# ucl-exoplanets/wayne

Measured on AMD Instinct MI355X. Metric: simulated WFC3-IR exposures/sec (1014x1014, NSAMP=16, spatial scan), higher is better.
Workload: dtype k_ramp<float, true, 1, false, true>: exact integer sums (int64 accumulators + int32 sky counts) then an all-f32 per-read chain; f32 thrower (int32 LDS tiles -> int64 fixed-point accumulators, 2^-28 e-); f32 reads; 1 GPU; cfg4: G141 spatial scan 5 px/s, SUBARRAY=1024 (frame 1014x1014), SPARS10 NSAMP=16, K=128 sub-samples, W=4494 bins, 9.92e+08 electrons/exposure, all detector effects on (flat, sky, cosmic rays, gain, dark, non-linearity, clip, read noise), thrower=split (wide component per electron, narrow component multinomial), f32 reads (the default of ExposureGenerator, Observation, VisitRunner and the CLI), on; exposures_per_rank=2241

## Files before the change

include/wayne_hip.h:

```cpp
#ifndef WAYNE_HIP_H
#define WAYNE_HIP_H

#include <stddef.h>
#include <stdint.h>

#ifdef __cplusplus
extern "C" {
#endif

#define WAYNE_ABI_VERSION 7

#define WAYNE_OK 0
#define WAYNE_E_INVALID (-1)
#define WAYNE_E_NEGATIVE (-2)
#define WAYNE_E_OVERFLOW (-3)
#define WAYNE_E_NOMEM (-4)
#define WAYNE_E_HIP (-5)
#define WAYNE_E_NODEVICE (-6)
#define WAYNE_E_STATE (-7)

#define WAYNE_RNG_REPLAY 0
#define WAYNE_RNG_PHILOX 1
#define WAYNE_RNG_SPLIT 2

// ... 64 lines not shown
  const float *lin[4];
  const float *dark_sci;
  const float *dark_err;
  const double *zero_read;
} wayne_calibration;

int wayne_ctx_set_calibration(wayne_ctx *ctx, const wayne_calibration *c);


typedef struct wayne_exposure_desc {
  uint32_t seed;
  uint32_t exposure_index;
  int rng_mode;
  int threads_compat;
  uint32_t flags;
  int sub_scale;

  int n_wl;
  const double *wl_um;
  const double *flux;
  const double *depth;

  int n_samples;
  const double *x_ref;
  const double *y_ref;
  const double *dur_ms;
  const int32_t *replay_seed;
  const int32_t *sample_read;

  int n_reads;
  const double *read_dt_s;

  double sky_ct_s;
  double cosmic_rate;
  double scale_factor;
  double noise_mean;
  double noise_std;

  int thrower_margin;
  int thrower_splits;

  const double *lc_z;
  const double *lc_hidden;
  const double *lc_rp;
  double lc_ld[4];
} wayne_exposure_desc;

int wayne_ctx_slots(const wayne_ctx *ctx);
int wayne_exposure_upload(wayne_ctx *ctx, int slot, const wayne_exposure_desc *d);
int wayne_exposure_run(wayne_ctx *ctx, int slot);
int wayne_exposure_run_checked(wayne_ctx *ctx, int slot);
int wayne_exposure_status(wayne_ctx *ctx, int slot, int *status);
unsigned long long wayne_ctx_reruns(const wayne_ctx *ctx);
int wayne_exposure_download(wayne_ctx *ctx, int slot, void *out_reads);
int wayne_exposure_fetch_async(wayne_ctx *ctx, int slot);
int wayne_exposure_wait(wayne_ctx *ctx, int slot, void **host_reads);
void *wayne_exposure_device_reads(wayne_ctx *ctx, int slot);
int wayne_exposure_synthesize(wayne_ctx *ctx, const wayne_exposure_desc *d,
                              void *out_reads);

int wayne_exposure_debug_fetch(wayne_ctx *ctx, int slot, int32_t *counts,
                               double *x_pos, double *y_pos, double *acc_e);
int wayne_exposure_debug_depth(wayne_ctx *ctx, int slot, double *depth);
int wayne_exposure_debug_boxes(wayne_ctx *ctx, int slot, int32_t *boxes, int32_t *segments, int *use_box);
int wayne_exposure_run_front(wayne_ctx *ctx, int slot);
int wayne_exposure_run_back(wayne_ctx *ctx, int slot);
int wayne_exposure_ramp_variant(wayne_ctx *ctx, int slot, char *buf, int cap);


typedef struct wayne_source_desc {
  uint32_t tag;
  int n_wl;
  const double *wl_um;
  const double *flux;
  double dx, dy;
} wayne_source_desc;

#define WAYNE_MAX_SOURCES 8

int wayne_exposure_set_sources(wayne_ctx *ctx, int slot, const wayne_source_desc *src, int n);
uint32_t wayne_source_seed(uint32_t seed, uint32_t tag);
int wayne_exposure_debug_fetch_source(wayne_ctx *ctx, int slot, int source, int32_t *counts, double *x_pos,
                                      double *y_pos);


typedef struct wayne_trap_desc {
  double n_traps[2];
  double efficiency[2];
  double lifetime_s[2];
  int n_rate;
  double rate_lo, rate_hi;
  const double *start[2];
} wayne_trap_desc;

#define WAYNE_MAX_TRAP_RATES 4096

int wayne_exposure_set_traps(wayne_ctx *ctx, int slot, const wayne_trap_desc *t);

typedef struct wayne_trap_history_desc {
  double gap_s;
  int lit;
  double fill[2];
} wayne_trap_history_desc;

int wayne_ctx_trap_state_reset(wayne_ctx *ctx, const double initial[2]);
int wayne_ctx_trap_state_upload(wayne_ctx *ctx, const float *state);
int wayne_ctx_trap_state_download(wayne_ctx *ctx, float *state);

int wayne_exposure_set_trap_history(wayne_ctx *ctx, int slot, const wayne_trap_history_desc *h);


#define WAYNE_X_LINEARISE (1u << 0)
#define WAYNE_X_DARK (1u << 1)
#define WAYNE_X_GAIN (1u << 2)
#define WAYNE_X_SKY (1u << 3)
#define WAYNE_X_LAST_READ (1u << 4)
#define WAYNE_X_ALL 31u

typedef struct wayne_extract_desc {
  uint32_t steps;
  int row_lo[17];
  int row_hi[17];
  int bg_col_lo;
  int bg_col_hi;
} wayne_extract_desc;

int wayne_exposure_set_extraction(wayne_ctx *ctx, int slot, const wayne_extract_desc *x);
int wayne_exposure_fetch_spectra_async(wayne_ctx *ctx, int slot);
int wayne_exposure_wait_spectra(wayne_ctx *ctx, int slot, double **spectra, double **sky);
int wayne_exposure_download_spectra(wayne_ctx *ctx, int slot, double *spectra, double *sky);
typedef struct wayne_crrej_desc {
  double k;
  double read_noise_e;
} wayne_crrej_desc;

int wayne_exposure_set_crrej(wayne_ctx *ctx, int slot, const wayne_crrej_desc *r);
int wayne_exposure_rejected(wayne_ctx *ctx, int slot, const uint32_t **n_rejected);
int wayne_exposure_download_crmask(wayne_ctx *ctx, int slot, uint16_t *mask);
#define WAYNE_C_FLAT (1u << 0)
#define WAYNE_MAX_CHANNELS 256
#define WAYNE_MAX_CHANNEL_HULL 384

typedef struct wayne_channels_desc {
  int n_channels;
  const double *edges_um;
  const double *wl_a;
  const double *wl_b;
  uint32_t flags;
} wayne_channels_desc;

int wayne_exposure_set_channels(wayne_ctx *ctx, int slot, const wayne_channels_desc *d);
int wayne_exposure_channels(wayne_ctx *ctx, int slot, const double **channels);
typedef struct wayne_variance_desc {
  double read_noise;
} wayne_variance_desc;

int wayne_exposure_set_variance(wayne_ctx *ctx, int slot, const wayne_variance_desc *v);
int wayne_exposure_variances(wayne_ctx *ctx, int slot, const double **spectra_var, const double **sky_var,
                             const double **channels_var);
#define WAYNE_MAX_OPTIMAL_HALF_WIDTH 16
typedef struct wayne_optimal_desc {
  int half_width;
} wayne_optimal_desc;

int wayne_exposure_set_optimal(wayne_ctx *ctx, int slot, const wayne_optimal_desc *d);
int wayne_exposure_optimal(wayne_ctx *ctx, int slot, const double **optimal, const double **optimal_var);
// ... 104 lines not shown
```

wayne_amd/_lib.py:

```python
import ctypes as C
import os
import threading
import weakref

import numpy as np

from . import build as _build

OK, E_INVALID, E_NEGATIVE, E_OVERFLOW, E_NOMEM, E_HIP, E_NODEVICE, E_STATE = 0, -1, -2, -3, -4, -5, -6, -7
RNG_REPLAY, RNG_PHILOX, RNG_SPLIT = 0, 1, 2
F_ADD_FLAT = 1 << 0
F_ADD_GAIN_VARIATIONS = 1 << 1
F_ADD_NON_LINEAR = 1 << 2
F_CLIP_DET_LIMITS = 1 << 3
F_ADD_READ_NOISE = 1 << 4
F_ADD_STELLAR_NOISE = 1 << 5
F_ADD_DARK = 1 << 6
F_ADD_INITIAL_BIAS = 1 << 7
F_OUT_F64 = 1 << 16
F_OUT_U16 = 1 << 18
OUT_FLAGS = {np.dtype(np.float32): 0, np.dtype(np.float64): F_OUT_F64, np.dtype(np.uint16): F_OUT_U16}
F_EXACT_SAMPLERS = 1 << 17
PROF_KERNELS = 8
ABI_VERSION = 7
# ... 73 lines not shown

class CrrejDesc(C.Structure):
    _fields_ = [("k", C.c_double), ("read_noise_e", C.c_double)]


class ChannelsDesc(C.Structure):
    _fields_ = [("n_channels", C.c_int), ("edges_um", _dp), ("wl_a", _dp), ("wl_b", _dp), ("flags", C.c_uint32)]


class VarianceDesc(C.Structure):
    _fields_ = [("read_noise", C.c_double)]


class RampFitDesc(C.Structure):
    _fields_ = [("steps", C.c_uint32), ("read_noise_e", C.c_double), ("k_jump", C.c_double), ("saturation_dn", C.c_double)]


class ImaDesc(C.Structure):
    _fields_ = [("steps", C.c_uint32), ("units", C.c_int), ("read_noise_e", C.c_double), ("saturation_dn", C.c_double)]


class SpotsDesc(C.Structure):
    _fields_ = [("n", C.c_int32), ("cx", C.c_double * 8), ("cy", C.c_double * 8), ("radius", C.c_double * 8),
                ("contrast", C.POINTER(C.c_double)), ("px", C.POINTER(C.c_double)), ("py", C.POINTER(C.c_double))]


class IpcDesc(C.Structure):
    _fields_ = [("k", (C.c_double * 3) * 3)]


class OptimalDesc(C.Structure):
    _fields_ = [("half_width", C.c_int)]


class Profile(C.Structure):
    _fields_ = [("name", C.c_char_p * PROF_KERNELS), ("launches", C.c_uint64 * PROF_KERNELS),
                ("ms", C.c_double * PROF_KERNELS), ("electrons", C.c_uint64)]


_vp = C.c_void_p
SYMBOLS = {
    "wayne_abi_version": (C.c_int, []),
    "wayne_strerror": (C.c_char_p, [C.c_int]),
    "wayne_build_flags": (C.c_char_p, []),
    "wayne_device_count": (C.c_int, []),
    "wayne_ctx_create": (_vp, [C.c_int, C.POINTER(C.c_int)]),
    "wayne_ctx_destroy": (None, [_vp]),
    "wayne_last_error": (C.c_char_p, [_vp]),
    "wayne_ctx_synchronize": (C.c_int, [_vp]),
    "wayne_ctx_stream": (_vp, [_vp]),
    "wayne_ctx_set_knob": (C.c_int, [_vp, C.c_char_p, C.c_longlong]),
    "wayne_ctx_get_knob": (C.c_int, [_vp, C.c_char_p, C.POINTER(C.c_longlong)]),
    "wayne_psf_apply": (C.c_int, [_vp, _vp, C.c_int, _vp, _vp, _vp, _vp, _vp, C.c_int, C.c_int,
                                  C.c_uint32, C.c_int, C.c_int, C.c_uint32, C.c_uint32, _vp]),
    "wayne_psf_apply_ex": (C.c_int, [_vp, _vp, C.c_int, _vp, _vp, _vp, _vp, _vp, C.c_int, C.c_int,
                                     C.c_uint32, C.c_int, C.c_int, C.c_uint32, C.c_uint32, C.c_uint32, _vp]),
    "wayne_ctx_set_grism": (C.c_int, [_vp, C.POINTER(GrismDesc)]),
    "wayne_ctx_set_calibration": (C.c_int, [_vp, C.POINTER(Calibration)]),
    "wayne_ctx_slots": (C.c_int, [_vp]),
    "wayne_exposure_upload": (C.c_int, [_vp, C.c_int, C.POINTER(ExposureDesc)]),
    "wayne_exposure_run": (C.c_int, [_vp, C.c_int]),
    "wayne_exposure_run_checked": (C.c_int, [_vp, C.c_int]),
    "wayne_exposure_status": (C.c_int, [_vp, C.c_int, C.POINTER(C.c_int)]),
    "wayne_ctx_reruns": (C.c_ulonglong, [_vp]),
    "wayne_exposure_download": (C.c_int, [_vp, C.c_int, _vp]),
    "wayne_exposure_fetch_async": (C.c_int, [_vp, C.c_int]),
    "wayne_exposure_wait": (C.c_int, [_vp, C.c_int, C.POINTER(C.c_void_p)]),
    "wayne_exposure_device_reads": (_vp, [_vp, C.c_int]),
    "wayne_exposure_synthesize": (C.c_int, [_vp, C.POINTER(ExposureDesc), _vp]),
    "wayne_exposure_debug_fetch": (C.c_int, [_vp, C.c_int, _vp, _vp, _vp, _vp]),
    "wayne_exposure_debug_depth": (C.c_int, [_vp, C.c_int, _vp]),
    "wayne_exposure_debug_boxes": (C.c_int, [_vp, C.c_int, _vp, _vp, C.POINTER(C.c_int)]),
    "wayne_exposure_run_front": (C.c_int, [_vp, C.c_int]),
    "wayne_exposure_run_back": (C.c_int, [_vp, C.c_int]),
    "wayne_exposure_ramp_variant": (C.c_int, [_vp, C.c_int, C.c_char_p, C.c_int]),
    "wayne_exposure_set_sources": (C.c_int, [_vp, C.c_int, C.POINTER(SourceDesc), C.c_int]),
    "wayne_source_seed": (C.c_uint32, [C.c_uint32, C.c_uint32]),
    "wayne_exposure_set_traps": (C.c_int, [_vp, C.c_int, C.POINTER(TrapDesc)]),
    "wayne_ctx_trap_state_reset": (C.c_int, [_vp, _dp]),
    "wayne_ctx_trap_state_upload": (C.c_int, [_vp, _vp]),
    "wayne_ctx_trap_state_download": (C.c_int, [_vp, _vp]),
    "wayne_exposure_set_trap_history": (C.c_int, [_vp, C.c_int, C.POINTER(TrapHistoryDesc)]),
    "wayne_exposure_debug_fetch_source": (C.c_int, [_vp, C.c_int, C.c_int, _vp, _vp, _vp]),
    "wayne_exposure_set_extraction": (C.c_int, [_vp, C.c_int, C.POINTER(ExtractDesc)]),
    "wayne_exposure_fetch_spectra_async": (C.c_int, [_vp, C.c_int]),
    "wayne_exposure_wait_spectra": (C.c_int, [_vp, C.c_int, C.POINTER(_dp), C.POINTER(_dp)]),
    "wayne_exposure_download_spectra": (C.c_int, [_vp, C.c_int, _vp, _vp]),
    "wayne_exposure_set_crrej": (C.c_int, [_vp, C.c_int, C.POINTER(CrrejDesc)]),
    "wayne_exposure_rejected": (C.c_int, [_vp, C.c_int, C.POINTER(C.POINTER(C.c_uint32))]),
    "wayne_exposure_download_crmask": (C.c_int, [_vp, C.c_int, _vp]),
    "wayne_exposure_set_channels": (C.c_int, [_vp, C.c_int, C.POINTER(ChannelsDesc)]),
    "wayne_exposure_channels": (C.c_int, [_vp, C.c_int, C.POINTER(_dp)]),
    "wayne_exposure_set_variance": (C.c_int, [_vp, C.c_int, C.POINTER(VarianceDesc)]),
    "wayne_exposure_variances": (C.c_int, [_vp, C.c_int, C.POINTER(_dp), C.POINTER(_dp), C.POINTER(_dp)]),
    "wayne_exposure_set_optimal": (C.c_int, [_vp, C.c_int, C.POINTER(OptimalDesc)]),
    "wayne_exposure_optimal": (C.c_int, [_vp, C.c_int, C.POINTER(_dp), C.POINTER(_dp)]),
    "wayne_exposure_deliver_profile": (C.c_int, [_vp, C.c_int, C.c_int]),
    "wayne_exposure_set_optimal_profile": (C.c_int, [_vp, C.c_int, _dp, C.POINTER(C.c_int)]),
    "wayne_exposure_set_optimal_profile_tagged": (C.c_int, [_vp, C.c_int, _dp, C.POINTER(C.c_int), C.c_uint64]),
    "wayne_ctx_profile_uploads": (C.c_ulonglong, [_vp]),
    "wayne_exposure_set_optimal_channels": (C.c_int, [_vp, C.c_int, C.c_int]),
    "wayne_exposure_optimal_channels": (C.c_int, [_vp, C.c_int, C.POINTER(_dp), C.POINTER(_dp)]),
    "wayne_exposure_fetch_profile": (C.c_int, [_vp, C.c_int]),
    "wayne_exposure_profile": (C.c_int, [_vp, C.c_int, C.POINTER(_dp), C.POINTER(C.c_size_t)]),
    "wayne_extract_profile": (C.c_int, [_vp, C.POINTER(C.c_uint64), C.POINTER(C.c_double)]),
    "wayne_fits_layout": (C.c_int, [C.c_int, C.c_int, C.c_uint32, C.POINTER(C.c_size_t), C.POINTER(C.c_size_t),
                                    C.POINTER(C.c_int)]),
    "wayne_exposure_set_fits": (C.c_int, [_vp, C.c_int, C.c_int]),
    "wayne_exposure_fetch_fits_async": (C.c_int, [_vp, C.c_int]),
    "wayne_exposure_wait_fits": (C.c_int, [_vp, C.c_int, C.POINTER(C.c_void_p)]),
    "wayne_exposure_download_fits": (C.c_int, [_vp, C.c_int, _vp]),
    "wayne_fits_profile": (C.c_int, [_vp, C.POINTER(C.c_uint64), C.POINTER(C.c_double)]),
    "wayne_exposure_set_expected": (C.c_int, [_vp, C.c_int, C.c_int]),
    "wayne_exposure_download_expected": (C.c_int, [_vp, C.c_int, _dp]),
    "wayne_expected_profile": (C.c_int, [_vp, C.POINTER(C.c_uint64), C.POINTER(C.c_double)]),
    "wayne_exposure_set_rampfit": (C.c_int, [_vp, C.c_int, C.POINTER(RampFitDesc)]),
    "wayne_exposure_download_rampfit": (C.c_int, [_vp, C.c_int, _dp, _dp, C.POINTER(C.c_uint32)]),
    "wayne_rampfit_profile": (C.c_int, [_vp, C.POINTER(C.c_uint64), C.POINTER(C.c_double)]),
    "wayne_ima_layout": (C.c_int, [C.c_int, C.c_int, C.POINTER(C.c_size_t), C.POINTER(C.c_size_t), C.POINTER(C.c_size_t)]),
    "wayne_exposure_set_ima": (C.c_int, [_vp, C.c_int, C.POINTER(ImaDesc)]),
    "wayne_exposure_download_ima": (C.c_int, [_vp, C.c_int, _vp]),
    "wayne_ima_profile": (C.c_int, [_vp, C.POINTER(C.c_uint64), C.POINTER(C.c_double)]),
    "wayne_ipc_weights": (C.c_int, [C.POINTER(IpcDesc), C.POINTER(C.c_int32)]),
    "wayne_exposure_set_ipc": (C.c_int, [_vp, C.c_int, C.POINTER(IpcDesc)]),
    "wayne_ipc_profile": (C.c_int, [_vp, C.POINTER(C.c_uint64), C.POINTER(C.c_double)]),
    "wayne_exposure_set_limb_darkening": (C.c_int, [_vp, C.c_int, _dp, C.c_int]),
    "wayne_exposure_set_spots": (C.c_int, [_vp, C.c_int, C.POINTER(SpotsDesc), C.c_int, C.c_int]),
    "wayne_spot_lens_basis": (None, [C.c_double] * 6 + [_dp]),
    "wayne_spot_rule": (None, [_dp, _dp]),
    "wayne_spots_profile": (C.c_int, [_vp, C.POINTER(C.c_uint64), C.POINTER(C.c_double)]),
    "wayne_profile_enable": (C.c_int, [_vp, C.c_int]),
    "wayne_profile_select": (C.c_int, [_vp, C.c_uint]),
    "wayne_profile_reset": (C.c_int, [_vp]),
    "wayne_profile_get": (C.c_int, [_vp, C.POINTER(Profile)]),
    "wayne_philox4x32": (None, [_vp, _vp, _vp]),
    "wayne_host_sample_draws": (None, [C.c_uint32, C.c_uint32, C.c_int, _vp, _vp, _vp]),
}

_lib = None


def load():
    global _lib, _lib_path
    if _lib is None:
        path = _build.LIB
        override = os.environ.get("WAYNE_HIP_LIB")
        if override:
            path = override
        elif _build.stale():
            if os.path.exists(_build.HIPCC):
                _build.build(verbose=False)
            elif not os.path.exists(path):
                raise ImportError("libwayne_hip.so is not built and hipcc is unavailable (%s)" % _build.HIPCC)
        L = C.CDLL(path)
        for name, (res, args) in SYMBOLS.items():
            f = getattr(L, name)
            f.restype = res
            f.argtypes = args
        if L.wayne_abi_version() != ABI_VERSION:
            raise ImportError("libwayne_hip.so ABI version mismatch")
        flags = L.wayne_build_flags().decode().split()
        if flags and os.environ.get("WAYNE_ALLOW_FLAGGED_LIB", "") != "1":
            raise ImportError("%s was built with %s: not the product's library (tests and measurement scripts that mean "
                              "to load it set WAYNE_ALLOW_FLAGGED_LIB=1)" % (path, " ".join(flags)))
        _lib = L
        _lib_path = path
    return _lib


_lib_path = None


def library_info():
    L = load()
    return _lib_path or _build.LIB, L.wayne_build_flags().decode().strip()


def ptr(a, ctype=None):
    if a is None:
        return None
    assert a.flags["C_CONTIGUOUS"]
    if ctype is None:
        return a.ctypes.data_as(C.c_void_p)
    return a.ctypes.data_as(C.POINTER(ctype))


def out_dtype_of(flags):
    return np.dtype(np.float64 if flags & F_OUT_F64 else np.uint16 if flags & F_OUT_U16 else np.float32)


def f64(a):
    return np.ascontiguousarray(a, dtype=np.float64)


def f32(a):
    return np.ascontiguousarray(a, dtype=np.float32)


def i32(a):
    return np.ascontiguousarray(a, dtype=np.int32)


KNOBS = ("tile_ints", "batch", "thin", "no_acc_box", "lane_reach", "throw_wgs", "keep_narrow", "no_fuse", "fork_narrow",
         "streams", "upload_timing", "ramp_reads", "narrow_compact", "lane_tight_tile",
         "fuse_thrower", "prep_wl_per_run")
_live_contexts = weakref.WeakSet()
_knob_defaults = {}


def set_knob_all(name, value):
    if name not in KNOBS:
        raise KeyError("no knob named %r" % (name,))
    if value is None:
        _knob_defaults.pop(name, None)
    else:
        _knob_defaults[name] = int(value)
    for c in list(_live_contexts):
        if getattr(c, "_h", None):
            c.set_knob(name, value)


def reset_knobs_all():
    for name in list(_knob_defaults):
        set_knob_all(name, None)


class Context(object):

    def __init__(self, device=0):
        self._L = load()
        st = C.c_int(0)
        self._h = self._L.wayne_ctx_create(int(device), C.byref(st))
        if not self._h:
            msg = self._L.wayne_strerror(st.value).decode()
            cls = WayneNoDeviceError if st.value == E_NODEVICE else WayneError
            raise cls(st.value, "wayne_ctx_create(device=%d): %s -- the HIP path is the only path, "
                                "there is no CPU fallback" % (device, msg))
        self.device = device
        self._slot_meta = {}
        self._slot_src = {}
        self._slot_crrej = set()
        self._slot_chan = {}
        self._slot_var = set()
        self._slot_opt = set()
        self._slot_optch = set()
        self._slot_prof = set()
        self._slot_fits = {}
        self._slot_expected = {}
        self._slot_rampfit = {}
        self._slot_ima = {}
        _live_contexts.add(self)
        for name, value in _knob_defaults.items():
            self.set_knob(name, value)

    def close(self):
        if getattr(self, "_h", None):
            self._L.wayne_ctx_destroy(self._h)
            self._h = None

    def __del__(self):
        try:
            self.close()
        except Exception:
            pass

    def __enter__(self):
        return self

    def __exit__(self, *a):
        self.close()

    def check(self, status):
        if status != OK:
            raise WayneError(status, self._L.wayne_last_error(self._h).decode())

    def synchronize(self):
        self.check(self._L.wayne_ctx_synchronize(self._h))

    def set_knob(self, name, value):
        self.check(self._L.wayne_ctx_set_knob(self._h, name.encode(), -1 if value is None else int(value)))

    def get_knob(self, name):
        v = C.c_longlong(0)
        self.check(self._L.wayne_ctx_get_knob(self._h, name.encode(), C.byref(v)))
        return None if v.value < 0 else int(v.value)

    @property
    def stream(self):
# ... 472 lines not shown
        self.check(self._L.wayne_extract_profile(self._h, C.byref(n), C.byref(ms)))
        return {"launches": int(n.value), "ms": float(ms.value)}

    def set_ipc(self, slot, ipc):
        if ipc is None:
            self.check(self._L.wayne_exposure_set_ipc(self._h, int(slot), None))
            return
        self.check(self._L.wayne_exposure_set_ipc(self._h, int(slot), C.byref(ipc_desc(ipc))))

    def ipc_profile(self):
        n, ms = C.c_uint64(0), C.c_double(0.0)
        self.check(self._L.wayne_ipc_profile(self._h, C.byref(n), C.byref(ms)))
        return int(n.value), float(ms.value)

    def set_traps(self, slot, traps):
        if traps is None:
            self.check(self._L.wayne_exposure_set_traps(self._h, int(slot), None))
            return
        m, table = traps.traps, np.ascontiguousarray(traps.table, dtype=np.float64)
        if table.ndim != 2 or table.shape[0] != 2:
            raise ValueError("charge traps: the start tables have shape (2, G)")
        t = TrapDesc()
        t.n_traps[:] = [float(v) for v in m.array("n_traps")]
        t.efficiency[:] = [float(v) for v in m.array("efficiency")]
        t.lifetime_s[:] = [float(v) for v in m.array("lifetime_s")]
        t.n_rate, t.rate_lo, t.rate_hi = int(table.shape[1]), float(m.rate_lo), float(m.rate_hi)
        rows = [np.ascontiguousarray(table[0]), np.ascontiguousarray(table[1])]
        t.start[0], t.start[1] = ptr(rows[0], C.c_double), ptr(rows[1], C.c_double)
        self.check(self._L.wayne_exposure_set_traps(self._h, int(slot), C.byref(t)))

    def set_trap_history(self, slot, history):
        if history is None:
            self.check(self._L.wayne_exposure_set_trap_history(self._h, int(slot), None))
            return
        h = TrapHistoryDesc()
        h.gap_s, h.lit = float(history.gap_s), int(bool(history.lit))
        h.fill[:] = [float(v) for v in history.fill]
        self.check(self._L.wayne_exposure_set_trap_history(self._h, int(slot), C.byref(h)))

    def trap_state_reset(self, initial):
        v = (C.c_double * 2)(float(initial[0]), float(initial[1]))
        self.check(self._L.wayne_ctx_trap_state_reset(self._h, v))

    def trap_state_upload(self, state):
        if not getattr(self, "S", 0):
            raise WayneError(E_STATE, "trap_state_upload: set the calibration first")
        state = np.ascontiguousarray(state, dtype=np.float32)
        if state.shape != (self.S, self.S, 2):
            raise ValueError("trap state: expected shape (%d, %d, 2), got %s" % (self.S, self.S, state.shape))
        self.check(self._L.wayne_ctx_trap_state_upload(self._h, state.ctypes.data_as(C.c_void_p)))

    def trap_state_download(self):
        if not getattr(self, "S", 0):
            raise WayneError(E_STATE, "trap_state_download: set the calibration first")
        out = np.empty((self.S, self.S, 2), dtype=np.float32)
        self.check(self._L.wayne_ctx_trap_state_download(self._h, out.ctypes.data_as(C.c_void_p)))
        return out

    def set_sources(self, slot, sources):
        sources = list(sources)
        arr = (SourceDesc * max(len(sources), 1))()
        keep = []
        for i, s in enumerate(sources):
            wl, fl = f64(s.wl), f64(s.flux)
            if wl.size != fl.size:
                raise ValueError("contaminant %d: wl and flux differ in length" % i)
            keep += [wl, fl]
            arr[i].tag, arr[i].n_wl = int(s.tag), wl.size
            arr[i].wl_um, arr[i].flux = ptr(wl, C.c_double), ptr(fl, C.c_double)
            arr[i].dx, arr[i].dy = float(s.dx), float(s.dy)
        self._slot_src[slot] = ()
        self.check(self._L.wayne_exposure_set_sources(self._h, int(slot), arr, len(sources)))
        self._slot_src[slot] = tuple(int(k.size) for k in keep[0::2])

    def debug_fetch_source(self, slot, source):
        K, W, R, _ = self._slot_meta[slot]
        if source > 0:
            W = self._slot_src[slot][source - 1]
        counts = np.empty((K, W), dtype=np.int32)
        x = np.empty((K, W), dtype=np.float64)
        y = np.empty((K, W), dtype=np.float64)
        self.check(self._L.wayne_exposure_debug_fetch_source(self._h, int(slot), int(source), ptr(counts), ptr(x), ptr(y)))
        return counts, x, y

    def run(self, slot):
        self.check(self._L.wayne_exposure_run(self._h, int(slot)))

    def run_checked(self, slot):
        self.check(self._L.wayne_exposure_run_checked(self._h, int(slot)))

    def run_front(self, slot):
        self.check(self._L.wayne_exposure_run_front(self._h, int(slot)))

    def run_back(self, slot):
        self.check(self._L.wayne_exposure_run_back(self._h, int(slot)))

    def ramp_variant(self, slot):
        buf = C.create_string_buffer(128)
        self.check(self._L.wayne_exposure_ramp_variant(self._h, int(slot), buf, len(buf)))
        return buf.value.decode()

    def status(self, slot):
        st = C.c_int(0)
        self.check(self._L.wayne_exposure_status(self._h, int(slot), C.byref(st)))
        return st.value

    @property
    def reruns(self):
        return int(self._L.wayne_ctx_reruns(self._h))

    def download(self, slot):
        K, W, R, dtype = self._slot_meta[slot]
        out = np.empty((R + 1, self.S, self.S), dtype=dtype)
        self.check(self._L.wayne_exposure_download(self._h, int(slot), ptr(out)))
        return out

    def fetch_async(self, slot):
        self.check(self._L.wayne_exposure_fetch_async(self._h, int(slot)))

    def wait(self, slot):
        K, W, R, dtype = self._slot_meta[slot]
        p = C.c_void_p()
        self.check(self._L.wayne_exposure_wait(self._h, int(slot), C.byref(p)))
        n = (R + 1) * self.S * self.S
        buf = (C.c_ubyte * (n * dtype.itemsize)).from_address(p.value)
        return np.frombuffer(buf, dtype=dtype).reshape(R + 1, self.S, self.S)

    def synthesize(self, desc):
        self.upload(0, desc)
        self.run(0)
        return self.download(0)

    def debug_depth(self, slot):
        K, W, R, _ = self._slot_meta[slot]
        out = np.empty((K, W), dtype=np.float64)
        self.check(self._L.wayne_exposure_debug_depth(self._h, int(slot), ptr(out)))
        return out

    def debug_boxes(self, slot):
        boxes = np.zeros((16, 4), dtype=np.int32)
        seg = np.zeros(16, dtype=np.int32)
        use = C.c_int(0)
        self.check(self._L.wayne_exposure_debug_boxes(self._h, int(slot), ptr(boxes), ptr(seg), C.byref(use)))
        return bool(use.value), boxes, seg

    def debug_fetch(self, slot, acc=False):
        K, W, R, _ = self._slot_meta[slot]
        counts = np.empty((K, W), dtype=np.int32)
        x = np.empty((K, W), dtype=np.float64)
        y = np.empty((K, W), dtype=np.float64)
        a = np.empty((R, self.S, self.S), dtype=np.float64) if acc else None
        self.check(self._L.wayne_exposure_debug_fetch(self._h, int(slot), ptr(counts), ptr(x), ptr(y), ptr(a)))
        return counts, x, y, a

    def profile_enable(self, on=True):
        self.check(self._L.wayne_profile_enable(self._h, 1 if on else 0))

    def profile_select(self, names=None):
        if names is None:
            mask = 0xFFFFFFFF
        else:
            order = list(self.profile_get().keys())[:PROF_KERNELS] + ["k_extract", "k_fits_words", "k_expect", "k_ramp_fit", "k_ima", "k_ipc",
                                                                     "k_lightcurve_spots"]
            mask = 0
            for n in names:
                mask |= 1 << order.index(n)
# ... 184 lines not shown
```

wayne_amd/csrc/common.h:

```cpp
#pragma once
#include <hip/hip_runtime.h>
#include <stdint.h>
#include <type_traits>
#include "philox.h"
#include "plan_consts.h"
#include "samplers.h"

namespace wayne {

constexpr int kQBits = 28;
constexpr double kQ = 268435456.0;
constexpr double kInvQ = 1.0 / 268435456.0;
constexpr double kGain = 2.35;
constexpr double kReadNoise = 14.1 / 2.35;
constexpr double kMinCounts = -20.0;
constexpr double kMaxCounts = 78000.0;
constexpr double kPi = 3.14159265358979323846;



struct SubInfo {
  uint32_t electrons;
  int tx0, ty0, tw, th;
  int read;
  int replay_seed;
  int pad_;
  double x_ref, y_ref;
  double a_t_i, a_w, b_w;
  double inv_norm;
};

struct WlArrays {
  double* ratio;
  double* sigl;
  double* sigh;
  double* sens;
  double* dlam;
};

__device__ __forceinline__ double poly3(const double* c, double x) {
  return ((c[0] * x + c[1]) * x + c[2]) * x + c[3];
}

#if defined(__HIPCC__)
struct BinLocal { float fx, fy; int ox, oy; bool sane; };
__device__ __forceinline__ BinLocal bin_local(double xd, double yd) {
  BinLocal b;
  const bool sane = fabs(xd) < 1e6 && fabs(yd) < 1e6;
  b.sane = sane;
  const double flx = sane ? floor(xd) : 0., fly = sane ? floor(yd) : 0.;
  b.fx = (float)(xd - flx); b.fy = (float)(yd - fly);
  b.ox = (int)flx; b.oy = (int)fly;
#ifdef WAYNE_NEGCTL_DROP_FRACTION
  b.fx = 0.f; b.fy = 0.f;
#endif
  return b;
}
__device__ __forceinline__ int floor_to_int(float v) {
  int r;
  asm("v_cvt_flr_i32_f32 %0, %1" : "=v"(r) : "v"(v));
  return r;
}


template <int CTRL> __device__ __forceinline__ int dpp_row(int v) { return __builtin_amdgcn_update_dpp(v, v, CTRL, 0xF, 0xF, false); }
#define WAYNE_ROW16(name, T, cast_in, cast_out, op)                                   \
  __device__ __forceinline__ T name(T v) {                                            \
    v = op(v, cast_out(dpp_row<0x128>(cast_in(v))));                   \
    v = op(v, cast_out(dpp_row<0x124>(cast_in(v))));                   \
    v = op(v, cast_out(dpp_row<0x122>(cast_in(v))));                   \
    v = op(v, cast_out(dpp_row<0x121>(cast_in(v))));                   \
    return v;                                                                         \
  }
__device__ __forceinline__ int wayne_addi(int a, int b) { return a + b; }
WAYNE_ROW16(row16_min, float, __float_as_int, __int_as_float, fminf)
WAYNE_ROW16(row16_max, float, __float_as_int, __int_as_float, fmaxf)
WAYNE_ROW16(row16_mini, int, , , min)
WAYNE_ROW16(row16_maxi, int, , , max)
WAYNE_ROW16(row16_sum, int, , , wayne_addi)
#undef WAYNE_ROW16
__device__ __forceinline__ int wave_mini(int v) {
  v = row16_mini(v);
  return min(min(__builtin_amdgcn_readlane(v, 0), __builtin_amdgcn_readlane(v, 16)),
             min(__builtin_amdgcn_readlane(v, 32), __builtin_amdgcn_readlane(v, 48)));
}
__device__ __forceinline__ int wave_maxi(int v) {
  v = row16_maxi(v);
  return max(max(__builtin_amdgcn_readlane(v, 0), __builtin_amdgcn_readlane(v, 16)),
             max(__builtin_amdgcn_readlane(v, 32), __builtin_amdgcn_readlane(v, 48)));
}
__device__ __forceinline__ unsigned long long wave_sum_u32(uint32_t n) {
  const int lo = row16_sum((int)(n & 0xFFFFFFu)), hi = row16_sum((int)(n >> 24));
  const unsigned long long L = (unsigned long long)(uint32_t)(__builtin_amdgcn_readlane(lo, 0) + __builtin_amdgcn_readlane(lo, 16) +
                                                              __builtin_amdgcn_readlane(lo, 32) + __builtin_amdgcn_readlane(lo, 48));
  const unsigned long long H = (unsigned long long)(uint32_t)(__builtin_amdgcn_readlane(hi, 0) + __builtin_amdgcn_readlane(hi, 16) +
                                                              __builtin_amdgcn_readlane(hi, 32) + __builtin_amdgcn_readlane(hi, 48));
  return L + (H << 24);
}
#endif

}
```

wayne_amd/csrc/k_narrow.h:

```cpp
#pragma once
#include "common.h"
#include "k_throw.h"

namespace wayne {

constexpr int kNarrowCells = 2 * kNarrowR + 1;
constexpr int kPoolRows = 2 * kNarrowR + 2;
constexpr int kNarrowTile = 1536;

constexpr float kTailCut = 6.5f;
template <class M>
__device__ __forceinline__ float upper_tail(float t) {
  if (__all(t > kTailCut)) return 0.f;
  const float z = t * 0.70710678118654752f;
  const float u = M::div_(1.f, 1.f + 0.5f * z);
  float p = 0.17087277f;
  p = fmaf(p, u, -0.82215223f);
  p = fmaf(p, u, 1.48851587f);
  p = fmaf(p, u, -1.13520398f);
  p = fmaf(p, u, 0.27886807f);
  p = fmaf(p, u, -0.18628806f);
  p = fmaf(p, u, 0.09678418f);
  p = fmaf(p, u, 0.37409196f);
  p = fmaf(p, u, 1.00002368f);
  p = fmaf(p, u, -1.26551223f);
  p = fmaf(-z, z, p);
  return (t > kTailCut) ? 0.f : (0.5f * u) * M::exp_(p);
}

constexpr int kLaneTile = 9216;
constexpr int kNarrowLds = kNarrowTile + kPoolRows * kNarrowThreads + 2 * kNarrowThreads;
constexpr int kThrowerLds = kNarrowLds > kLaneTile ? kNarrowLds : kLaneTile;

template <int FLUSH, bool FAST, bool COMPACT>
__device__ __forceinline__ void narrow_body(const ThrowArgs& a, int* const lds, const unsigned by) {
  typedef typename std::conditional<FAST, FastMath, ExactMath<float> >::type M;
  int* const tile = lds;
  float (*const s_q)[kNarrowThreads] = reinterpret_cast<float (*)[kNarrowThreads]>(lds + kNarrowTile);
  int* const s_pool = lds + kNarrowTile + kPoolRows * kNarrowThreads;
  float* const s_cond = reinterpret_cast<float*>(s_pool + kNarrowThreads);
  __shared__ int s_box[4];
  __shared__ float s_fc[10];
  __shared__ int s_gx[COMPACT ? kNarrowThreads / 16 : 1], s_gj[COMPACT ? kNarrowThreads / 16 : 1], s_hist[COMPACT ? 32 : 1];
  if (threadIdx.x < 10) s_fc[threadIdx.x] = (float)kStirlingSmall[threadIdx.x];
  if (COMPACT && threadIdx.x < 32) s_hist[threadIdx.x] = 0;
  const int k = blockIdx.x;
  const int tid = threadIdx.x;
  const uint32_t order_word = reinterpret_cast<const uint32_t*>(a.chunk_order)[by >> 2];
  const int w = (int)((order_word >> (8 * (by & 3))) & 0xFFu) * kNarrowThreads + tid;
  const SubInfo si = a.sub[k];
  int n0 = 0;
  double xd = 0., yd = 0., sgd = 1.;
  if (w < a.W) {
    const size_t kw = (size_t)k * a.W + w;
    n0 = a.nsplit[kw];
    xd = a.xpos[kw];
    yd = a.ypos[kw];
    sgd = a.sigl[w];
  }
  if (!__syncthreads_or(n0 > 0)) return;
  const bool split = n0 > 0;
  BinLocal bl{};
  if (split) bl = bin_local(xd, yd);
  const bool act = split && bl.sane;
  const float sg = split ? (float)sgd : 1.f;
  const int ic0 = bl.ox, jc0 = bl.oy;
  s_pool[tid] = 0;
  if (tid == 0) { s_box[0] = 0x7FFFFFFF; s_box[1] = -0x7FFFFFFF; s_box[2] = 0x7FFFFFFF; s_box[3] = -0x7FFFFFFF; }
  __syncthreads();
  {
    const int x_lo = wave_mini(act ? ic0 - kNarrowR : 0x7FFFFFFF), x_hi = wave_maxi(act ? ic0 + kNarrowR + 1 : -0x7FFFFFFF);
    const int y_lo = wave_mini(act ? jc0 - kNarrowR : 0x7FFFFFFF), y_hi = wave_maxi(act ? jc0 + kNarrowR + 1 : -0x7FFFFFFF);
    if ((tid & 63) == 0) {
      atomicMin(&s_box[0], x_lo); atomicMax(&s_box[1], x_hi);
      atomicMin(&s_box[2], y_lo); atomicMax(&s_box[3], y_hi);
    }
  }
  __syncthreads();
  int tx0 = max(s_box[0], 1), tx1 = min(s_box[1], a.N), ty0 = max(s_box[2], 1), ty1 = min(s_box[3], a.N);
  int tw = max(tx1 - tx0, 0), th = max(ty1 - ty0, 0);
  if ((long long)tw * th > kNarrowTile) { th = min(th, kNarrowTile / max(tw, 1)); if (th < 1) { th = 0; tw = 0; } }
  const int tarea = tw * th;
  for (int i = tid; i < tarea; i += kNarrowThreads) tile[i] = 0;

  auto deposit = [&](int ci, int rj, int m) {
    const int lx = ci - tx0, ly = rj - ty0;
    if ((unsigned)lx < (unsigned)tw && (unsigned)ly < (unsigned)th)
      atomicAdd(&tile[ly * tw + lx], m);
    else if (ci > 0 && ci < a.N && rj > 0 && rj < a.N)
      deposit_global<FLUSH>(a, si, ci, rj, m);
  };

  const bool any_multi = __any(act);
  const float inv_s = 1.f / sg;
  const int grp = tid & ~15, gl = tid & 15;
  bool pool = false;
  int X0 = 0, J0 = 0, res = 0;
  float Z = 1.f, Rb = 0.f, yl = 0.f;
  if (any_multi) {
    const int cnt = row16_sum(split ? 1 : 0), cnt_sane = row16_sum(act ? 1 : 0), tot = row16_sum(split ? n0 : 0);
    const int icmin = row16_mini(act ? ic0 : 0x7FFFFFFF), icmax = row16_maxi(act ? ic0 : -0x7FFFFFFF);
    const int jcmin = row16_mini(act ? jc0 : 0x7FFFFFFF);
    X0 = icmin - kNarrowR;
    J0 = jcmin - kNarrowR;
    yl = act ? (float)(yd - (double)J0) : 0.f;
    const float ymin = row16_min(act ? yl : 3e38f), ymax = row16_max(act ? yl : -3e38f);
    const float smin = row16_min(split ? sg : 3e38f), smax = row16_max(split ? sg : 0.f);
    pool = cnt >= 2 && cnt_sane == cnt && icmax - icmin <= 2 && (ymax - ymin) <= 0.25f * smin && smax <= 1.1f * smin &&
           tot <= 16777216;

    float qh[kPoolRows];
#pragma unroll
    for (int t = 0; t < kPoolRows; ++t) qh[t] = 3e38f;
    if (act && pool) {
      float Ep = -yl, Ap = upper_tail<M>(fabsf(Ep) * inv_s), S = 0.f;
#pragma unroll
      for (int t = 0; t < kPoolRows; ++t) {
        const float E = (float)(t + 1) - yl, A = upper_tail<M>(fabsf(E) * inv_s);
        const float m = (Ep >= 0.f) ? Ap - A : ((E <= 0.f) ? A - Ap : 1.f - Ap - A);
        qh[t] = fmaxf(m, 0.f);
        S += qh[t];
        Ep = E; Ap = A;
      }
#pragma unroll
      for (int t = 0; t < kPoolRows; ++t) qh[t] = M::div_(qh[t], S);
    } else if (act) {
      const float f = bl.fy;
      float up = upper_tail<M>((1.f - f) * inv_s), lo = upper_tail<M>(f * inv_s);
      s_q[0][tid] = 1.f - up - lo;
      for (int c = 1; c < kNarrowCells; ++c) {
        const int d = (c + 1) >> 1;
        const float rem = up + lo;
        float Q;
        if (c & 1) { const float nx = upper_tail<M>(((float)(d + 1) - f) * inv_s); Q = up - nx; up = nx; }
        else       { const float nx = upper_tail<M>(((float)d + f) * inv_s);       Q = lo - nx; lo = nx; }
        s_q[c][tid] = fminf(fmaxf(M::div_(Q, rem), 0.f), 1.f);
      }
    }
    if (__any(pool)) {
      float qb[kPoolRows];
#pragma unroll
      for (int t = 0; t < kPoolRows; ++t) qb[t] = row16_min(qh[t]);
      float PL[kNarrowR + 1], SU[kPoolRows + 1];
      PL[0] = qb[0];
#pragma unroll
      for (int t = 1; t <= kNarrowR; ++t) PL[t] = PL[t - 1] + qb[t];
      SU[kPoolRows] = 0.f;
#pragma unroll
      for (int t = kPoolRows - 1; t > kNarrowR; --t) SU[t] = SU[t + 1] + qb[t];
      Z = fminf(PL[kNarrowR] + SU[kNarrowR + 1], 1.f);
      if (act && pool) {
#pragma unroll
        for (int t = 0; t < kPoolRows; ++t) {
          Rb += qh[t] - qb[t];
          s_q[t][tid] = Rb;
        }
      }
      if (pool && gl == 0) {
        s_cond[grp] = fminf(fmaxf(M::div_(qb[kNarrowR], PL[kNarrowR] + SU[kNarrowR + 1]), 0.f), 1.f);
#pragma unroll
        for (int i = 1; i < kPoolRows; ++i) {
          const int u = (i + 1) >> 1;
// ... 83 lines not shown
          if (left > 0.f) {
            m = binomial<M>(left, s_cond[grp + i], rp, s_fc);
            left -= m;
          }
          if (m > 0.f) {
            const int u = (i + 1) >> 1;
            deposit(X0 + gl, J0 + ((i & 1) ? kNarrowR + u : kNarrowR - u), (int)m);
          }
        }
      }
    }
  }
  if (COMPACT) {
    __builtin_amdgcn_fence(__ATOMIC_RELEASE, "wavefront");
    __builtin_amdgcn_wave_barrier();
    __builtin_amdgcn_fence(__ATOMIC_ACQUIRE, "wavefront");
    const int mine = pool ? s_pool[tid] : 0;
    if (gl == 0) { s_gx[tid >> 4] = X0; s_gj[tid >> 4] = J0; }
    if (__syncthreads_or(mine > 0)) {
      int* const list = reinterpret_cast<int*>(&s_q[0][0]);
      const int cls = (mine > 0) ? 31 - __clz(mine) : 0;
      int rank = 0;
      if (mine > 0) rank = atomicAdd(&s_hist[cls], 1);
      __syncthreads();
      const int lane = tid & 63;
      const int h = (lane < 32) ? s_hist[31 - lane] : 0;
      int incl = h;
#pragma unroll
      for (int off = 1; off < 32; off <<= 1) {
        const int v = __shfl_up(incl, off);
        if (lane >= off) incl += v;
      }
      const int first = __shfl(incl - h, 31 - cls), n_live = __shfl(incl, 31);
      if (mine > 0) list[first + rank] = tid;
      __syncthreads();
      if ((tid & ~63) < n_live) {
        const int slot = (tid < n_live) ? list[tid] : 0;
        float left = (tid < n_live) ? (float)s_pool[slot] : 0.f;
        const int cgrp = slot & ~15, cl = slot & 15;
        const int cX = s_gx[slot >> 4] + cl, cJ0 = s_gj[slot >> 4];
        SeededStream rp(a.seed, STAGE_POOL, (uint32_t)(w - tid + slot) >> 4, (uint32_t)k + a.subsample0, a.exposure, (uint32_t)cl);
        for (int i = 0; i < kPoolRows; ++i) {
          if (!__any(left > 0.f)) break;
          float m = 0.f;
          if (left > 0.f) {
            m = binomial<M>(left, s_cond[cgrp + i], rp, s_fc);
            left -= m;
          }
          if (m > 0.f) {
            const int u = (i + 1) >> 1;
            deposit(cX, cJ0 + ((i & 1) ? kNarrowR + u : kNarrowR - u), (int)m);
          }
        }
      }
    }
  }
  __syncthreads();
  flush_tile<FLUSH, false, kNarrowThreads>(a, si, tile, tx0, ty0, tw, tarea);
}

template <int FLUSH, bool FAST, bool COMPACT>
__global__ __launch_bounds__(kNarrowThreads) void k_narrow(ThrowArgs a) {
  __shared__ int lds[kNarrowLds];
  narrow_body<FLUSH, FAST, COMPACT>(a, lds, blockIdx.y);
}

constexpr float kLaneR16 = 4.63f;
constexpr float kLaneR34 = 6.9f;
constexpr int kLaneMargin = 30;
constexpr int kLaneReachMax = 48;


template <int FLUSH, bool THIN, bool BATCH, bool FUSED>
__device__ __forceinline__ void lane_body(const ThrowArgs& a, const PrepArgs& p, const CosmicArgs& ca, int* const tile, const unsigned by) {
  __shared__ SubInfo s_sub[FUSED ? kLaneBatchMax : 1];
  __shared__ uint32_t s_hits;
  __shared__ unsigned short s_list[THIN ? kLaneListCap : 1];
  __shared__ int s_cnt[2];
  __shared__ int s_box[4];
  __shared__ int s_reach;
  const int k0 = BATCH ? (int)blockIdx.x * a.kb : (int)blockIdx.x, k1 = BATCH ? min(k0 + a.kb, a.K) : k0 + 1;
  const int tid = threadIdx.x;
  const uint32_t order_word = reinterpret_cast<const uint32_t*>(a.lane_order)[by >> 2];
  const int w = (int)((order_word >> (8 * (by & 3))) & 0xFFu) * kLaneThreads + tid;
  const bool inw = w < a.W;
  int n_one = 0, nw_one = 0;
  BinLocal bl_one{};
  float ch = 0.f, cl = 0.f, sh = 0.f, sl = 0.f;
  if (inw) {
    double sh_d = a.sigh[w], sl_d = a.sigl[w];
    if (!FUSED && !BATCH) {
      const size_t kw0 = (size_t)k0 * a.W + w;
      n_one = a.nlane[kw0];
      const double xd = a.xpos[kw0], yd = a.ypos[kw0];
      nw_one = a.nwide[kw0];
      bl_one = bin_local(xd, yd);
      nw_one = min(max(nw_one, 0), n_one);
    }
    sh = (float)sh_d; sl = (float)sl_d;
    ch = (-1.3862943611198906f * sh) * sh;
    cl = (-1.3862943611198906f * sl) * sl;
  }
  const bool bad_h = !(ch > -3e38f), bad_l = !(cl > -3e38f);
  if (bad_h) ch = 0.f;
  if (bad_l) cl = 0.f;
  double f_wl = 0., f_flux = 0., f_sens = 0., f_dlam = 0., f_ratio = 0., f_sigl = 0.;
  unsigned long long f_electrons = 0ull;
  if (FUSED) {
    if (ca.rate >= 0.) {
      const int n_wg = gridDim.x * gridDim.y;
      for (int r = blockIdx.y * gridDim.x + blockIdx.x; r < ca.R; r += n_wg) { cosmic_hits(ca, r, &s_hits); __syncthreads(); }
    }
    if (inw) { f_wl = p.wl[w]; f_flux = p.flux[w]; f_sens = p.wa.sens[w]; f_dlam = p.wa.dlam[w]; f_ratio = p.wa.ratio[w]; f_sigl = p.wa.sigl[w]; }
    if (tid < k1 - k0) {
      const int k = k0 + tid;
      s_sub[tid] = make_sub_info(p, k, p.x_ref[k], p.y_ref[k], p.tr + kTrStride * (size_t)k, 0u, 1e300, -1e300, 1e300, -1e300);
    }
  }
  int x_lo = 0x7FFFFFFF, x_hi = -0x7FFFFFFF, y_lo = 0x7FFFFFFF, y_hi = -0x7FFFFFFF;
  float reach = 0.f;
  bool any = false;
  for (int k = k0; k < k1; ++k) {
    const size_t kw = (size_t)k * a.W + (inw ? w : 0);
    int n = 0, nw = 0;
    int ic = 0, jc = 0;
    bool sane = false;
    if (FUSED) {
      if (inw) {
        float x = 0.f, y = 0.f;
        bin_position_bound(p, f_wl, p.tr + kTrStride * (size_t)k, p.x_ref[k], p.y_ref[k], &x, &y);
        sane = fabsf(x) < 1e6f && fabsf(y) < 1e6f;
        ic = (int)floorf(x); jc = (int)floorf(y);
        n = 2; nw = 1;
      }
    } else if (!BATCH) {
      n = n_one;
      if (n > 0) { sane = bl_one.sane; ic = bl_one.ox; jc = bl_one.oy; nw = nw_one; }
    } else if (inw) {
      n = a.nlane[kw];
      if (n > 0) {
        const BinLocal b = bin_local(a.xpos[kw], a.ypos[kw]);
        sane = b.sane; ic = b.ox; jc = b.oy;
        nw = min(max(a.nwide[kw], 0), n);
      }
    }
    if (n > 0) {
      any = true;
      const bool sig_ok = (nw > 0 ? (sh >= 0.f && sh < 1e6f) : true) && (n > nw ? (sl >= 0.f && sl < 1e6f) : true);
      const float smax = fmaxf(nw > 0 ? sh : 0.f, n > nw ? sl : 0.f);
      float r = sig_ok ? a.lane_reach_sigmas * smax + 1.f : __int_as_float(0x7F800000);
      if (sane) {
        constexpr int spare = FUSED ? 1 : 0;
        x_lo = min(x_lo, ic - spare); x_hi = max(x_hi, ic + spare); y_lo = min(y_lo, jc - spare); y_hi = max(y_hi, jc + spare);
      } else {
        r = __int_as_float(0x7F800000);
      }
      reach = fmaxf(reach, r);
    }
  }
  if (!__syncthreads_or(any)) return;
  if (tid == 0) { s_box[0] = 0x7FFFFFFF; s_box[1] = -0x7FFFFFFF; s_box[2] = 0x7FFFFFFF; s_box[3] = -0x7FFFFFFF; s_reach = 0; s_cnt[0] = 0; s_cnt[1] = 0; }
  __syncthreads();
  {
    x_lo = wave_mini(x_lo); x_hi = wave_maxi(x_hi); y_lo = wave_mini(y_lo); y_hi = wave_maxi(y_hi);
    const int r_hi = wave_maxi(__float_as_int(reach));
    if ((tid & 63) == 0) {
      atomicMin(&s_box[0], x_lo); atomicMax(&s_box[1], x_hi);
      atomicMin(&s_box[2], y_lo); atomicMax(&s_box[3], y_hi);
      atomicMax(&s_reach, r_hi);
    }
  }
  __syncthreads();
  const float reach_wg = __int_as_float(s_reach);
  bool sure = reach_wg <= (float)kLaneReachMax;
  const int margin = sure ? (int)ceilf(reach_wg) : kLaneMargin;
  const int bx0 = s_box[0] - margin, bx1 = s_box[1] + margin + 1, by0 = s_box[2] - margin, by1 = s_box[3] + margin + 1;
  int tx0 = max(bx0, 1), tx1 = min(bx1, a.N), ty0 = max(by0, 1), ty1 = min(by1, a.N);
  int tw = max(tx1 - tx0, 0), th = max(ty1 - ty0, 0);
  sure = sure && s_box[0] <= s_box[1] && tx0 == bx0 && tx1 == bx1 && ty0 == by0 && ty1 == by1 && (long long)tw * th <= kLaneTile;
  while ((long long)tw * th > kLaneTile && th > 1) { ty0 += 1; th = max(th - 2, 1); }
  while ((long long)tw * th > kLaneTile && tw > 1) { tx0 += 1; tw = max(tw - 2, 1); }
  if ((long long)tw * th > kLaneTile) { tw = 0; th = 0; }
  const int tarea = tw * th;
  for (int i = tid; i < tarea; i += kLaneThreads) tile[i] = 0;

  int par = 0;
  auto tile_add = [&](int addr) {
    if (THIN) {
      if (atomicAdd((int*)((char*)tile + addr), 1) == 0) {
        const unsigned long long m = __ballot(1);
        const int before = __builtin_amdgcn_mbcnt_hi((unsigned)(m >> 32), __builtin_amdgcn_mbcnt_lo((unsigned)m, 0u));
        int base = 0;
        if (before == 0) base = atomicAdd(&s_cnt[par], __popcll(m));
        base = __builtin_amdgcn_readfirstlane(base);
        if (base + before < kLaneListCap) s_list[base + before] = (unsigned short)(addr >> 2);
      }
    } else {
      atomicAdd((int*)((char*)tile + addr), 1);
    }
  };

  for (int k = k0; k < k1; ++k) {
  const size_t kw = (size_t)k * a.W + (inw ? w : 0);
  int n = 0, nw = 0;
  BinLocal bl{};
  if (FUSED) {
    if (inw) {
      const BinPlan b = plan_bin(p, k, w, f_wl, f_flux, f_sens, f_dlam, f_ratio, f_sigl, p.tr + kTrStride * (size_t)k, p.x_ref[k],
                                 p.y_ref[k], p.dur_ms[k], p.depth ? p.depth[kw] : 0.);
      p.counts[kw] = (int32_t)b.count;
      if (b.overflow) raise_status(p, 1);
      if (b.narrow > 0u || b.rest > 0u) raise_status(p, 2);
      n = (int)b.lane;
      f_electrons += b.lane;
      if (n > 0) { bl = bin_local(b.xs, b.ys); nw = min(max(b.nwide, 0), n); }
    }
  } else if (!BATCH) {
    n = n_one;
  } else if (inw) {
    n = a.nlane[kw];
  }
  if (!__syncthreads_or(n > 0)) continue;
  const SubInfo si = FUSED ? s_sub[k - k0] : a.sub[__builtin_amdgcn_readfirstlane(k)];
  if (!FUSED && !BATCH) {
    if (n > 0) { bl = bl_one; nw = nw_one; }
  } else if (!FUSED && n > 0) {
    bl = bin_local(a.xpos[kw], a.ypos[kw]);
    nw = min(max(a.nwide[kw], 0), n);
  }
  const float x = n > 0 ? bl.fx : -1e30f, y = n > 0 ? bl.fy : -1e30f;
  const int ox = bl.ox, oy = bl.oy;

  const int tw4 = tw * 4;
  const int origin = (oy - ty0) * tw4 + (ox - tx0) * 4;
  uint32_t refine = 0u;
  auto draw = [&](SeededStream& rng, uint32_t wd, float c, float c16, float px, float py, float& vx, float& vy) {
    const float rev = __uint_as_float(__builtin_amdgcn_alignbit(0x7Fu, wd, 9));
    const uint32_t h = wd & 0xFFFFu;
    float r2 = fmaf(c, __builtin_amdgcn_logf((float)h + 0.5f), c16);
    if (__builtin_expect(h == 0u, 0)) {
      refine = refine * 1664525u + 1013904223u;
      r2 = fmaf(c, __builtin_amdgcn_logf((float)(refine >> 15) + 0.5f), -33.f * c);
    }
    const float Rs = __builtin_amdgcn_sqrtf(r2);
    vx = fmaf(__builtin_amdgcn_cosf(rev), Rs, px);
    vy = fmaf(__builtin_amdgcn_sinf(rev), Rs, py);
  };
  const uint32_t oxl = (uint32_t)ox - (uint32_t)tx0, oyl = (uint32_t)oy - (uint32_t)ty0;
  auto deposit_checked = [&](float vx, float vy) {
    uint32_t lx, ly;
    asm("v_cvt_flr_i32_f32 %0, %2\n\tv_cvt_flr_i32_f32 %1, %3\n\tv_add_u32 %0, %0, %4\n\tv_add_u32 %1, %1, %5"
        : "=&v"(lx), "=&v"(ly) : "v"(vx), "v"(vy), "v"(oxl), "v"(oyl));
    if (lx < (uint32_t)tw && ly < (uint32_t)th) {
      tile_add(__umul24(ly, tw4) + (lx << 2));
    } else {
      const int xi = (int)(lx + (uint32_t)tx0), yi = (int)(ly + (uint32_t)ty0);
      if (xi > 0 && xi < a.N && yi > 0 && yi < a.N) deposit_global<FLUSH>(a, si, xi, yi, 1);
    }
  };
  auto throw_sure = [&](uint32_t wd, float c, float c16, bool live) {
    const float rev = __uint_as_float(__builtin_amdgcn_alignbit(0x7Fu, wd, 9));
    const float Rs = __builtin_amdgcn_sqrtf(fmaf(c, __builtin_amdgcn_logf((float)(wd & 0xFFFFu) + 0.5f), c16));
// ... 124 lines not shown
```

wayne_amd/csrc/k_prep.h:

```cpp
#pragma once
#include "common.h"

namespace wayne {


__device__ __forceinline__ void prep_wl_bin(const GrismDev& g, int W, const double* __restrict__ wl, const WlArrays& o, int i) {
  const double x = wl[i];
  o.ratio[i] = poly3(g.p_ratio, x);
  o.sigl[i] = poly3(g.p_sigl, x);
  o.sigh[i] = poly3(g.p_sigh, x);

  double s;
  const int n = g.n_sens;
  if (n <= 0) {
    s = 1.0;
  } else if (n < 2 || x <= g.sens_wl[0]) {
    s = (x != x) ? x : g.sens_val[0];
  } else if (x >= g.sens_wl[n - 1]) {
    s = g.sens_val[n - 1];
  } else {
    const double w0 = g.sens_wl[0], w1 = g.sens_wl[n - 1];
    int lo = (int)((x - w0) / (w1 - w0) * (double)(n - 1));
    lo = min(max(lo, 0), n - 2);
    if (g.sens_wl[lo] > x) {
// ... 1 lines not shown
        lo -= 1;
      } else {
        int hi = lo;
        lo = 0;
        while (hi - lo > 1) { const int mid = (lo + hi) >> 1; if (g.sens_wl[mid] <= x) lo = mid; else hi = mid; }
      }
    } else if (!(x < g.sens_wl[lo + 1])) {
      if (lo + 2 <= n - 1 && x < g.sens_wl[lo + 2]) {
        lo += 1;
      } else {
        int hi = n - 1;
        lo += 1;
        while (hi - lo > 1) { const int mid = (lo + hi) >> 1; if (g.sens_wl[mid] <= x) lo = mid; else hi = mid; }
      }
    }
    lo = min(lo, n - 2);
    const double slope = (g.sens_val[lo + 1] - g.sens_val[lo]) / (g.sens_wl[lo + 1] - g.sens_wl[lo]);
    s = slope * (x - g.sens_wl[lo]) + g.sens_val[lo];
  }
  o.sens[i] = s;

  double left, right;
  if (W < 2) {
    left = right = 0.0;
  } else {
    left = (i == 0) ? (wl[1] - wl[0]) / 2. : (wl[i] - wl[i - 1]) / 2.;
    right = (i == W - 1) ? (wl[W - 1] - wl[W - 2]) / 2. : (wl[i + 1] - wl[i]) / 2.;
  }
  o.dlam[i] = left + right;
}
__global__ void k_prep_wl(GrismDev g, int W, const double* __restrict__ wl, WlArrays o) {
  const int i = blockIdx.x * blockDim.x + threadIdx.x;
  if (i < W) prep_wl_bin(g, W, wl, o, i);
}
__global__ void k_prep_wl_run(GrismDev g, int W, const double* __restrict__ wl, WlArrays o, uint32_t* misc, int K,
                              const double* __restrict__ x_ref, const double* __restrict__ y_ref, double* __restrict__ tr) {
  const int i = blockIdx.x * blockDim.x + threadIdx.x;
  if (misc && i < 16) misc[i] = 0u;
  if (i < K) {
    double* t = tr + kTrStride * (size_t)i;
    trace_coeffs(g, x_ref[i], y_ref[i], t);
    t[6] = 1. / t[4];
    t[7] = 0.;
  }
  if (i < W) prep_wl_bin(g, W, wl, o, i);
}

struct PrepArgs {
  GrismDev g;
  int W, K, N;
  int sub_scale;
  int margin;
  int max_tile;
  uint32_t seed, exposure;
  uint32_t flags;
  int split_min;
  int lane_max;
  double scale_factor;
  const double* wl;
  const double* flux;
  const double* depth;
  const double* x_ref;
  const double* y_ref;
  const double* dur_ms;
  const int32_t* replay_seed;
  const int32_t* sample_read;
  const double* tr;
  WlArrays wa;
  int32_t* counts;
  int32_t* nwide;
  int32_t* nsplit;
  int32_t* nlane;
  uint32_t* prefix;
  double* xpos;
  double* ypos;
  SubInfo* sub;
  unsigned long long* total_electrons;
  uint32_t* status;
  uint32_t run;
  uint32_t* chunk_total;
  double* chunk_box;
  int fix_inline;
  int no_narrow;
};

__device__ __forceinline__ void raise_status(const PrepArgs& a, int bit) { atomicMax(a.status + (bit >> 1), a.run); }

constexpr int kCounterStripes = 64;
constexpr int kCounterStride = 16;
__device__ __forceinline__ void count_electrons(unsigned long long* counter, unsigned wg, unsigned long long n) {
  atomicAdd(counter + (size_t)kCounterStride * (wg & (kCounterStripes - 1)), n);
}

#ifndef WAYNE_PREP_THREADS
#define WAYNE_PREP_THREADS 512
#endif
constexpr int kPrepThreads = WAYNE_PREP_THREADS;
constexpr int kMaxPrepChunks = 128;

struct CosmicArgs {
  int R, N, S;
  uint32_t seed, exposure;
  double rate;
  const double* read_dt;
  long long* acc;
  uint32_t* seg;
};

__device__ __forceinline__ void cosmic_hits(const CosmicArgs& a, int r, uint32_t* s_n) {
  if (threadIdx.x == 0) {
    const double rate_size = a.rate / (1024. * 1024.) * (double)((long long)a.N * a.N);
    PhiloxStream rng(a.seed, STAGE_CR_COUNT, 0u, (uint32_t)r, a.exposure);
    double n = poisson<ExactMath<double> >(rate_size * a.read_dt[r], rng);
    if (!(n >= 0.)) n = 0.;
    if (n > 1e7) n = 1e7;
    *s_n = (uint32_t)n;
  }
  __syncthreads();
  const uint32_t n = *s_n;
  for (uint32_t i = threadIdx.x; i < n; i += blockDim.x) {
    const u32x4 w = philox4x32_10(i, 0u, (uint32_t)r, a.exposure, a.seed, STAGE_CR_HIT);
    const uint32_t energy = 10000u + uint_below(w.v[0], 25000u);
    const uint32_t y = uint_below(w.v[1], (uint32_t)a.N);
    const uint32_t x = uint_below(w.v[2], (uint32_t)a.N);
    const long long q = (long long)energy << kQBits;
    const size_t pix = (size_t)(y + kBorder) * a.S + (x + kBorder);
    atomicAdd((unsigned long long*)&a.acc[(size_t)r * a.S * a.S + pix], (unsigned long long)q);
    atomicOr(&a.seg[pix >> 6], 1u << r);
  }
}

#if defined(__HIP_DEVICE_COMPILE__)
__device__ __forceinline__ int ptrs_squeeze(double lam, double k, double lhs_arg) {
  const double d = k - lam;
  if (!(k >= 10. && lam <= 4194304. && fabs(d) <= 0.25 * lam)) return 0;
  const float df = (float)d, kf = (float)k;
  const float rl = __builtin_amdgcn_rcpf((float)lam), rk = __builtin_amdgcn_rcpf(kf);
  const float x = df * rl;
  float p = 1.f / 15.f;
  p = fmaf(p, x, -1.f / 14.f); p = fmaf(p, x, 1.f / 13.f); p = fmaf(p, x, -1.f / 12.f);
  p = fmaf(p, x, 1.f / 11.f);  p = fmaf(p, x, -1.f / 10.f); p = fmaf(p, x, 1.f / 9.f);
  p = fmaf(p, x, -1.f / 8.f);  p = fmaf(p, x, 1.f / 7.f);   p = fmaf(p, x, -1.f / 6.f);
  p = fmaf(p, x, 1.f / 5.f);   p = fmaf(p, x, -1.f / 4.f);  p = fmaf(p, x, 1.f / 3.f);
  p = fmaf(p, x, -0.5f);
  const float scale = fmaf(df * df, rl, 1.f);
  const float ln2 = 0.6931471805599453f;
  const float rhs = -(df * df) * rl - kf * (p * x * x) - 0.5f * ln2 * __builtin_amdgcn_logf(6.283185307179586f * kf) -
                    rk * (1.f / 12.f - rk * rk * (1.f / 360.f));
  const float D = ln2 * __builtin_amdgcn_logf((float)lhs_arg) - rhs;
  const float eps = 2e-4f * scale;
  return (D <= -eps) ? 1 : ((D >= eps) ? -1 : 0);
}

template <class RNG>
__device__ __forceinline__ double poisson_small(double lam, RNG& rng) {
  const double u = u01d(rng.next());
  const float lf = (float)lam, uf = (float)u;
  float p = FastMath::exp_(-lf), c = p;
  int k = 0;
  bool unsure = true;
  for (int it = 1; it < 64; ++it) {
    const float tol = fmaf(c, 2e-5f, 2e-7f);
    if (uf <= c - tol) { unsure = false; break; }
    if (!(uf > c + tol)) break;
    p = p * (lf * (1.0f / (float)it));
    c = c + p;
// ... 85 lines not shown
  const double y = __dadd_rn(__dmul_rn(m_t, x - x_ref), c_t) + y_ref;
  *xs = x - (double)a.sub_scale;
  *ys = y - (double)a.sub_scale;
}
__device__ __forceinline__ void bin_position_bound(const PrepArgs& a, double wl, const double* tr, double x_ref, double y_ref,
                                                   float* xs, float* ys) {
  const double x = (wl - tr[5]) * tr[6];
  const double y = fma(tr[0], x - x_ref, tr[1]) + y_ref;
  *xs = (float)(x - (double)a.sub_scale);
  *ys = (float)(y - (double)a.sub_scale);
}
__device__ __forceinline__ double bin_mean_counts(const PrepArgs& a, double flux_w, double sens_w, double dlam_w, double dur,
                                                  double depth) {
  double f = flux_w;
  if (a.depth) f = f * (1. - depth);
  double lam = f * sens_w;
  lam = lam * dlam_w;
  lam = lam * 1e4;
  lam = lam * dur;
  lam = lam * 1e-3;
  lam = lam * a.scale_factor;
  return lam;
}
__device__ __forceinline__ BinPlan plan_bin(const PrepArgs& a, int k, int w, double wl, double flux_w, double sens_w,
                                            double dlam_w, double ratio_w, double sigl_w, const double* tr,
                                            double x_ref, double y_ref, double dur, double depth) {
  BinPlan o;
  bin_position(a, wl, tr, x_ref, y_ref, &o.xs, &o.ys);
  const double lam = bin_mean_counts(a, flux_w, sens_w, dlam_w, dur, depth);
  double cnt;
  if ((a.flags & (1u << 5)) != 0) {
    PhiloxStream rng(a.seed, STAGE_COUNTS, (uint32_t)w, (uint32_t)k, a.exposure);
    cnt = poisson_counts(lam, rng);
  } else {
    cnt = rint(lam);
  }
  o.overflow = false;
  if (!(cnt >= 0.)) cnt = 0.;
  if (cnt > 2147483647.) { cnt = 2147483647.; o.overflow = true; }
  const uint32_t c = (uint32_t)cnt;
  o.count = c;
  const double nw = (double)(int32_t)c * ratio_w;
  o.nwide = (nw >= 2147483647.) ? 2147483647 : (nw <= -2147483648.) ? (int32_t)(-2147483647 - 1) : (int32_t)nw;
  o.narrow = 0u; o.lane = 0u; o.rest = c;
  if (a.nsplit) {
    const uint32_t wide = (uint32_t)min(max(o.nwide, 0), (int32_t)min(c, 0x7FFFFFFFu));
    const uint32_t narrow = c - wide;
    const bool split = a.split_min > 0 && narrow >= (uint32_t)a.split_min && narrow <= kSplitMaxNarrow && sigl_w > 0.05 &&
                       sigl_w * 6.5 <= (double)kNarrowR;
    const uint32_t ind = split ? wide : c;
    const bool lane = a.split_min > 0 && ind <= (uint32_t)a.lane_max;
    o.narrow = split ? narrow : 0u;
    o.lane = lane ? ind : 0u;
    o.rest = lane ? 0u : ind;
  }
  return o;
}

__global__ __launch_bounds__(kPrepThreads) void k_prep_sub(PrepArgs a, CosmicArgs ca) {
  const int k = blockIdx.x;
  const int ch = blockIdx.y;
  const int tid = threadIdx.x;
  const int lane = tid & 63, wave = tid >> 6;
  const int W = a.W;
  constexpr int NW = kPrepThreads / 64;
  __shared__ uint32_t s_wsum[NW];
  __shared__ double s_red[4][NW];
  __shared__ uint32_t s_hits;

  if (ca.rate >= 0.) {
    const int n_wg = gridDim.x * gridDim.y;
    for (int r = blockIdx.y * gridDim.x + blockIdx.x; r < ca.R; r += n_wg) { cosmic_hits(ca, r, &s_hits); __syncthreads(); }
  }
  const double x_ref = a.x_ref[k], y_ref = a.y_ref[k];
  const double* s_tr = a.tr + kTrStride * (size_t)k;
  const double dur = a.dur_ms[k];

  double xmin = 1e300, xmax = -1e300, ymin = 1e300, ymax = -1e300;
  bool overflow = false;
  uint32_t n_split = 0;

  const int w = ch * kPrepThreads + tid;
  uint32_t c = 0;
  if (w < W) {
    const size_t kw = (size_t)k * W + w;
    const BinPlan b = plan_bin(a, k, w, a.wl[w], a.flux[w], a.wa.sens[w], a.wa.dlam[w], a.wa.ratio[w], a.wa.sigl[w], s_tr,
                               x_ref, y_ref, dur, a.depth ? a.depth[kw] : 0.);
    a.xpos[kw] = b.xs;
    a.ypos[kw] = b.ys;
    a.counts[kw] = (int32_t)b.count;
    a.nwide[kw] = b.nwide;
    overflow = b.overflow;
    c = b.count;
    if (c > 0) {
      xmin = fmin(xmin, b.xs); xmax = fmax(xmax, b.xs);
      ymin = fmin(ymin, b.ys); ymax = fmax(ymax, b.ys);
    }
    if (a.nsplit) {
      a.nsplit[kw] = (int32_t)b.narrow;
      a.nlane[kw] = (int32_t)b.lane;
      n_split = b.narrow + b.lane;
      c = b.rest;
      if (a.fix_inline && c > 0u) raise_status(a, 2);
      if (a.no_narrow && b.narrow > 0u) raise_status(a, 2);
    }
  }
  if (overflow) raise_status(a, 1);
  const unsigned long long n_split_total = wave_sum_u32(n_split);
  __shared__ unsigned long long s_split[NW];
  if (lane == 0) s_split[wave] = n_split_total;

  if (!a.fix_inline) {
    uint32_t incl = c;
#pragma unroll
    for (int off = 1; off < 64; off <<= 1) {
      const uint32_t v = __shfl_up(incl, off);
      if (lane >= off) incl += v;
    }
    if (lane == 63) s_wsum[wave] = incl;
    for (int off = 32; off > 0; off >>= 1) {
      xmin = fmin(xmin, __shfl_down(xmin, off));
      xmax = fmax(xmax, __shfl_down(xmax, off));
      ymin = fmin(ymin, __shfl_down(ymin, off));
      ymax = fmax(ymax, __shfl_down(ymax, off));
    }
    if (lane == 0) {
      s_red[0][wave] = xmin; s_red[1][wave] = xmax;
      s_red[2][wave] = ymin; s_red[3][wave] = ymax;
    }
    __syncthreads();
    uint64_t wave_off = 0, chunk_total = 0;
#pragma unroll
    for (int i = 0; i < NW; ++i) {
      const uint32_t t = s_wsum[i];
      if (i < wave) wave_off += t;
      chunk_total += t;
    }
    if (chunk_total > 0xFFFFFFFFull) raise_status(a, 1);
    if (w < W) a.prefix[(size_t)k * (W + 1) + w] = (uint32_t)(wave_off + incl - c);
    if (tid == 0) {
      for (int i = 1; i < NW; ++i) {
        xmin = fmin(xmin, s_red[0][i]); xmax = fmax(xmax, s_red[1][i]);
        ymin = fmin(ymin, s_red[2][i]); ymax = fmax(ymax, s_red[3][i]);
      }
      const size_t ci = (size_t)k * gridDim.y + ch;
      a.chunk_total[ci] = (uint32_t)chunk_total;
      a.chunk_box[4 * ci + 0] = xmin; a.chunk_box[4 * ci + 1] = xmax;
      a.chunk_box[4 * ci + 2] = ymin; a.chunk_box[4 * ci + 3] = ymax;
    }
  }
  __syncthreads();
  if (tid == 0) {
    unsigned long long tot = 0;
    for (int i = 0; i < NW; ++i) tot += s_split[i];
    if (tot) count_electrons(a.total_electrons, blockIdx.y * gridDim.x + blockIdx.x, tot);
  }

  if (a.fix_inline && ch == 0 && tid == 0) a.sub[k] = make_sub_info(a, k, x_ref, y_ref, s_tr, 0u, 1e300, -1e300, 1e300, -1e300);
}

__global__ __launch_bounds__(kPrepThreads) void k_prep_fix(PrepArgs a, int n_chunks) {
  const int k = blockIdx.x;
  const int tid = threadIdx.x;
  const int W = a.W;
  __shared__ uint32_t s_off[kMaxPrepChunks];
  __shared__ uint32_t s_E;
  __shared__ int s_over;
  if (tid == 0) {
    uint64_t run = 0;
    int over = 0;
    for (int i = 0; i < n_chunks; ++i) {
      s_off[i] = (uint32_t)run;
      run += a.chunk_total[(size_t)k * n_chunks + i];
      if (run > 0xFFFFFFFFull) over = 1;
    }
    s_E = (uint32_t)run;
    s_over = over;
  }
  __syncthreads();
  for (int w = tid; w < W; w += kPrepThreads) a.prefix[(size_t)k * (W + 1) + w] += s_off[w / kPrepThreads];
  if (tid == 0) {
    if (s_over) raise_status(a, 1);
    double xmin = 1e300, xmax = -1e300, ymin = 1e300, ymax = -1e300;
    for (int i = 0; i < n_chunks; ++i) {
      const size_t ci = (size_t)k * n_chunks + i;
      xmin = fmin(xmin, a.chunk_box[4 * ci + 0]); xmax = fmax(xmax, a.chunk_box[4 * ci + 1]);
      ymin = fmin(ymin, a.chunk_box[4 * ci + 2]); ymax = fmax(ymax, a.chunk_box[4 * ci + 3]);
    }
    const double x_ref = a.x_ref[k], y_ref = a.y_ref[k];
    double tr[6];
    trace_coeffs(a.g, x_ref, y_ref, tr);
    const uint32_t E = s_E;
    a.prefix[(size_t)k * (W + 1) + W] = E;
    a.sub[k] = make_sub_info(a, k, x_ref, y_ref, tr, E, xmin, xmax, ymin, ymax);
    count_electrons(a.total_electrons, k, (unsigned long long)E);
  }
}

}
```

wayne_amd/csrc/k_ramp.h:

```cpp
#pragma once
#include "common.h"

namespace wayne {

struct RampArgs {
  int R, N, S;
  uint32_t seed, exposure, flags;
  double sky_ct_s;
  double noise_mean, noise_std;
  const double* read_dt;
  long long* acc;
  const float* pfl;
  const float* sky;
  const float* lin[4];
  const float* dark_sci;
  const float* dark_err;
  const double* zero_read;
  void* out;
  const uint32_t* sky_alias;
  uint32_t alias_mask;
  int sky_levels;
  float sky_level[16];
  unsigned char sky_tab0[16];
  float bg[16];
  int tab0[16];
  int use_box;
  int box[16][4];
  uint32_t* seg;
};

struct TrapArgs {
  const double* start_d;
  const float* start_f;
  int G;
  double rate_lo, ln_lo, u_scale;
  double eta[2], eta_n[2], inv_tau[2];
  double sum_dt;
  double sum_bg;
  float eta_f[2], eta_n_f[2], inv_tau_f[2], inv_sum_dt_f, sum_bg_f;
  float dt[16], inv_dt[16];
};

struct TrapHistArgs {
  float2* state;
  double gap_s;
  float gap_f;
  int lit;
  double fill[2];
  float fill_f[2];
  double n[2];
  float n_f[2];
};

__device__ __forceinline__ float one_minus_exp_neg(float x) {
  const float p = x * fmaf(x, fmaf(x, fmaf(x, fmaf(x, 1.f / 120.f, -1.f / 24.f), 1.f / 6.f), -0.5f), 1.f);
  return x < 0.125f ? p : 1.0f - __builtin_amdgcn_exp2f(-1.4426950408889634f * x);
}
__device__ __forceinline__ double one_minus_exp_neg(double x) { return -expm1(-x); }

template <class T>
__device__ __forceinline__ T trap_step(T E, T f, T dt, T eta, T eta_n, T inv_tau) {
  const T c = eta_n * f + inv_tau;
  T einf;
  if constexpr (std::is_same<T, float>::value) einf = (eta * f) * __builtin_amdgcn_rcpf(c);
  else einf = (eta * f) / c;
  return E + (einf - E) * one_minus_exp_neg(c * dt);
}

template <class T>
__device__ __forceinline__ T trap_start(const T* tab, const TrapArgs& t, int pop, T f) {
  const T* e = tab + pop * t.G;
  const T lo = (T)t.rate_lo;
  if (!(f > (T)0)) return e[0];
  if (f < lo) return e[0] + (e[1] - e[0]) * (f / lo);
  T ln_f;
  if constexpr (std::is_same<T, float>::value) ln_f = __logf(f);
  else ln_f = log(f);
  const T u = (ln_f - (T)t.ln_lo) * (T)t.u_scale;
  if (!(u < (T)(t.G - 2))) return e[t.G - 1];
  const int i = (int)u;
  const T w = u - (T)i;
  return e[1 + i] + (e[2 + i] - e[1 + i]) * w;
}


#ifndef WAYNE_RAMP_THREADS
#define WAYNE_RAMP_THREADS 1024
#endif
constexpr int kRampThreads = WAYNE_RAMP_THREADS;

template <bool FAST>
__device__ __forceinline__ void bm_pair(uint32_t w0, uint32_t w1, float& z0, float& z1) {
  const float rev = rev12(w0), ub = u01f(w1);
  if (FAST) {
    const float Rr = __builtin_amdgcn_sqrtf(-1.3862943611198906f * __builtin_amdgcn_logf(ub));
// ... 126 lines not shown
  k += (wr > sr.t2) ? 1 : 0;
  if (wr > sr.t3) {
    k += 1;
    const float u = u01f(wr);
    float t = sr.term3, cdf = sr.c3;
#pragma nounroll
    for (int it = 4; it < 512; ++it) {
      t = t * FastMath::div_(sr.m, (float)it);
      const float cn = cdf + t;
#ifndef WAYNE_NEGCTL_SKY_RUNAWAY
      if (cn == cdf) break;
#endif
      cdf = cn;
      if (!(u > cdf)) break;
      k = k + 1;
    }
  }
  return k;
}

template <bool FAST>
__device__ __forceinline__ void sky_counts(const RampArgs& a, uint32_t p, int tid, bool active, float skyv,
                                           const float* s_c, uint32_t (*s_sky)[kRampThreads]) {
  typedef typename std::conditional<FAST, FastMath, ExactMath<float> >::type M;
  SeededStream rng(a.seed, STAGE_SKY, p, 0u, a.exposure);
  int r = 0, mode = 0, guard = 0;
  PtrsSetup<M> ps;
  ps.lam = ps.b = ps.a = ps.vr = ps.loglam = ps.invalpha = 0.f;
  float prod = 1.f, enlam = 0.f, kk = 0.f, lam = 0.f;
  const int R = a.R;
  while (__any(active)) {
    if (active) {
      float done = -1.f;
      if (mode == 0) {
        lam = skyv * s_c[r];
        if (!(lam > 0.f)) {
          done = 0.f;
        } else if (lam < 10.f) {
          enlam = M::exp_(-lam); prod = 1.f; kk = 0.f; mode = 1;
        } else if (lam < 256.f) {
          if (lam != ps.lam) ps.init(lam);
          mode = 2;
        } else {
          done = (float)poisson<ExactMath<double> >((double)lam, rng);
        }
      }
      if (mode == 1) {
        prod = prod * M::u01(rng.next());
        if (prod > enlam) kk = kk + 1.f; else done = kk;
      } else if (mode == 2) {
        uint32_t w1, w2;
        rng.next2(w1, w2);
        float k;
        if (ps.trial(w1, w2, k)) done = k;
      }
      if (++guard > 64 + 600 * kMaxReads && done < 0.f) done = floorf(lam + 0.5f);
      if (done >= 0.f) {
        s_sky[r][tid] = (uint32_t)done;
        mode = 0;
        if (++r >= R) active = false;
      }
    }
  }
}

template <class OutT, bool FAST, int SKY, bool NOISE, bool ALLON, bool TRAP = false, bool HIST = false>
__device__ __forceinline__ void ramp_body(const RampArgs& a, const TrapArgs& tr = TrapArgs{},
                                          const TrapHistArgs& th = TrapHistArgs{}) {
  static_assert(TRAP || !HIST, "a carried history needs the traps");
  constexpr bool ALIAS = SKY != 0;
  constexpr bool U16 = std::is_same<OutT, uint16_t>::value;
  typedef typename std::conditional<U16, float, OutT>::type ArithT;
  constexpr bool PROD = std::is_same<ArithT, float>::value && FAST && SKY == 1 && !NOISE;
  typedef typename std::conditional<FAST, FastMath, ExactMath<float> >::type M;
  static_assert(kSkyAlias <= kRampThreads, "the sky tables and the per-thread sky counts share one LDS array");
  __shared__ uint32_t s_tab[kMaxReads][ALIAS ? kSkyAlias : kRampThreads];
  __shared__ float s_c[kMaxReads + 1];
  __shared__ int s_tab0[kMaxReads + 1];
  const int S = a.S;
  const int tid = threadIdx.x;
  const int p_raw = blockIdx.x * blockDim.x + tid;
  const bool valid = p_raw < S * S;
  const int p = valid ? p_raw : 0;
  const int Y = p / S, X = p - Y * S;
  const bool interior = valid && (X >= kBorder && X < S - kBorder && Y >= kBorder && Y < S - kBorder);
  const size_t SS = (size_t)S * S;
  OutT* out = (OutT*)a.out;
  const bool clip = (a.flags & (1u << 3)) != 0;
  const bool rdn = (a.flags & (1u << 4)) != 0;
  const bool do_dark = (a.flags & (1u << 6)) != 0 && a.dark_sci && a.dark_err;
  const bool do_lin = (a.flags & (1u << 2)) != 0 && a.lin[0];
  const bool gainvar = (a.flags & (1u << 1)) != 0 && a.pfl;
  const bool do_noise = NOISE && (a.noise_mean != 0.) && (a.noise_std != 0.);
  const bool do_sky = a.sky_ct_s > 0. && a.sky;

  typedef unsigned v2u __attribute__((ext_vector_type(2)));
  const int n_acc = (int)((size_t)a.R * SS * sizeof(long long)), n_f32 = (int)((size_t)a.R * SS * sizeof(float));
  const int n_out = (int)((size_t)(a.R + 1) * SS * sizeof(OutT));
  const __amdgpu_buffer_rsrc_t rs_acc = __builtin_amdgcn_make_buffer_rsrc((void*)a.acc, 0, n_acc, 0x00020000);
  const __amdgpu_buffer_rsrc_t rs_ds = __builtin_amdgcn_make_buffer_rsrc((void*)a.dark_sci, 0, a.dark_sci ? n_f32 : 0, 0x00020000);
  const __amdgpu_buffer_rsrc_t rs_de = __builtin_amdgcn_make_buffer_rsrc((void*)a.dark_err, 0, a.dark_err ? n_f32 : 0, 0x00020000);
  const __amdgpu_buffer_rsrc_t rs_out = __builtin_amdgcn_make_buffer_rsrc((void*)out, 0, n_out, 0x00020000);
  const uint32_t off8 = (uint32_t)p * 8u, off4 = (uint32_t)p * 4u, offo = (uint32_t)p * (uint32_t)sizeof(OutT);
  const uint32_t acc_plane = (uint32_t)(SS * sizeof(long long)), f32_plane = (uint32_t)(SS * sizeof(float));
  const uint32_t out_plane = (uint32_t)(SS * sizeof(OutT));
  constexpr int kNT = 2;
  auto ld_acc = [&](int r) -> long long {
    const v2u w = __builtin_amdgcn_raw_buffer_load_b64(rs_acc, off8, (uint32_t)r * acc_plane, 0);
    return (long long)(((unsigned long long)w.y << 32) | w.x);
  };
  auto ld_f32 = [&](const __amdgpu_buffer_rsrc_t& rs, int r) -> float {
#ifdef WAYNE_TIMING_RAMP_NO_DARK
    return 0.02f + 1e-9f * (float)(r + (int)off4);
#endif
    return __uint_as_float(__builtin_amdgcn_raw_buffer_load_b32(rs, off4, (uint32_t)r * f32_plane, kNT));
  };
  auto st_out = [&](int plane, ArithT v) {
    if constexpr (U16) {
      const float q = __builtin_amdgcn_fmed3f(__builtin_rintf(v), 0.f, 65535.f);
      const unsigned short w = (v != v) ? (unsigned short)0 : (unsigned short)(int)q;
      __builtin_amdgcn_raw_buffer_store_b16(w, rs_out, offo, (uint32_t)plane * out_plane, kNT);
    } else if constexpr (sizeof(OutT) == 4) {
      __builtin_amdgcn_raw_buffer_store_b32(__float_as_uint((float)v), rs_out, offo, (uint32_t)plane * out_plane, kNT);
    } else {
      const unsigned long long b = (unsigned long long)__double_as_longlong((double)v);
      const v2u w = {(unsigned)b, (unsigned)(b >> 32)};
      __builtin_amdgcn_raw_buffer_store_b64(w, rs_out, offo, (uint32_t)plane * out_plane, kNT);
    }
  };

  const int lane_r = min(tid & 63, kMaxReads);
  const int p0 = __builtin_amdgcn_readfirstlane(p_raw) & ~63;
#ifdef WAYNE_TIMING_RAMP_NO_ONCE
  const float t_sky = (interior && do_sky) ? 1.0f + 1e-4f * (float)(p & 255) : 0.f;
  const float t_pfl = 1.0f + 1e-5f * (float)(p & 127);
  float c1 = 0, c2 = 7e-7f + 1e-12f * (float)(p & 63), c3 = 0, c4 = 0;
#else
  const float t_sky = (interior && do_sky) ? a.sky[p] : 0.f;
  const float t_pfl = (interior && gainvar) ? a.pfl[p] : 1.0f;
  float c1 = 0, c2 = 0, c3 = 0, c4 = 0;
  if (do_lin && valid) { c1 = a.lin[0][p]; c2 = a.lin[1][p]; c3 = a.lin[2][p]; c4 = a.lin[3][p]; }
#endif
  const double t_zero = (valid && a.zero_read && (a.flags & (1u << 7))) ? a.zero_read[p] : 0.;
  const int v_bg = __float_as_int(a.bg[lane_r]), v_tab0 = a.tab0[lane_r];
  const int v_lvl = __float_as_int(a.sky_level[lane_r]);
  int bx0 = 0, bx1 = 0, by0 = 0, by1 = 0;
  uint32_t t_seg = 0u;
  if (a.use_box) {
    bx0 = a.box[lane_r][0]; bx1 = a.box[lane_r][1]; by0 = a.box[lane_r][2]; by1 = a.box[lane_r][3];
    if (p0 < S * S) t_seg = a.seg[p0 >> 6];
  }
  constexpr int kTabWords = kMaxReads * kSkyAlias, kTabPer = (kTabWords + kRampThreads - 1) / kRampThreads;
  uint32_t t_tab[ALIAS ? kTabPer : 1];
  if (ALIAS && do_sky) {
#pragma unroll
    for (int i = 0; i < kTabPer; ++i) {
      const int j = tid + i * kRampThreads;
      t_tab[i] = j < kTabWords ? a.sky_alias[j] : 0u;
    }
  }

  const bool ld_dark = do_dark && valid;
  float ds_next = ld_dark ? ld_f32(rs_ds, 0) : 0.f, de_next = ld_dark ? ld_f32(rs_de, 0) : 0.f;

  SeededStream rn, rg;
  if (rdn || do_dark || (ALIAS && do_sky)) rn = SeededStream(a.seed, STAGE_READ, (uint32_t)p, 0u, a.exposure);
  SeededStream& rs = rn;
  if (do_noise) rg = SeededStream(a.seed, STAGE_NOISE, (uint32_t)p, 0u, a.exposure);
  asm volatile("" : "+v"(c1), "+v"(c2), "+v"(c3), "+v"(c4));
  asm volatile("" : "+v"(ds_next), "+v"(de_next));

  if (tid < a.R) {
    s_c[tid] = __int_as_float(v_bg);
    s_tab0[tid] = v_tab0;
  }
  if (ALIAS && do_sky) {
#pragma unroll
    for (int i = 0; i < kTabPer; ++i) {
      const int j = tid + i * kRampThreads;
      if (j < kTabWords) (&s_tab[0][0])[j] = t_tab[i];
    }
  }
  const float skyv = t_sky;
  __syncthreads();
  if (!ALIAS) {
    if (do_sky) sky_counts<FAST>(a, (uint32_t)p, tid, interior && skyv > 0.f, skyv, s_c,
                                 (uint32_t (*)[kRampThreads])&s_tab[0][0]);
    __syncthreads();
  }
  if (!valid) return;
  int sky_lvl = 0;
  float sky_base = __int_as_float(__builtin_amdgcn_readlane(v_lvl, 0));
  if (ALIAS && skyv > 0.f) {
    for (int l = 1; l < a.sky_levels; ++l) {
      const float lv = __int_as_float(__builtin_amdgcn_readlane(v_lvl, l));
      if (lv <= skyv) { sky_lvl += 1; sky_base = lv; }
    }
  }

  const int wy0 = p0 / S, wy1 = min(p0 + 63, S * S - 1) / S, wx0 = p0 - wy0 * S;
  unsigned long long live_bits = ~0ull;
  if (a.use_box) {
    uint32_t cbits = 0u;
    if (p0 < S * S) {
      cbits = __builtin_amdgcn_readfirstlane(t_seg);
      if (cbits != 0u && (tid & 63) == 0) a.seg[p0 >> 6] = 0u;
    }
    const bool rows = wy0 < by1 && wy1 >= by0;
    const bool cols = (wy0 != wy1) || (wx0 < bx1 && wx0 + 64 > bx0);
    live_bits = __ballot((rows && cols) || ((cbits >> lane_r) & 1u) != 0u);
  }
  auto acc_live = [&](int r) -> bool { return ((live_bits >> r) & 1ull) != 0ull; };

  double z = t_zero;
  if (clip) z = fmin(fmax(z, kMinCounts), kMaxCounts);
  if (!interior) z = 0.;
  {
    float zd, zr;
    uint32_t w0, w1;
    rn.next2(w0, w1);
    double v = z;
    if (rdn) { bm_pair<FAST>(w0, w1, zd, zr); v = v + kReadNoise * (double)zr; }
    st_out(0, (ArithT)v);
  }

  const float g32 = 2.35f / t_pfl;
  double inv_g = 1.0 / kGain;
  if (interior && gainvar && !PROD) inv_g = 1.0 / (double)g32;

  float te_s = 0.f, te_f = 0.f, te_0 = 0.f;
  double td_s = 0., td_f = 0.;
  const __amdgpu_buffer_rsrc_t rs_state =
      __builtin_amdgcn_make_buffer_rsrc((void*)th.state, 0, HIST ? (int)(SS * sizeof(float2)) : 0, 0x00020000);
  if constexpr (TRAP) {
    if (interior) {
      v2u st_bits = {0u, 0u};
      if constexpr (HIST) st_bits = __builtin_amdgcn_raw_buffer_load_b64(rs_state, off8, 0, 0);
      long long qs = 0;
      for (int r = 0; r < a.R; ++r)
        if (acc_live(r)) qs += ld_acc(r);
      const float sky_px = skyv > 0.f ? skyv : 0.f;
      if constexpr (PROD) {
        const float e_acc = fmaf((float)(int)(qs >> 32), 16.0f, (float)(uint32_t)qs * 3.725290298461914e-09f);
        const float fbar = fmaf(sky_px, tr.sum_bg_f, e_acc) * tr.inv_sum_dt_f;
        if constexpr (HIST) {
          const float f_gap = th.lit ? fbar : 0.f;
          te_s = trap_step<float>(__uint_as_float(st_bits.x), f_gap, th.gap_f, tr.eta_f[0], tr.eta_n_f[0], tr.inv_tau_f[0]);
          te_f = trap_step<float>(__uint_as_float(st_bits.y), f_gap, th.gap_f, tr.eta_f[1], tr.eta_n_f[1], tr.inv_tau_f[1]);
          te_s = fminf(te_s + th.fill_f[0], th.n_f[0]);
          te_f = fminf(te_f + th.fill_f[1], th.n_f[1]);
        } else {
          te_s = trap_start<float>(tr.start_f, tr, 0, fbar);
          te_f = trap_start<float>(tr.start_f, tr, 1, fbar);
        }
        te_0 = te_s + te_f;
      } else {
        const double fbar = ((double)qs * kInvQ + (double)sky_px * tr.sum_bg) / tr.sum_dt;
        if constexpr (HIST) {
          const double f_gap = th.lit ? fbar : 0.;
          td_s = trap_step<double>((double)__uint_as_float(st_bits.x), f_gap, th.gap_s, tr.eta[0], tr.eta_n[0], tr.inv_tau[0]);
          td_f = trap_step<double>((double)__uint_as_float(st_bits.y), f_gap, th.gap_s, tr.eta[1], tr.eta_n[1], tr.inv_tau[1]);
          td_s = fmin(td_s + th.fill[0], th.n[0]);
          td_f = fmin(td_f + th.fill[1], th.n[1]);
        } else {
          td_s = trap_start<double>(tr.start_d, tr, 0, fbar);
          td_f = trap_start<double>(tr.start_d, tr, 1, fbar);
        }
      }
    }
  }
  auto st_state = [&](float es, float ef) {
    if (interior)
      __builtin_amdgcn_raw_buffer_store_b64(v2u{__float_as_uint(es), __float_as_uint(ef)}, rs_state, off8, 0, 0);
  };

  long long q_next = (interior && acc_live(0)) ? ld_acc(0) : 0;
  double cum = 0.;
  NlState nl = {0.f, 0.f, 0.f};
  float sky_c = -1.f;
  SkyRem srem;
  srem.m = 0.f; srem.t0 = srem.t1 = srem.t2 = srem.t3 = 0xFFFFFFFFu; srem.c3 = 1.f; srem.term3 = 0.f;
  if (PROD) {
    {
      const bool f_dark = ALLON || do_dark, f_lin = ALLON || do_lin, f_clip = ALLON || clip, f_rdn = ALLON || rdn;
      const float inv_gf = !interior ? 0.f : (gainvar ? 1.0f / g32 : (float)(1.0 / kGain));
      const float c1p = (1.0f + c1) - 1.0f;
      const float zf = (float)z;
      const bool has_sky_px = skyv > 0.f;
      uint32_t bg_prev = 0xFFFFFFFFu;
      unsigned long long Q = 0ull;
      int ksum = 0;
      bool q_any = false;
      SkyRem sr;
      sr.m = 0.f; sr.t0 = sr.t1 = sr.t2 = sr.t3 = 0xFFFFFFFFu; sr.c3 = 1.f; sr.term3 = 0.f;
#ifndef WAYNE_RAMP_PF
#define WAYNE_RAMP_PF 2
#endif
      constexpr int PF = WAYNE_RAMP_PF;
      long long qA = q_next, qB = 0, qC = 0;
      float dsA = ds_next, deA = de_next, dsB = 0.f, deB = 0.f, dsC = 0.f, deC = 0.f;
      if (PF == 2 && a.R > 1) {
        if (acc_live(1)) qB = ld_acc(1);
        if (f_dark) { dsB = ld_f32(rs_ds, 1); deB = ld_f32(rs_de, 1); }
      }
      auto step = [&](const int r, const long long q, const float ds, const float de, long long& q_nx, float& ds_nx,
                      float& de_nx) {
        const bool live = acc_live(r);
        if (r + PF < a.R) {
          if (acc_live(r + PF)) q_nx = ld_acc(r + PF);
          if (f_dark) { ds_nx = ld_f32(rs_ds, r + PF); de_nx = ld_f32(rs_de, r + PF); }
        }
        const float bg = __int_as_float(__builtin_amdgcn_readlane(v_bg, r));
        const int tab = __builtin_amdgcn_readlane(v_tab0, r);
        const uint32_t bg_bits = __builtin_amdgcn_readfirstlane(__float_as_uint(bg));
        if (bg_bits != bg_prev) {
          bg_prev = bg_bits;
          sr.set(fmaxf(skyv * bg - sky_base * bg, 0.f));
        }
        float dn = 0.f;
        if (live) {
          if (q != 0) __builtin_amdgcn_raw_buffer_store_b64(v2u{0u, 0u}, rs_acc, off8, (uint32_t)r * acc_plane, 0);
          Q += (unsigned long long)q;
          q_any = true;
          if constexpr (TRAP) dn = fmaf((float)(int)(q >> 32), 16.0f, (float)(uint32_t)q * 3.725290298461914e-09f);
        }
        if constexpr (TRAP) {
          if (has_sky_px && bg > 0.f) {
            const int k_sky = sky_draw_count_int(s_tab[tab + sky_lvl], sr, rn);
            ksum += k_sky;
            dn += (float)k_sky;
          }
        } else {
          if (has_sky_px && bg > 0.f) ksum += sky_draw_count_int(s_tab[tab + sky_lvl], sr, rn);
        }
        float zd = 0.f, zr = 0.f;
        uint32_t w0, w1;
        rn.next2(w0, w1);
        if (f_rdn || f_dark) bm_pair<true>(w0, w1, zd, zr);
        float e = (float)ksum;
        if (q_any) {
          asm volatile("" ::: "memory");
          e = fmaf((float)(int)(Q >> 32), 16.0f, fmaf((float)(uint32_t)Q, 3.725290298461914e-09f, e));
        }
        if constexpr (TRAP) {
          const float f = dn * tr.inv_dt[r], dt = tr.dt[r];
          te_s = trap_step<float>(te_s, f, dt, tr.eta_f[0], tr.eta_n_f[0], tr.inv_tau_f[0]);
          te_f = trap_step<float>(te_f, f, dt, tr.eta_f[1], tr.eta_n_f[1], tr.inv_tau_f[1]);
          e = e - ((te_s + te_f) - te_0);
        }
        float v = e * inv_gf;
        if (f_dark) v = v + fmaf(de, zd, ds);
        if (f_lin) v = nonlinear_gap_f32(v, c1p, c2, c3, c4, nl);
        if (f_clip) v = __builtin_amdgcn_fmed3f(v, (float)kMinCounts, (float)kMaxCounts);
        if (!interior) v = 0.f;
        const float tail = f_rdn ? fmaf((float)kReadNoise, zr, zf) : zf;
        st_out(r + 1, (ArithT)(v + tail));
      };
      int r = 0;
      if (PF == 1) {
        for (; r + 1 < a.R; r += 2) {
          step(r, qA, dsA, deA, qB, dsB, deB);
          step(r + 1, qB, dsB, deB, qA, dsA, deA);
        }
        if (r < a.R) step(r, qA, dsA, deA, qB, dsB, deB);
      } else {
        for (; r + 2 < a.R; r += 3) {
          step(r, qA, dsA, deA, qC, dsC, deC);
          step(r + 1, qB, dsB, deB, qA, dsA, deA);
// ... 25 lines not shown
        const double dt = a.read_dt[r];
        float z0, z1;
        bm_pair<FAST>(g0, g1, z0, z1);
        px = px + (a.noise_mean * dt + (a.noise_std * dt) * (double)z0);
      }
      if (skyv > 0.f) {
        const float lam = skyv * s_c[r];
        if (ALIAS && FAST && SKY == 1) {
          if (s_c[r] != sky_c) {
            sky_c = s_c[r];
            srem.set(fmaxf(lam - sky_base * sky_c, 0.f));
          }
          if constexpr (TRAP) {
            if (lam > 0.f) {
              const double k = (double)sky_draw_count_int(s_tab[s_tab0[r] + sky_lvl], srem, rs);
              px = px + k;
              chg = chg + k;
            }
          } else {
            if (lam > 0.f) px = px + (double)sky_draw_count_int(s_tab[s_tab0[r] + sky_lvl], srem, rs);
          }
        } else if (ALIAS) {
          if (lam > 0.f) {
            const double k = (double)sky_draw<M, SKY == 2>(s_tab[s_tab0[r] + sky_lvl], sky_base * s_c[r], lam, rs);
            px = px + k;
            if constexpr (TRAP) chg = chg + k;
          }
        } else {
          const double k = (double)s_tab[r][tid];
          px = px + k;
          if constexpr (TRAP) chg = chg + k;
        }
      }
      if constexpr (TRAP) {
        const double dt = a.read_dt[r];
        const double es = trap_step<double>(td_s, chg / dt, dt, tr.eta[0], tr.eta_n[0], tr.inv_tau[0]);
        const double ef = trap_step<double>(td_f, chg / dt, dt, tr.eta[1], tr.eta_n[1], tr.inv_tau[1]);
        px = px - ((es + ef) - (td_s + td_f));
        td_s = es;
        td_f = ef;
      }
      px = px * inv_g;
    }
    cum = cum + px;
    double v = cum;
    float zd = 0.f, zr = 0.f;
    uint32_t w0, w1;
    rn.next2(w0, w1);
    if (rdn || ld_dark) bm_pair<FAST>(w0, w1, zd, zr);
    if (interior) {
      if (do_dark) {
        const double err = (de > 0.f) ? (double)de : (double)0.00001f;
        v = v + ((double)ds + err * (double)zd);
      }
      if (do_lin) v = nonlinear_response(v, c1, c2, c3, c4, nl);
      if (clip) v = fmin(fmax(v, kMinCounts), kMaxCounts);
    } else {
      v = 0.;
    }
    v = v + z;
    if (rdn) v = v + kReadNoise * (double)zr;
    st_out(r + 1, (ArithT)v);
  }
  if constexpr (HIST) st_state((float)td_s, (float)td_f);
}

template <class OutT, bool FAST, int SKY, bool NOISE, bool ALLON = false>
__global__ __launch_bounds__(kRampThreads) __attribute__((amdgpu_waves_per_eu(8, 8))) void k_ramp(RampArgs a) {
  ramp_body<OutT, FAST, SKY, NOISE, ALLON>(a);
}
template <class OutT, bool FAST, int SKY, bool NOISE>
__global__ __launch_bounds__(kRampThreads) void k_ramp_wide(RampArgs a) {
  ramp_body<OutT, FAST, SKY, NOISE, false>(a);
}
template <class OutT, bool FAST, int SKY, bool NOISE, bool ALLON>
__global__ __launch_bounds__(kRampThreads) void k_ramp_trap(RampArgs a, TrapArgs t) {
  ramp_body<OutT, FAST, SKY, NOISE, ALLON, true>(a, t);
}
template <class OutT, bool FAST, int SKY, bool NOISE, bool ALLON>
__global__ __launch_bounds__(kRampThreads) void k_ramp_hist(RampArgs a, TrapArgs t, TrapHistArgs h) {
  ramp_body<OutT, FAST, SKY, NOISE, ALLON, true, true>(a, t, h);
}

__global__ __launch_bounds__(256) void k_trap_state_fill(float2* state, int n, float initial_s, float initial_f) {
  const int i = blockIdx.x * blockDim.x + threadIdx.x;
  if (i < n) state[i] = make_float2(initial_s, initial_f);
}

}
```

wayne_amd/csrc/k_throw.h:

```cpp
#pragma once
#include "common.h"
#include "flush_math.h"
#include "k_prep.h"

namespace wayne {

constexpr int kThrowThreads = 512;
constexpr int kThrowPCache = 256;

struct ThrowArgs {
  int W, K, N, S;
  int kb;
  int splits;
  int min_wgs;
  int threads_compat;
  uint32_t seed, exposure, subsample0;
  uint32_t flags;
  int margin, lds_ints;
  int flat_off;
  int off32;
  float lane_reach_sigmas;
  double flat_wmin, flat_wmax, flat_inv_range;
  const SubInfo* sub;
  const uint32_t* prefix;
  const int32_t* nwide;
  const int32_t* nsplit;
  const int32_t* nlane;
  unsigned char chunk_order[kMaxChunks];
  unsigned char lane_order[kMaxChunks];
  const double* xpos;
  const double* ypos;
  const double* sigl;
  const double* sigh;
  const float* flat[4];
  long long* acc;
  int32_t* frame;
};

struct Affine { uint32_t a, c; };
__device__ __forceinline__ uint32_t lcg_jump(uint32_t state, uint64_t n) {
  uint32_t a = 1103515245u, c = 12345u;
  uint32_t ra = 1u, rc = 0u;
  while (n) {
    if (n & 1ull) { ra = ra * a; rc = rc * a + c; }
    c = c * a + c;
    a = a * a;
    n >>= 1;
  }
  return ra * state + rc;
}
__device__ __forceinline__ int rand_r_step(uint32_t& s) {
  uint32_t r;
  s = s * 1103515245u + 12345u; r = (s >> 16) & 2047u;
  s = s * 1103515245u + 12345u; r = (r << 10) ^ ((s >> 16) & 1023u);
  s = s * 1103515245u + 12345u; r = (r << 10) ^ ((s >> 16) & 1023u);
  return (int)r;
}

__device__ __forceinline__ double flat_poly(const ThrowArgs& a, const SubInfo& si, int x, int y, float f0, float f1, float f2, float f3) {
  const int xf = x + a.flat_off, yf = y + a.flat_off;
  const double arr = si.y_ref - (double)yf + si.a_t_i * si.x_ref - si.a_t_i * (double)xf;
  const double d = fabs(arr) * si.inv_norm;
  const double wl = si.a_w * d + si.b_w;
  const double t = (wl - a.flat_wmin) * a.flat_inv_range;
  const double t2 = t * t, t3 = t2 * t;
  const double f = (double)f0 + ((double)f1 * t) + ((double)f2 * t2) +
                   ((double)f3 * t3);
  return (double)(float)f;
}
__device__ __forceinline__ double flat_value(const ThrowArgs& a, const SubInfo& si, int x, int y) {
  const size_t i = (size_t)y * a.N + x;
  return flat_poly(a, si, x, y, a.flat[0][i], a.flat[1][i], a.flat[2][i], a.flat[3][i]);
}

struct ThrowBin {
  float x, y;
  float ch, cl;
  uint32_t bin_end;
  uint32_t wide_end;
  int ox, oy;
};

__device__ __forceinline__ ThrowBin load_throw_bin(const uint32_t* P, const int32_t* NW, const double* XP, const double* YP,
                                                   const double* sigl, const double* sigh, int b) {
  ThrowBin r;
  const BinLocal bl = bin_local(XP[b], YP[b]);
  r.x = bl.fx; r.y = bl.fy; r.ox = bl.ox; r.oy = bl.oy;
  const float sh = (float)sigh[b], sl = (float)sigl[b];
  r.ch = (-1.3862943611198906f * sh) * sh;
  r.cl = (-1.3862943611198906f * sl) * sl;
  const uint32_t start = P[b];
  r.bin_end = P[b + 1];
  r.wide_end = start + min((uint32_t)max(NW[b], 0), r.bin_end - start);
  return r;
}

template <int FLUSH>
__device__ __forceinline__ void deposit_global(const ThrowArgs& a, const SubInfo& si, int x, int y, int n) {
  if (FLUSH == 0) {
    atomicAdd(&a.frame[(size_t)y * a.N + x], n);
  } else {
    double v = (double)n;
    if ((a.flags & 1u) && a.flat[0]) v = v * flat_value(a, si, x, y);
    const long long q = __double2ll_rn(v * kQ);
    atomicAdd((unsigned long long*)&a.acc[((size_t)si.read * a.S + (y + kBorder)) * a.S + (x + kBorder)],
              (unsigned long long)q);
  }
}

template <int FLUSH, bool CLEAR, int T>
__device__ __forceinline__ void flush_tile(const ThrowArgs& a, const SubInfo& si, int* const tile, int tx0, int ty0, int tw, int tarea) {
  const int tid = threadIdx.x;
  if (tarea <= 0) return;
  const FlushWalk w = flush_walk(T, tw, tx0, a.N, a.S);
  FlushCell c = flush_first(tid, tw, tx0, ty0, a.N, a.S, kBorder, kBorder);
  if (!a.off32) {
    for (int i = tid; i < tarea; i += T, flush_next(c, w)) {
      const int m = tile[i];
      if (m > 0) {
// ... 278 lines not shown
```

wayne_amd/csrc/plan_consts.h:

```cpp
#pragma once
#include <math.h>
#include <stdint.h>
#include "philox.h"

namespace wayne {

constexpr int kBorder = 5;

struct GrismDev {
  double trace[9], wlsol[9];
  double p_ratio[4], p_sigl[4], p_sigh[4];
  double flat_wmin, flat_wmax;
  int n_sens;
  const double* sens_wl;
  const double* sens_val;
};

constexpr int kSplitMin = 32;
constexpr int kNarrowR = 6;
constexpr int kLaneMax = 4096;
constexpr int kLaneReach = 64 * kLaneMax;
constexpr uint32_t kSplitMaxNarrow = 1u << 24;

constexpr int kNarrowThreads = 512;
constexpr int kLaneThreads = 512;
constexpr int kMaxChunks = 128;
constexpr int kLaneListCap = 4096;
constexpr int kLaneBatchMax = 32;

constexpr int kSkyAlias = 256;
constexpr float kSkyPiece = 16.f;
constexpr int kMaxReads = 15;

constexpr int kExtractRows = 32;
constexpr int kExtractProducts = kMaxReads + 2;
constexpr int kExtractMaxS = 1024;
constexpr unsigned X_LINEARISE = 1u << 0, X_DARK = 1u << 1, X_GAIN = 1u << 2, X_SKY = 1u << 3, X_LAST_READ = 1u << 4;
constexpr unsigned X_ALL = X_LINEARISE | X_DARK | X_GAIN | X_SKY | X_LAST_READ;
constexpr int kCrMargin = 7;
constexpr int kCrHalo = 2;
constexpr int kCrTileCols = 64, kCrTileRows = kExtractRows;
constexpr int kChanMaxChannels = 256;
constexpr int kChanMaxHull = 384;
constexpr unsigned C_FLAT = 1u << 0, C_ALL = C_FLAT;
constexpr int kOptMaxH = 16;

constexpr int kTrStride = 8;

WAYNE_HD void trace_coeffs(const GrismDev& g, double x_ref, double y_ref, double* o) {
    const double* t = g.trace;
    const double* b = g.wlsol;
    const double m_t = t[3] + t[4] * x_ref + t[5] * y_ref + t[6] * (x_ref * x_ref) +
                       t[7] * x_ref * y_ref + t[8] * (y_ref * y_ref);
    const double c_t = t[0] + t[1] * x_ref + t[2] * y_ref;
    const double m_w = b[3] + b[4] * x_ref + b[5] * y_ref + b[6] * (x_ref * x_ref) +
                       b[7] * x_ref * y_ref + b[8] * (y_ref * y_ref);
    const double c_w = (b[0] + b[1] * x_ref) + b[2] * y_ref;
    const double xa = x_ref + 10, xb = x_ref + 20;
    const double ya = m_t * (xa - x_ref) + c_t + y_ref;
    const double yb = m_t * (xb - x_ref) + c_t + y_ref;
    const double da = sqrt((ya - y_ref) * (ya - y_ref) + (xa - x_ref) * (xa - x_ref));
    const double db = sqrt((yb - y_ref) * (yb - y_ref) + (xb - x_ref) * (xb - x_ref));
    const double wa_ = (m_w * da + c_w) * 1e-4;
    const double wb_ = (m_w * db + c_w) * 1e-4;
    const double m_wl = (wb_ - wa_) / (xb - xa);
    const double c_wl = wa_ - m_wl * xa;
    o[0] = m_t; o[1] = c_t; o[2] = m_w; o[3] = c_w; o[4] = m_wl; o[5] = c_wl;
}

}
```

wayne_amd/csrc/wayne_hip.hip:

```cpp
#include "../../include/wayne_hip.h"

#include <hip/hip_runtime.h>
#include <hip/hip_ext.h>

#include <algorithm>
#include <chrono>
#include <cmath>
#include <cstdio>
#include <cstdlib>
#include <cstring>
#include <limits>
#include <map>
#include <new>
#include <string>
#include <type_traits>
#include <vector>

#include "kernels.h"
#include "host_plan.h"

using namespace wayne;

struct wayne_ctx;

// ... 27 lines not shown
  hipError_t reserve(size_t bytes) {
    if (!owns) { p = nullptr; cap = 0; owns = true; }
    if (bytes <= cap) return hipSuccess;
    if (p) (void)hipFree(p);
    p = nullptr;
    cap = 0;
    if (bytes == 0) return hipSuccess;
    hipError_t e = hipMalloc(&p, bytes);
    if (e == hipSuccess) cap = bytes;
    return e;
  }
  void view(void* at) {
    if (owns && p) (void)hipFree(p);
    p = at;
    cap = 0;
    owns = false;
  }
  template <class T> T* as() const { return (T*)p; }
};

struct PinnedBuf {
  char* p = nullptr;
  size_t cap = 0;
  PinnedBuf() = default;
  PinnedBuf(const PinnedBuf&) = delete;
  PinnedBuf& operator=(const PinnedBuf&) = delete;
  ~PinnedBuf() { if (p) (void)hipHostFree(p); }
  bool reserve(size_t bytes) {
    if (bytes <= cap) return true;
    if (p) (void)hipHostFree(p);
    p = nullptr;
    cap = 0;
    if (hipHostMalloc((void**)&p, bytes, hipHostMallocDefault) != hipSuccess) { p = nullptr; return false; }
    cap = bytes;
    return true;
  }
};

struct StageArena {
  PinnedBuf host;
  DevBuf dev;
  hipEvent_t ev = nullptr;
  bool pending = false;
  size_t used = 0;
  ~StageArena() { if (ev) (void)hipEventDestroy(ev); }
  int begin(wayne_ctx* c, size_t bytes, const char* nomem_msg, bool with_event = true) {
    if (pending) { HIP_TRY(c, hipEventSynchronize(ev)); pending = false; }
    if (!host.reserve(align64(bytes))) return fail(c, WAYNE_E_NOMEM, nomem_msg);
    if (with_event && !ev) HIP_TRY(c, hipEventCreateWithFlags(&ev, hipEventDisableTiming));
    HIP_TRY(c, dev.reserve(host.cap));
    used = 0;
    return WAYNE_OK;
  }
  char* place(DevBuf& view, size_t bytes) {
    bytes = std::max<size_t>(bytes, 1);
    if (used + bytes > host.cap) return nullptr;
    char* h = host.p + used;
    view.view((char*)dev.p + used);
    used += align64(bytes);
    return h;
  }
  bool put(DevBuf& view, const void* src, size_t bytes) {
    char* h = place(view, bytes);
    if (h && bytes) std::memcpy(h, src, bytes);
    return h != nullptr;
  }
  int commit(wayne_ctx* c, hipStream_t stream) {
    HIP_TRY(c, hipMemcpyAsync(dev.p, host.p, used, hipMemcpyHostToDevice, stream));
    if (ev) { HIP_TRY(c, hipEventRecord(ev, stream)); pending = true; }
    return WAYNE_OK;
  }
  template <class T> const T* host_of(const DevBuf& view) const { return (const T*)(host.p + ((const char*)view.p - (const char*)dev.p)); }
};

struct SourceState {
  bool fused_last = false;
  PrepArgs last_prep{};
  int last_chunks = 0;
  int W = 0;
  uint32_t seed = 0;
  DevBuf wl, flux, xref, yref;
  DevBuf ratio, sigl, sigh, sens, dlam;
  DevBuf counts, nwide, nsplit, nlane, prefix, xpos, ypos, sub, chunk_total, chunk_box;
  DevBuf tr;
  int kb = 1;
  bool thin = false;
  double max_narrow = 0.;
  double max_chunk_electrons = 0.;
  double est_thrown = 0.;
  unsigned char chunk_order[kMaxChunks] = {0};
  unsigned char lane_order[kMaxChunks] = {0};
  StageArena src_stage;
  plan::WlCache wl_cache;
};

constexpr int kMaxSources = WAYNE_MAX_SOURCES;

struct Slot : SourceState {
  bool uploaded = false;
  bool front_done = false;
  bool acc_dirty = false;
  bool acc_init = false;
  bool force_throw = false;
  bool ran = false;
  uint32_t run_no = 0, pinned_run = 0, ex_pinned_run = 0;
  wayne_exposure_desc d{};
  int K = 0, R = 0;
  bool has_depth = false, has_replay_seed = false, has_lc = false, has_lc_hidden = false;
  DevBuf depth, dur, rseed, sread, read_dt, lc_z, lc_hidden, lc_rp;
  int n_extra = 0;
  SourceState extra[kMaxSources];
  uint32_t extra_tag[kMaxSources] = {0};
  SourceState& source(int i) { return i == 0 ? *this : extra[i - 1]; }
  DevBuf acc, out, misc;
  DevBuf seg;
  bool use_box = false;
  int acc_box[16][4] = {{0}};
  PinnedBuf pinned;
  struct Misc {
    unsigned long long spare;
    uint32_t over_run, beyond_run;
    int bits(uint32_t run) const { return (run && over_run == run ? 1 : 0) | (run && beyond_run == run ? 2 : 0); }
  };
  Misc* pinned_misc = nullptr;
  StageArena sky_stage;
  DevBuf sky_tab;
  std::vector<uint32_t> sky_tab_keys;
  bool sky_alias_on = false, sky_pieces = false;
  uint32_t sky_mask = 0;
  int sky_L = 1;
  float sky_level[16] = {0};
  unsigned char sky_tab0[16] = {0};
  std::vector<double> read_dt_host;
  double lc_p_lo = 0., lc_p_hi = 0.;
  bool ld_on = false;
  StageArena ld_stage;
  DevBuf ld_tab;
  bool spots_on = false;
  StageArena spot_stage;
  DevBuf spot_contrast, spot_px, spot_py, spot_ld;
  SpotArgs spot_args{};
  bool traps_on = false;
  double trap_n[2] = {1., 1.}, trap_eta[2] = {0., 0.}, trap_tau[2] = {1., 1.}, trap_lo = 0., trap_hi = 0.;
  int trap_G = 0;
  StageArena trap_stage;
  DevBuf trap_d, trap_f;
  bool hist_on = false;
  double hist_gap = 0., hist_fill[2] = {0., 0.};
  int hist_lit = 0;
  bool extract_on = false;
  wayne_extract_desc ex{};
  int ex_chunks = 0;
  DevBuf ex_part, ex_out;
  plan::SpectraLayout lay;
  PinnedBuf ex_pinned;
  Misc* ex_pinned_misc = nullptr;
  const char* ex_base = nullptr;
  std::vector<double> ex_host;
  bool crrej_on = false;
  double cr_k = 0., cr_rn = 0.;
  int cr_lo = 0, cr_hi = 0;
  DevBuf cr_mask, ex_part_n;
  bool chan_on = false;
  int ch_C = 0, ch_lo = 0, ch_hi = 0;
  uint32_t ch_flags = 0;
  StageArena ch_stage;
  DevBuf ch_edges, ch_wa, ch_wb, ch_part;
  bool var_on = false;
  double var_rn = 0.;
  DevBuf ex_part_v, ch_part_v;
  bool opt_on = false;
  int opt_H = 0;
  DevBuf opt_part;
  bool prof_deliver = false, prof_valid = false, prof_fetched = false;
  DevBuf prof_planes;
  PinnedBuf prof_pinned;
  bool prof_fixed = false;
  int prof_rows[kExtractProducts] = {0};
  DevBuf prof_fix;
  bool optch_on = false;
  DevBuf optch_part;
  bool prof_fix_valid = false;
  size_t prof_fix_n = 0;
  uint64_t prof_fix_hash = 0;
  int prof_fix_R = 0;
  bool fits_on = false;
  size_t fits_plane_bytes = 0, fits_stride = 0;
  DevBuf fits_dev;
  PinnedBuf fits_pinned;
  Misc* fits_pinned_misc = nullptr;
  uint32_t fits_pinned_run = 0;
  int expect_mode = 0;
  DevBuf expect_plane;
  bool rampfit_on = false, rampfit_ran = false;
  wayne_rampfit_desc rampfit{};
  DevBuf rampfit_planes;
  bool ima_on = false, ima_ran = false;
  wayne_ima_desc ima{};
  size_t ima_sci_stride = 0, ima_dq_stride = 0, ima_imset_stride = 0;
  DevBuf ima_dev;
  bool ipc_on = false, ipc_front = false, b_dirty = false;
  int ipc_w[9] = {0};
  DevBuf acc_b, seg_b;
  StageArena stage;
};

struct ProfRec {
  int kernel;
  hipEvent_t a, b;
};

constexpr int kSlots = 256;

}

constexpr int kStreams = 2;

struct Knobs {
  long long tile_ints = -1;
  long long batch = -1;
  long long thin = -1;
  long long no_acc_box = -1;
  long long lane_reach = -1;
  long long throw_wgs = -1;
  long long keep_narrow = -1;
  long long no_fuse = -1;
  long long fork_narrow = -1;
  long long streams = -1;
  long long upload_timing = -1;
  long long narrow_compact = -1;
  long long prep_wl_per_run = -1;
  long long fuse_thrower = -1;
  long long lane_tight_tile = -1;
  long long ramp_reads = -1;
};
struct KnobName { const char* name; const char* env; long long Knobs::*field; };
const KnobName kKnobNames[] = {
    {"tile_ints", "WAYNE_TILE_INTS", &Knobs::tile_ints},       {"batch", "WAYNE_BATCH", &Knobs::batch},
    {"thin", "WAYNE_THIN", &Knobs::thin},                      {"no_acc_box", "WAYNE_NO_ACC_BOX", &Knobs::no_acc_box},
    {"lane_reach", "WAYNE_LANE_REACH", &Knobs::lane_reach},    {"throw_wgs", "WAYNE_THROW_WGS", &Knobs::throw_wgs},
    {"keep_narrow", "WAYNE_KEEP_NARROW", &Knobs::keep_narrow}, {"no_fuse", "WAYNE_NO_FUSE", &Knobs::no_fuse},
    {"fork_narrow", "WAYNE_FORK_NARROW", &Knobs::fork_narrow}, {"streams", "WAYNE_STREAMS", &Knobs::streams},
    {"upload_timing", "WAYNE_UPLOAD_TIMING", &Knobs::upload_timing}, {"ramp_reads", "WAYNE_RAMP_READS", &Knobs::ramp_reads},
    {"narrow_compact", "WAYNE_NARROW_COMPACT", &Knobs::narrow_compact},
    {"lane_tight_tile", "WAYNE_LANE_TIGHT_TILE", &Knobs::lane_tight_tile},
    {"fuse_thrower", "WAYNE_FUSE_THROWER", &Knobs::fuse_thrower},
    {"prep_wl_per_run", "WAYNE_PREP_WL_PER_RUN", &Knobs::prep_wl_per_run},
};
constexpr size_t kMiscBytes = 64;

constexpr size_t kCounterBytes = (size_t)kCounterStripes * kCounterStride * sizeof(unsigned long long);

struct CtxStreams {
  hipStream_t stream = nullptr;
  hipStream_t streams[kStreams] = {nullptr, nullptr};
  hipStream_t side[kStreams] = {nullptr, nullptr};
  hipEvent_t ev_fork[kStreams] = {nullptr, nullptr}, ev_join[kStreams] = {nullptr, nullptr};
  bool fork_narrow = true;
  hipEvent_t ev_kdone[kStreams] = {nullptr, nullptr};
  bool kdone_valid[kStreams] = {false, false};
  hipEvent_t ev_trap_chain = nullptr;
  bool trap_chain_valid = false;
  ~CtxStreams() {
    if (ev_trap_chain) (void)hipEventDestroy(ev_trap_chain);
    for (int i = 0; i < kStreams; ++i) {
      if (streams[i]) (void)hipStreamDestroy(streams[i]);
      if (side[i]) (void)hipStreamDestroy(side[i]);
      if (ev_fork[i]) (void)hipEventDestroy(ev_fork[i]);
      if (ev_join[i]) (void)hipEventDestroy(ev_join[i]);
      if (ev_kdone[i]) (void)hipEventDestroy(ev_kdone[i]);
    }
  }
};

struct wayne_ctx : CtxStreams {
  int device = 0;
  int n_streams = kStreams;
  Knobs knobs;
  DevBuf status_all;
  PinnedBuf status_host;
  std::string err;
  bool have_grism = false;
  unsigned long long grism_gen = 1;
  GrismDev g{};
  DevBuf sens_wl, sens_val;
  plan::SpectrumEstimate est;
  plan::SpectrumEstimate src_est[kMaxSources];
  bool have_cal = false;
  int subarray = 0, N = 0, S = 0, cal_R = 0;
  DevBuf flat[4], pfl, sky, lin[4], dark_sci, dark_err, zero_read;
  bool has_flat = false, has_pfl = false, has_sky = false, has_lin = false, has_dark = false,
       has_zero = false;
  float sky_max = 0.f, sky_min = 0.f;
  std::vector<float> sky_sorted;
  double up_us[6] = {0, 0, 0, 0, 0, 0};
  long up_calls = 0;
  Slot slots[kSlots];
  DevBuf pa_prefix, pa_nwide, pa_nsplit, pa_nlane, pa_x, pa_y, pa_sl, pa_sh, pa_sub, pa_frame;
  StageArena pa_stage;
  bool prof_on = false;
  unsigned prof_mask = ~0u;
  std::vector<ProfRec> prof;
  std::vector<hipEvent_t> ev_pool;
  uint64_t prof_launches[kProfKernels] = {0};
  double prof_ms[kProfKernels] = {0};
  uint64_t electrons = 0;
  uint64_t profile_uploads = 0;
  DevBuf trap_state;
  bool trap_state_valid = false;
  uint64_t reruns = 0;
  DevBuf counters;
};

namespace {

void plan_lanes(const wayne_ctx* c, SourceState& ss, int K, int W) {
  int kb = 1;
  plan::lane_batches(K, W, ss.max_chunk_electrons, &kb, &ss.thin);
  {
    if (c->knobs.batch >= 0) kb = (int)std::min<long long>(std::max<long long>(c->knobs.batch, 1), kLaneBatchMax);
    if (c->knobs.thin >= 0) ss.thin = c->knobs.thin != 0;
  }
  ss.kb = kb;
}

int reserve_source(wayne_ctx* c, SourceState& ss, int K, int W) {
  const size_t KW = (size_t)K * W, n_chunks = (size_t)(W + kPrepThreads - 1) / kPrepThreads;
  for (DevBuf* b : {&ss.ratio, &ss.sigl, &ss.sigh, &ss.sens, &ss.dlam}) HIP_TRY(c, b->reserve((size_t)W * sizeof(double)));
  for (DevBuf* b : {&ss.counts, &ss.nwide, &ss.nsplit, &ss.nlane}) HIP_TRY(c, b->reserve(KW * sizeof(int32_t)));
  HIP_TRY(c, ss.prefix.reserve((size_t)K * (W + 1) * sizeof(uint32_t)));
  HIP_TRY(c, ss.xpos.reserve(KW * sizeof(double)));
  HIP_TRY(c, ss.ypos.reserve(KW * sizeof(double)));
  HIP_TRY(c, ss.sub.reserve((size_t)K * sizeof(SubInfo)));
  HIP_TRY(c, ss.chunk_total.reserve(K * n_chunks * sizeof(uint32_t)));
  HIP_TRY(c, ss.chunk_box.reserve(K * n_chunks * 4 * sizeof(double)));
  return WAYNE_OK;
}

void adopt_plan(const wayne_ctx* c, SourceState& ss, int K, int W, const plan::ThrowPlan& tp) {
  ss.est_thrown = tp.est_thrown; ss.max_chunk_electrons = tp.max_chunk_electrons; ss.max_narrow = tp.max_narrow;
  std::memcpy(ss.chunk_order, tp.chunk_order, sizeof ss.chunk_order);
  std::memcpy(ss.lane_order, tp.lane_order, sizeof ss.lane_order);
  plan_lanes(c, ss, K, W);
}

int fail(wayne_ctx* c, int code, const std::string& msg) {
  if (c) c->err = msg;
  return code;
}

hipEvent_t get_event(wayne_ctx* c) {
  if (!c->ev_pool.empty()) {
    hipEvent_t e = c->ev_pool.back();
    c->ev_pool.pop_back();
    return e;
  }
  hipEvent_t e = nullptr;
  if (hipEventCreate(&e) != hipSuccess) return nullptr;
  return e;
}

struct ProfScope {
  wayne_ctx* c;
  ProfRec rec{};
  bool on;
  bool ext = false;
  ProfScope(wayne_ctx* c_, int kernel, bool ext_launch = false) : c(c_), on(c_->prof_on && ((c_->prof_mask >> kernel) & 1u)) {
    if (!on) return;
    rec.kernel = kernel;
    rec.a = get_event(c);
    rec.b = get_event(c);
    if (!rec.a || !rec.b) { on = false; return; }
    ext = ext_launch;
    if (!ext) (void)hipEventRecord(rec.a, c->stream);
  }
  ~ProfScope() {
    if (!on) return;
    if (!ext) (void)hipEventRecord(rec.b, c->stream);
    c->prof.push_back(rec);
  }
};

int sync_all(wayne_ctx* c) {
  for (int i = 0; i < kStreams; ++i) {
    HIP_TRY(c, hipStreamSynchronize(c->streams[i]));
    if (c->side[i]) HIP_TRY(c, hipStreamSynchronize(c->side[i]));
  }
  return WAYNE_OK;
}

void use_slot_stream(wayne_ctx* c, int slot) { c->stream = c->streams[slot % c->n_streams]; }

int collect_profile(wayne_ctx* c) {
  int rc = sync_all(c);
  if (rc) return rc;
  for (ProfRec& r : c->prof) {
    float ms = 0.f;
    if (hipEventElapsedTime(&ms, r.a, r.b) == hipSuccess) {
      c->prof_ms[r.kernel] += ms;
      c->prof_launches[r.kernel] += 1;
    }
    c->ev_pool.push_back(r.a);
    c->ev_pool.push_back(r.b);
  }
  c->prof.clear();
  return WAYNE_OK;
}

template <class T>
int upload(wayne_ctx* c, DevBuf& b, const T* src, size_t n) {
  HIP_TRY(c, b.reserve(std::max<size_t>(n, 1) * sizeof(T)));
  if (n) HIP_TRY(c, hipMemcpyAsync(b.p, src, n * sizeof(T), hipMemcpyHostToDevice, c->stream));
  return WAYNE_OK;
}

using plan::build_sky_alias;

template <class T>
// ... 812 lines not shown
    a.frame = c->pa_frame.as<int32_t>();
    if ((size + kNarrowThreads - 1) / kNarrowThreads > kMaxChunks && (any_lane || any_split))
      return fail(c, WAYNE_E_INVALID, "psf_apply: more than 65536 bins in split mode");
    for (int i = 0; i < kMaxChunks; ++i) a.chunk_order[i] = a.lane_order[i] = (unsigned char)i;
    if (run > 0) {
      ProfScope ps(c, PK_THROW);
      rc = (rng_mode == WAYNE_RNG_REPLAY) ? launch_throw<0, 0>(c, a, lds_ints) : launch_throw<1, 0>(c, a, lds_ints);
      if (rc) return rc;
    }
    const bool exact = (flags & WAYNE_F_EXACT_SAMPLERS) != 0;
    if (any_lane && any_split && fuse_thrower(c, a, false, exact)) {
      ProfScope ps_throw(c, PK_THROW);
      ProfScope ps(c, PK_LANE);
      if ((rc = launch_thrower<0>(c, a))) return rc;
    } else {
      if (any_lane) {
        ProfScope ps(c, PK_LANE);
        if ((rc = launch_lane<0>(c, a, false))) return rc;
      }
      if (any_split) {
        ProfScope ps(c, PK_NARROW);
        if ((rc = launch_narrow<0>(c, a, exact))) return rc;
      }
    }
    c->electrons += (uint64_t)total;
  }
  HIP_TRY(c, hipMemcpyAsync(out, c->pa_frame.p, (size_t)N * N * sizeof(int32_t), hipMemcpyDeviceToHost,
                            c->stream));
  HIP_TRY(c, hipStreamSynchronize(c->stream));
  return WAYNE_OK;
}

int wayne_ctx_set_grism(wayne_ctx* c, const wayne_grism_desc* g) {
  if (!c || !g) return WAYNE_E_INVALID;
  if (g->n_sens < 0 || (g->n_sens > 0 && (!g->sens_wl_um || !g->sens_val)))
    return fail(c, WAYNE_E_INVALID, "set_grism: sensitivity table");
  if (!plan::sens_table_ok(g->sens_wl_um, g->sens_val, g->n_sens))
    return fail(c, WAYNE_E_INVALID, "set_grism: sensitivity table must have finite values at finite, non-decreasing wavelengths");
  (void)hipSetDevice(c->device);
  c->stream = c->streams[0];
  int rc;
  if ((rc = upload(c, c->sens_wl, g->sens_wl_um, (size_t)g->n_sens))) return rc;
  if ((rc = upload(c, c->sens_val, g->sens_val, (size_t)g->n_sens))) return rc;
  HIP_TRY(c, hipStreamSynchronize(c->stream));
  GrismDev& d = c->g;
  std::memcpy(d.trace, g->trace_coeff, sizeof d.trace);
  std::memcpy(d.wlsol, g->wl_solution, sizeof d.wlsol);
  std::memcpy(d.p_ratio, g->psf_ratio_poly, sizeof d.p_ratio);
  std::memcpy(d.p_sigl, g->psf_sigmal_poly, sizeof d.p_sigl);
  std::memcpy(d.p_sigh, g->psf_sigmah_poly, sizeof d.p_sigh);
  d.flat_wmin = g->flat_wmin;
  d.flat_wmax = g->flat_wmax;
  d.n_sens = g->n_sens;
  d.sens_wl = c->sens_wl.as<double>();
  d.sens_val = c->sens_val.as<double>();
  c->have_grism = true;
  c->grism_gen += 1;
  c->est.set_grism(d, g->sens_wl_um, g->sens_val, g->n_sens);
  for (plan::SpectrumEstimate& e : c->src_est) e.set_grism(d, g->sens_wl_um, g->sens_val, g->n_sens);
  return WAYNE_OK;
}

int wayne_ctx_set_calibration(wayne_ctx* c, const wayne_calibration* k) {
  if (!c || !k) return WAYNE_E_INVALID;
  const int sub = k->subarray;
  if (sub != 64 && sub != 128 && sub != 256 && sub != 512 && sub != 1024)
    return fail(c, WAYNE_E_INVALID, "set_calibration: SUBARRAY must be 64,128,256,512 or 1024");
  if (k->n_reads < 1 || k->n_reads > kMaxReads) return fail(c, WAYNE_E_INVALID, "set_calibration: n_reads must be 1..15");
  (void)hipSetDevice(c->device);
  { int rc0 = sync_all(c); if (rc0) return rc0; }
  c->stream = c->streams[0];
  const int N = side_of(sub), S = N + 2 * kBorder;
  const size_t NN = (size_t)N * N, SS = (size_t)S * S;
  int rc;
  if (c->have_cal && S != c->S) c->trap_state_valid = false;
  c->has_flat = k->flat[0] && k->flat[1] && k->flat[2] && k->flat[3];
  if (c->has_flat)
    for (int i = 0; i < 4; ++i)
      if ((rc = upload(c, c->flat[i], k->flat[i], NN))) return rc;
  c->has_pfl = k->pfl != nullptr;
  if (c->has_pfl) {
    std::vector<float> v = embed(k->pfl, N, S, 1.0f);
    if ((rc = upload(c, c->pfl, v.data(), SS))) return rc;
    HIP_TRY(c, hipStreamSynchronize(c->stream));
  }
  c->has_sky = k->sky != nullptr;
  c->sky_max = 0.f;
  c->sky_min = 0.f;
  if (c->has_sky) {
    c->sky_sorted.clear();
    for (size_t i = 0; i < NN; ++i)
      if (k->sky[i] > 0.f) c->sky_sorted.push_back(k->sky[i]);
    std::sort(c->sky_sorted.begin(), c->sky_sorted.end());
    if (!c->sky_sorted.empty()) { c->sky_min = c->sky_sorted.front(); c->sky_max = c->sky_sorted.back(); }
    std::vector<float> v = embed(k->sky, N, S, 0.0f);
    if ((rc = upload(c, c->sky, v.data(), SS))) return rc;
    HIP_TRY(c, hipStreamSynchronize(c->stream));
  }
  c->has_lin = k->lin[0] && k->lin[1] && k->lin[2] && k->lin[3];
  if (c->has_lin)
    for (int i = 0; i < 4; ++i)
      if ((rc = upload(c, c->lin[i], k->lin[i], SS))) return rc;
  c->has_dark = k->dark_sci && k->dark_err;
  if (c->has_dark) {
    if ((rc = upload(c, c->dark_sci, k->dark_sci, SS * k->n_reads))) return rc;
    {
      std::vector<float> e(k->dark_err, k->dark_err + SS * k->n_reads);
      for (float& x : e) if (!(x > 0.f)) x = 0.00001f;
      if ((rc = upload(c, c->dark_err, e.data(), e.size()))) return rc;
      HIP_TRY(c, hipStreamSynchronize(c->stream));
    }
  }
  c->has_zero = k->zero_read != nullptr;
  if (c->has_zero)
    if ((rc = upload(c, c->zero_read, k->zero_read, SS))) return rc;
  HIP_TRY(c, hipStreamSynchronize(c->stream));
  c->subarray = sub; c->N = N; c->S = S; c->cal_R = k->n_reads;
  c->have_cal = true;
  c->grism_gen += 1;
  for (Slot& s : c->slots) { s.uploaded = false; s.acc_init = false; }
  return WAYNE_OK;
}

int wayne_exposure_upload(wayne_ctx* c, int slot, const wayne_exposure_desc* d) {
  if (!c || !d) return WAYNE_E_INVALID;
  if (slot < 0 || slot >= kSlots) return fail(c, WAYNE_E_INVALID, "upload: slot");
  if (!c->have_grism || !c->have_cal) return fail(c, WAYNE_E_STATE, "upload: set grism and calibration first");
  const int W = d->n_wl, K = d->n_samples, R = d->n_reads;
  if (W < 2 || K < 1 || R < 1) return fail(c, WAYNE_E_INVALID, "upload: need n_wl >= 2, n_samples >= 1, n_reads >= 1");
  if (R != c->cal_R) return fail(c, WAYNE_E_INVALID, "upload: n_reads differs from the calibration's");
  if (!d->wl_um || !d->flux || !d->x_ref || !d->y_ref || !d->dur_ms || !d->sample_read || !d->read_dt_s)
    return fail(c, WAYNE_E_INVALID, "upload: null array");
  if (d->rng_mode != WAYNE_RNG_REPLAY && d->rng_mode != WAYNE_RNG_PHILOX && d->rng_mode != WAYNE_RNG_SPLIT)
    return fail(c, WAYNE_E_INVALID, "upload: rng_mode");
  if ((d->flags & WAYNE_F_OUT_F64) && (d->flags & WAYNE_F_OUT_U16))
    return fail(c, WAYNE_E_INVALID, "upload: WAYNE_F_OUT_F64 and WAYNE_F_OUT_U16 are mutually exclusive");
  if (d->rng_mode == WAYNE_RNG_REPLAY && (d->threads_compat <= 0 || !d->replay_seed))
    return fail(c, WAYNE_E_INVALID, "upload: replay mode needs threads_compat >= 1 and replay_seed");
  for (int k = 0; k < K; ++k)
    if (d->sample_read[k] < 0 || d->sample_read[k] >= R) return fail(c, WAYNE_E_INVALID, "upload: sample_read out of range");
  if ((long long)K * W > 0x7FFFFFFFLL) return fail(c, WAYNE_E_INVALID, "upload: K*W too large");
  (void)hipSetDevice(c->device);
  use_slot_stream(c, slot);
  Slot& s = c->slots[slot];
  const auto t_up0 = std::chrono::steady_clock::now();
  auto lap = [&](int part, std::chrono::steady_clock::time_point& t_) {
    const auto now = std::chrono::steady_clock::now();
    c->up_us[part] += std::chrono::duration<double, std::micro>(now - t_).count();
    t_ = now;
  };
  auto t_lap = t_up0;
  s.uploaded = false;
  s.front_done = false;
  s.fused_last = false;
  s.n_extra = 0;
  s.traps_on = false;
  s.hist_on = false;
  ex_clear(s);
  s.fits_on = false;
  s.fits_pinned_misc = nullptr;
  s.expect_mode = 0;
  s.rampfit_on = s.rampfit_ran = false;
  s.ima_on = s.ima_ran = false;
  s.ld_on = false;
  s.ipc_on = false;
  s.spots_on = false;
// ... 66 lines not shown
  s.read_dt_host.assign(d->read_dt_s, d->read_dt_s + R);
  lap(0, t_lap);
  {
    plan::ThrowPlan tp;
    plan::estimate_thrown(c->est, W, d->wl_um, d->flux, K, d->dur_ms, d->scale_factor, d->rng_mode, &tp);
    adopt_plan(c, s, K, W, tp);
  }
  lap(1, t_lap);
  s.use_box = plan::accumulator_boxes(c->est, W, d->wl_um, d->flux, K, R, c->S, d->sub_scale, d->x_ref, d->y_ref,
                                      d->sample_read, s.acc_box) && !(c->knobs.no_acc_box > 0);
  lap(2, t_lap);
  {
    const size_t seg_bytes = ((SS + 63) / 64) * sizeof(uint32_t);
    if (s.seg.cap < seg_bytes) {
      HIP_TRY(c, s.seg.reserve(seg_bytes));
      HIP_TRY(c, hipMemsetAsync(s.seg.p, 0, s.seg.cap, c->stream));
    }
  }
  if ((rc = prepare_sky_tables(c, s))) return rc;
  lap(3, t_lap);
  c->up_calls += 1;
  s.force_throw = false;
  s.uploaded = true;
  s.front_done = false;
  return WAYNE_OK;
}

static int front_source(wayne_ctx* c, int slot, Slot& s, SourceState& ss, int src) {
  const wayne_exposure_desc& d = s.d;
  const int W = ss.W, K = s.K, R = s.R, N = c->N, S = c->S;
  WlArrays wa{ss.ratio.as<double>(), ss.sigl.as<double>(), ss.sigh.as<double>(), ss.sens.as<double>(),
              ss.dlam.as<double>()};
  if (c->knobs.prep_wl_per_run > 0 || ss.wl_cache.gen != c->grism_gen) {
    ProfScope ps(c, PK_PREP_WL);
    hipLaunchKernelGGL(k_prep_wl_run, dim3((std::max(W, K) + 255) / 256), dim3(256), 0, c->stream, c->g, W,
                       ss.wl.as<double>(), wa, src == 0 ? s.misc.as<uint32_t>() : nullptr, K, ss.xref.as<double>(), ss.yref.as<double>(),
                       ss.tr.as<double>());
    HIP_TRY(c, hipGetLastError());
    if (ss.wl_cache.valid) ss.wl_cache.gen = c->grism_gen;
  }
  bool skip_narrow = false;
  bool lane_unlimited = false;
  bool fused = false;
  const bool force_throw = s.force_throw || (s.traps_on && s.hist_on);
  const int margin = d.thrower_margin > 0 ? d.thrower_margin : 30;
  PrepArgs prep_args{};
  CosmicArgs cosmic_args{};
  {
    PrepArgs& a = prep_args;
    a.g = c->g;
    a.W = W; a.K = K; a.N = N;
    a.sub_scale = d.sub_scale;
    a.margin = margin;
    a.max_tile = 0x7FFFFFFF;
    a.seed = ss.seed; a.exposure = d.exposure_index; a.flags = d.flags;
    a.scale_factor = d.scale_factor;
    a.wl = ss.wl.as<double>(); a.flux = ss.flux.as<double>();
    a.depth = (src == 0 && s.has_depth) ? s.depth.as<double>() : nullptr;
    a.x_ref = ss.xref.as<double>(); a.y_ref = ss.yref.as<double>(); a.dur_ms = s.dur.as<double>();
    a.replay_seed = s.has_replay_seed ? s.rseed.as<int32_t>() : nullptr;
    a.sample_read = s.sread.as<int32_t>();
    a.tr = ss.tr.as<double>();
    a.wa = wa;
    a.counts = ss.counts.as<int32_t>(); a.nwide = ss.nwide.as<int32_t>();
    a.nsplit = ss.nsplit.as<int32_t>();
    a.nlane = ss.nlane.as<int32_t>();
    a.split_min = (d.rng_mode == WAYNE_RNG_SPLIT) ? kSplitMin : 0;
    int reach = kLaneReach;
    if (c->knobs.lane_reach >= 0) reach = (int)std::min<long long>(std::max<long long>(c->knobs.lane_reach, 1), kLaneReach);
    lane_unlimited = d.rng_mode == WAYNE_RNG_SPLIT && ss.est_thrown <= 0. && d.thrower_splits <= 0 && !force_throw &&
                     c->knobs.throw_wgs < 0;
    a.lane_max = lane_unlimited ? reach : kLaneMax;
    a.prefix = ss.prefix.as<uint32_t>(); a.xpos = ss.xpos.as<double>(); a.ypos = ss.ypos.as<double>();
    a.sub = ss.sub.as<SubInfo>();
    a.total_electrons = c->counters.as<unsigned long long>();
    a.status = (uint32_t*)(s.misc.as<char>() + 8);
    a.run = s.run_no;
    const int n_chunks = (W + kPrepThreads - 1) / kPrepThreads;
    a.chunk_total = ss.chunk_total.as<uint32_t>();
    a.chunk_box = ss.chunk_box.as<double>();
    a.fix_inline = lane_unlimited ? 1 : 0;
    skip_narrow = lane_unlimited && ss.max_narrow <= 6. && !(c->knobs.keep_narrow > 0);
    a.no_narrow = skip_narrow ? 1 : 0;
    CosmicArgs& ca = cosmic_args;
    ca.R = R; ca.N = N; ca.S = S; ca.seed = ss.seed; ca.exposure = d.exposure_index;
    ca.rate = (src == 0 && d.cosmic_rate >= 0.) ? d.cosmic_rate : -1.;
    ca.read_dt = s.read_dt.as<double>(); ca.acc = s.acc.as<long long>();
    ca.seg = s.seg.as<uint32_t>();
    fused = lane_unlimited && skip_narrow && ss.thin && !(c->knobs.no_fuse > 0);
    ss.fused_last = fused;
    ss.last_prep = a;
    ss.last_chunks = n_chunks;
    if (!fused) {
      ProfScope ps(c, PK_PREP_SUB);
      hipLaunchKernelGGL(k_prep_sub, dim3(K, n_chunks), dim3(kPrepThreads), 0, c->stream, a, ca);
      HIP_TRY(c, hipGetLastError());
      if (!a.fix_inline) {
        hipLaunchKernelGGL(k_prep_fix, dim3(K), dim3(kPrepThreads), 0, c->stream, a, n_chunks);
        HIP_TRY(c, hipGetLastError());
      }
    }
  }
  {
    ThrowArgs a{};
    a.W = W; a.K = K; a.N = N; a.S = S;
    a.off32 = offsets_fit_32(N, S) ? 1 : 0;
    a.kb = ss.kb;
    a.lane_reach_sigmas = lane_reach_sigmas(c);
    const int min_wgs = 1024;
    int splits = d.thrower_splits;
    if (splits <= 0) {
      if (c->knobs.throw_wgs >= 0) {
        splits = (int)std::max<long long>(1, (std::max<long long>(c->knobs.throw_wgs, 1) + K - 1) / K);
      } else {
        const double unit = (d.rng_mode == WAYNE_RNG_REPLAY) ? 1. : (double)kThrowBlock;
        const double lanes = 1.08 * ss.est_thrown / unit;
        splits = (int)std::min(4096., std::ceil(lanes / kThrowThreads));
        if (d.rng_mode == WAYNE_RNG_SPLIT && ss.est_thrown <= 0. && !force_throw) splits = -1;
        const int cap = std::max(1, (3072 + K - 1) / K);
        if (splits > 2 * cap) splits = cap;
        splits = splits < 0 ? 1 : std::max(splits, (min_wgs + K - 1) / K);
      }
    }
    a.min_wgs = min_wgs;
    a.splits = std::min(splits, 4096);
    a.margin = margin;
    const int lds_ints = thrower_lds_ints(c, a.splits, margin);
    a.lds_ints = lds_ints;
    a.threads_compat = d.threads_compat;
    a.seed = ss.seed; a.exposure = d.exposure_index; a.subsample0 = 0;
    a.flags = d.flags;
    a.flat_off = d.sub_scale;
    a.flat_wmin = c->g.flat_wmin; a.flat_wmax = c->g.flat_wmax;
    a.flat_inv_range = 1.0 / (c->g.flat_wmax - c->g.flat_wmin);
    a.sub = ss.sub.as<SubInfo>(); a.prefix = ss.prefix.as<uint32_t>(); a.nwide = ss.nwide.as<int32_t>();
    a.nsplit = ss.nsplit.as<int32_t>();
    a.nlane = ss.nlane.as<int32_t>();
    std::memcpy(a.chunk_order, ss.chunk_order, sizeof a.chunk_order);
    std::memcpy(a.lane_order, ss.lane_order, sizeof a.lane_order);
    a.xpos = ss.xpos.as<double>(); a.ypos = ss.ypos.as<double>();
    a.sigl = ss.sigl.as<double>(); a.sigh = ss.sigh.as<double>();
    for (int i = 0; i < 4; ++i) a.flat[i] = c->has_flat ? c->flat[i].as<float>() : nullptr;
    a.acc = s.acc.as<long long>();
    a.frame = nullptr;
    if ((d.flags & WAYNE_F_ADD_FLAT) && !c->has_flat) return fail(c, WAYNE_E_STATE, "run: add_flat without a flat cube");
    const int si_ = slot % c->n_streams;
    const bool fork = d.rng_mode == WAYNE_RNG_SPLIT && c->fork_narrow && !skip_narrow;
    const bool one_grid = d.rng_mode == WAYNE_RNG_SPLIT && !skip_narrow && !fork && !fused &&
                          fuse_thrower(c, a, ss.thin, (d.flags & WAYNE_F_EXACT_SAMPLERS) != 0);
    hipStream_t main_stream = c->stream;
    {
      ProfScope ps_throw(c, PK_THROW);
      if (fork) {
        HIP_TRY(c, hipEventRecord(c->ev_fork[si_], main_stream));
        HIP_TRY(c, hipStreamWaitEvent(c->side[si_], c->ev_fork[si_], 0));
        c->stream = c->side[si_];
        int rc;
        {
          ProfScope ps(c, PK_NARROW);
          rc = launch_narrow<1>(c, a, (d.flags & WAYNE_F_EXACT_SAMPLERS) != 0);
        }
        if (rc == WAYNE_OK && hipEventRecord(c->ev_join[si_], c->side[si_]) != hipSuccess)
          rc = fail(c, WAYNE_E_HIP, "run: event record on the side stream");
        c->stream = main_stream;
        if (rc) return rc;
      }
      int rc = lane_unlimited ? (int)WAYNE_OK
               : (d.rng_mode == WAYNE_RNG_REPLAY) ? launch_throw<0, 1>(c, a, lds_ints) : launch_throw<1, 1>(c, a, lds_ints);
      if (rc) return rc;
      if (d.rng_mode == WAYNE_RNG_SPLIT) {
        ProfScope ps(c, PK_LANE);
        if ((rc = one_grid ? launch_thrower<1>(c, a)
                  : fused  ? launch_lane<1>(c, a, true, &prep_args, &cosmic_args) : launch_lane<1>(c, a, ss.thin))) return rc;
      }
      if (fork) HIP_TRY(c, hipStreamWaitEvent(main_stream, c->ev_join[si_], 0));
    }
    if (!fork && !one_grid && d.rng_mode == WAYNE_RNG_SPLIT && !skip_narrow) {
      ProfScope ps(c, PK_NARROW);
      int rc = launch_narrow<1>(c, a, (d.flags & WAYNE_F_EXACT_SAMPLERS) != 0);
      if (rc) return rc;
    }
  }
  return WAYNE_OK;
}

static void ipc_dilate(const int (*box)[4], int S, int (*out)[4]) {
  for (int r = 0; r < 16; ++r) {
    const int* b = box[r];
    if (box_empty(b)) { std::memcpy(out[r], b, sizeof(int) * 4); continue; }
    out[r][0] = std::max(b[0] - 1, 0); out[r][1] = std::min(b[1] + 1, S);
    out[r][2] = std::max(b[2] - 1, 0); out[r][3] = std::min(b[3] + 1, S);
  }
}

static int launch_ipc(wayne_ctx* c, Slot& s) {
  const int S = c->S;
  IpcArgs a{};
  a.R = s.R; a.S = S;
  a.use_box = s.use_box ? 1 : 0;
  std::memcpy(a.w, s.ipc_w, sizeof a.w);
  a.a = s.acc.as<long long>(); a.b = s.acc_b.as<long long>();
  a.seg_a = s.seg.as<uint32_t>(); a.seg_b = s.seg_b.as<uint32_t>();
  const unsigned blocks = (unsigned)(((size_t)S * S + kIpcThreads - 1) / kIpcThreads);
  ProfScope ps(c, PK_IPC);
  ipc_dilate(s.acc_box, S, a.box);
  hipLaunchKernelGGL(k_ipc, dim3(blocks), dim3(kIpcThreads), 0, c->stream, a);
  HIP_TRY(c, hipGetLastError());
  std::memcpy(a.box, s.acc_box, sizeof a.box);
  hipLaunchKernelGGL(k_ipc_clear, dim3(blocks), dim3(kIpcThreads), 0, c->stream, a);
  HIP_TRY(c, hipGetLastError());
  return WAYNE_OK;
}

static void lc_rule(float* x, float* w, float* d) {
  const double h = 6.0 / (kLcNodes - 1);
  for (int i = 0; i < kLcNodes; ++i) {
    const double t = -3.0 + h * i, u = 0.5 * kPi * std::sinh(t);
    x[i] = (float)(0.5 * (1.0 + std::tanh(u)));
    w[i] = (float)(h * 0.25 * kPi * std::cosh(t) / (std::cosh(u) * std::cosh(u)));
    d[i] = (float)(0.5 * std::exp(-std::fabs(u)) / std::cosh(u));
  }
}

int wayne_exposure_run_front(wayne_ctx* c, int slot) {
  if (!c) return WAYNE_E_INVALID;
  if (slot < 0 || slot >= kSlots) return fail(c, WAYNE_E_INVALID, "run: slot");
  Slot& s = c->slots[slot];
// ... 26 lines not shown
    LcLdArgs a{};
    a.K = K; a.W = W;
    a.z = s.lc_z.as<double>();
    a.hidden = s.has_lc_hidden ? s.lc_hidden.as<double>() : nullptr;
    a.rp = s.lc_rp.as<double>();
    a.ld = s.ld_tab.as<double>();
    lc_rule(a.x, a.w, a.d);
    a.p_lo = s.lc_p_lo; a.p_hi = s.lc_p_hi;
    a.depth = s.depth.as<double>();
    ProfScope ps(c, PK_LIGHTCURVE);
    hipLaunchKernelGGL(k_lightcurve_ld, dim3(K), dim3(256), 0, c->stream, a);
    HIP_TRY(c, hipGetLastError());
  } else if (s.has_lc) {
    LcArgs a{};
    a.K = K; a.W = W;
    a.z = s.lc_z.as<double>();
    a.hidden = s.has_lc_hidden ? s.lc_hidden.as<double>() : nullptr;
    a.rp = s.lc_rp.as<double>();
    double sum = 0.;
    for (int i = 0; i < 4; ++i) { a.ld[i] = d.lc_ld[i]; sum += d.lc_ld[i] * (i + 1) / (i + 5.0); }
    a.f0 = kPi * (1.0 - sum);
    lc_rule(a.x, a.w, a.d);
    a.p_lo = s.lc_p_lo; a.p_hi = s.lc_p_hi;
    a.depth = s.depth.as<double>();
    ProfScope ps(c, PK_LIGHTCURVE);
    hipLaunchKernelGGL(k_lightcurve, dim3(K), dim3(256), 0, c->stream, a);
    HIP_TRY(c, hipGetLastError());
  }
  if (s.has_lc && s.spots_on) {
    SpotArgs a = s.spot_args;
    a.K = K; a.W = W;
    a.z = s.lc_z.as<double>();
    a.hidden = s.has_lc_hidden ? s.lc_hidden.as<double>() : nullptr;
    a.rp = s.lc_rp.as<double>();
    a.px = s.spot_px.as<double>(); a.py = s.spot_py.as<double>();
    a.contrast = s.spot_contrast.as<double>();
    if (s.ld_on) { a.ld = s.ld_tab.as<double>(); a.ld_plane = (size_t)W; a.ld_step = 1; }
    else         { a.ld = s.spot_ld.as<double>(); a.ld_plane = 1; a.ld_step = 0; }
    a.depth = s.depth.as<double>();
    ProfScope ps(c, PK_SPOTS);
    hipLaunchKernelGGL(k_lightcurve_spots, dim3(K, (W + 255) / 256), dim3(256), 0, c->stream, a);
    HIP_TRY(c, hipGetLastError());
  }

  if (s.run_no == 0xFFFFFFFFu) {
    HIP_TRY(c, hipMemsetAsync(s.misc.p, 0, kMiscBytes, c->stream));
    s.run_no = 0;
  }
  s.run_no += 1;
  for (int i = 0; i <= s.n_extra; ++i) {
    int rc = front_source(c, slot, s, s.source(i), i);
    if (rc) return rc;
  }
  s.acc_dirty = true;
  s.ipc_front = s.ipc_on;
  if (s.ipc_on) {
    s.b_dirty = true;
    if (int rc = launch_ipc(c, s)) return rc;
  }
  s.front_done = true;
  return WAYNE_OK;
}

int wayne_exposure_run_back(wayne_ctx* c, int slot) {
  if (!c) return WAYNE_E_INVALID;
  if (slot < 0 || slot >= kSlots) return fail(c, WAYNE_E_INVALID, "run: slot");
  Slot& s = c->slots[slot];
  if (!s.uploaded || !s.front_done) return fail(c, WAYNE_E_STATE, "run_back: run_front first");
  (void)hipSetDevice(c->device);
  use_slot_stream(c, slot);
  const wayne_exposure_desc& d = s.d;
  const int S = c->S;
  RampArgs a{};
  a.R = s.R; a.N = c->N; a.S = S;
#ifdef WAYNE_TIMING_KNOBS
  bool ramp_reads_cut = false;
  if (c->knobs.ramp_reads >= 0) { a.R = (int)std::max<long long>(1, std::min<long long>(s.R, c->knobs.ramp_reads)); ramp_reads_cut = a.R < s.R; }
#endif
  a.seed = d.seed; a.exposure = d.exposure_index; a.flags = d.flags;
  a.sky_ct_s = d.sky_ct_s; a.noise_mean = d.noise_mean; a.noise_std = d.noise_std;
  a.read_dt = s.read_dt.as<double>();
  a.acc = s.acc.as<long long>();
  a.pfl = c->has_pfl ? c->pfl.as<float>() : nullptr;
  a.sky = c->has_sky ? c->sky.as<float>() : nullptr;
  for (int i = 0; i < 4; ++i) a.lin[i] = c->has_lin ? c->lin[i].as<float>() : nullptr;
  a.dark_sci = c->has_dark ? c->dark_sci.as<float>() : nullptr;
  a.dark_err = c->has_dark ? c->dark_err.as<float>() : nullptr;
  a.zero_read = c->has_zero ? c->zero_read.as<double>() : nullptr;
  a.out = s.out.p;
  if ((d.flags & WAYNE_F_ADD_GAIN_VARIATIONS) && !c->has_pfl) return fail(c, WAYNE_E_STATE, "run: add_gain_variations without a pixel flat");
  if ((d.flags & WAYNE_F_ADD_NON_LINEAR) && !c->has_lin) return fail(c, WAYNE_E_STATE, "run: add_non_linear without coefficient planes");
  if (d.sky_ct_s > 0. && !c->has_sky) return fail(c, WAYNE_E_STATE, "run: sky background without a master sky");
  a.sky_alias = s.sky_alias_on ? s.sky_tab.as<uint32_t>() : nullptr;
  a.alias_mask = s.sky_alias_on ? s.sky_mask : 0u;
  a.sky_levels = s.sky_L;
  for (int l = 0; l < 16; ++l) { a.sky_level[l] = s.sky_level[l]; a.sky_tab0[l] = s.sky_tab0[l]; a.tab0[l] = s.sky_tab0[l]; a.bg[l] = 0.f; }
  for (int r = 0; r < s.R && r < 16; ++r) a.bg[r] = (float)(d.sky_ct_s * s.read_dt_host[r]);
  a.use_box = s.use_box ? 1 : 0;
  std::memcpy(a.box, s.acc_box, sizeof a.box);
  a.seg = s.seg.as<uint32_t>();
  if (s.ipc_front) {
    a.acc = s.acc_b.as<long long>();
    ipc_dilate(s.acc_box, S, a.box);
    a.seg = s.seg_b.as<uint32_t>();
  }
  const int threads = kRampThreads;
  const unsigned blocks = (unsigned)(((size_t)S * S + threads - 1) / threads);
  if (s.traps_on && s.hist_on && (!c->trap_state_valid || !c->ev_trap_chain))
    return fail(c, WAYNE_E_STATE, "run: a trap history without a trap state (wayne_ctx_trap_state_reset / _upload first)");
  {
    ProfScope ps(c, PK_RAMP, true);
    RampTrapKernel trap = nullptr;
    RampHistKernel hist = nullptr;
    void (*kern)(RampArgs) = select_ramp(c, s, nullptr, &trap, &hist);
    if (trap || hist) {
      TrapArgs t{};
      t.G = s.trap_G;
      t.start_d = s.trap_d.as<double>();
      t.start_f = s.trap_f.as<float>();
      t.rate_lo = s.trap_lo;
      t.ln_lo = std::log(s.trap_lo);
      t.u_scale = s.trap_G > 2 ? (double)(s.trap_G - 2) / std::log(s.trap_hi / s.trap_lo) : 0.;
      for (int p = 0; p < 2; ++p) {
        t.eta[p] = s.trap_eta[p];
        t.eta_n[p] = s.trap_eta[p] / s.trap_n[p];
        t.inv_tau[p] = 1.0 / s.trap_tau[p];
        t.eta_f[p] = (float)t.eta[p]; t.eta_n_f[p] = (float)t.eta_n[p]; t.inv_tau_f[p] = (float)t.inv_tau[p];
      }
      for (int r = 0; r < s.R && r < 16; ++r) {
        t.sum_dt += s.read_dt_host[r];
        t.sum_bg += (double)a.bg[r];
        t.dt[r] = (float)s.read_dt_host[r];
        t.inv_dt[r] = (float)(1.0 / s.read_dt_host[r]);
      }
      t.inv_sum_dt_f = (float)(1.0 / t.sum_dt);
      t.sum_bg_f = (float)t.sum_bg;
      if (hist) {
        TrapHistArgs h{};
        h.state = c->trap_state.as<float2>();
        h.gap_s = s.hist_gap; h.gap_f = (float)s.hist_gap;
        h.lit = s.hist_lit;
        for (int p = 0; p < 2; ++p) {
          h.fill[p] = s.hist_fill[p]; h.fill_f[p] = (float)s.hist_fill[p];
          h.n[p] = s.trap_n[p]; h.n_f[p] = (float)s.trap_n[p];
        }
        if (c->trap_chain_valid) HIP_TRY(c, hipStreamWaitEvent(c->stream, c->ev_trap_chain, 0));
        if (ps.on) hipExtLaunchKernelGGL(hist, dim3(blocks), dim3(threads), 0, c->stream, ps.rec.a, ps.rec.b, 0, a, t, h);
        else hipLaunchKernelGGL(hist, dim3(blocks), dim3(threads), 0, c->stream, a, t, h);
        HIP_TRY(c, hipEventRecord(c->ev_trap_chain, c->stream));
        c->trap_chain_valid = true;
      } else if (ps.on) hipExtLaunchKernelGGL(trap, dim3(blocks), dim3(threads), 0, c->stream, ps.rec.a, ps.rec.b, 0, a, t);
      else hipLaunchKernelGGL(trap, dim3(blocks), dim3(threads), 0, c->stream, a, t);
    } else {
      if (ps.on) hipExtLaunchKernelGGL(kern, dim3(blocks), dim3(threads), 0, c->stream, ps.rec.a, ps.rec.b, 0, a);
      else hipLaunchKernelGGL(kern, dim3(blocks), dim3(threads), 0, c->stream, a);
    }
    HIP_TRY(c, hipGetLastError());
  }
  if (s.extract_on)
    if (int rc = launch_extract(c, s)) return rc;
  if (s.fits_on)
    if (int rc = launch_fits(c, s)) return rc;
  if (s.rampfit_on)
    if (int rc = launch_rampfit(c, s)) return rc;
  if (s.ima_on)
    if (int rc = launch_ima(c, s)) return rc;
// ... 90 lines not shown
  HIP_TRY(c, hipMemcpyAsync(s.pinned_misc, s.misc.p, sizeof(Slot::Misc), hipMemcpyDeviceToHost, c->stream));
  s.pinned_run = s.run_no;
  return WAYNE_OK;
}

int wayne_exposure_wait(wayne_ctx* c, int slot, void** host_reads) {
  if (!c || !host_reads) return WAYNE_E_INVALID;
  if (slot < 0 || slot >= kSlots) return fail(c, WAYNE_E_INVALID, "wait: slot");
  Slot& s = c->slots[slot];
  if (!s.uploaded || !s.pinned.p || !s.pinned_misc) return fail(c, WAYNE_E_STATE, "wait: fetch_async first");
  (void)hipSetDevice(c->device);
  use_slot_stream(c, slot);
  HIP_TRY(c, hipStreamSynchronize(c->stream));
  *host_reads = s.pinned.p;
  bool reran = false;
  int rc = look_at_status(c, slot, s.pinned_misc, wayne_exposure_run, &reran, s.pinned_run);
  if (rc || !reran) return rc;
  if ((rc = wayne_exposure_fetch_async(c, slot))) return rc;
  if (s.extract_on && s.ex_pinned_misc && (rc = wayne_exposure_fetch_spectra_async(c, slot))) return rc;
  if (s.fits_on && s.fits_pinned_misc && (rc = wayne_exposure_fetch_fits_async(c, slot))) return rc;
  HIP_TRY(c, hipStreamSynchronize(c->stream));
  return look_at_status(c, slot, s.pinned_misc, nullptr, nullptr, s.pinned_run);
}

void* wayne_exposure_device_reads(wayne_ctx* c, int slot) {
  if (!c || slot < 0 || slot >= kSlots) return nullptr;
  return c->slots[slot].out.p;
}

int wayne_exposure_synthesize(wayne_ctx* c, const wayne_exposure_desc* d, void* out_reads) {
  int rc = wayne_exposure_upload(c, 0, d);
  if (rc) return rc;
  if ((rc = wayne_exposure_run(c, 0))) return rc;
  return wayne_exposure_download(c, 0, out_reads);
}

static int fetch_source(wayne_ctx* c, int slot, int src, int32_t* counts, double* x_pos, double* y_pos, double* acc_e) {
  if (!c) return WAYNE_E_INVALID;
  if (slot < 0 || slot >= kSlots) return fail(c, WAYNE_E_INVALID, "debug_fetch: slot");
  Slot& s = c->slots[slot];
  if (!s.uploaded) return fail(c, WAYNE_E_STATE, "debug_fetch: slot not uploaded");
  if (src < 0 || src > s.n_extra) return fail(c, WAYNE_E_INVALID, "debug_fetch: no such source in this slot");
  SourceState& ss = s.source(src);
  (void)hipSetDevice(c->device);
  use_slot_stream(c, slot);
  const size_t KW = (size_t)s.K * ss.W;
  if (counts) HIP_TRY(c, hipMemcpyAsync(counts, ss.counts.p, KW * sizeof(int32_t), hipMemcpyDeviceToHost, c->stream));
  if (ss.fused_last && (x_pos || y_pos)) {
    PrepArgs a = ss.last_prep;
    a.total_electrons = c->counters.as<unsigned long long>() + 1;
    CosmicArgs off{};
    off.rate = -1.;
    hipLaunchKernelGGL(k_prep_sub, dim3(s.K, ss.last_chunks), dim3(kPrepThreads), 0, c->stream, a, off);
    HIP_TRY(c, hipGetLastError());
  }
  if (x_pos) HIP_TRY(c, hipMemcpyAsync(x_pos, ss.xpos.p, KW * sizeof(double), hipMemcpyDeviceToHost, c->stream));
  if (y_pos) HIP_TRY(c, hipMemcpyAsync(y_pos, ss.ypos.p, KW * sizeof(double), hipMemcpyDeviceToHost, c->stream));
  {
    bool reran = false;
    int rc = look_at_status(c, slot, nullptr, s.front_done ? wayne_exposure_run_front : nullptr, &reran);
    if (rc) return rc;
    if (reran) return fetch_source(c, slot, src, counts, x_pos, y_pos, acc_e);
  }
  if (acc_e) {
    const size_t n = (size_t)s.R * c->S * c->S;
    std::vector<long long> tmp(n);
    const void* from = (s.front_done && s.ipc_front) ? s.acc_b.p : s.acc.p;
    HIP_TRY(c, hipMemcpyAsync(tmp.data(), from, n * sizeof(long long), hipMemcpyDeviceToHost, c->stream));
    HIP_TRY(c, hipStreamSynchronize(c->stream));
    for (size_t i = 0; i < n; ++i) acc_e[i] = (double)tmp[i] * kInvQ;
  }
  return look_at_status(c, slot, nullptr);
}

int wayne_exposure_debug_fetch(wayne_ctx* c, int slot, int32_t* counts, double* x_pos, double* y_pos,
                               double* acc_e) {
  return fetch_source(c, slot, 0, counts, x_pos, y_pos, acc_e);
}

int wayne_exposure_debug_fetch_source(wayne_ctx* c, int slot, int source, int32_t* counts, double* x_pos, double* y_pos) {
  return fetch_source(c, slot, source, counts, x_pos, y_pos, nullptr);
}

int wayne_exposure_debug_boxes(wayne_ctx* c, int slot, int32_t* boxes, int32_t* segments, int* use_box) {
  if (!c || !boxes || !segments || !use_box) return WAYNE_E_INVALID;
  if (slot < 0 || slot >= kSlots) return fail(c, WAYNE_E_INVALID, "debug_boxes: slot");
  Slot& s = c->slots[slot];
  if (!s.uploaded) return fail(c, WAYNE_E_STATE, "debug_boxes: slot not uploaded");
  *use_box = s.use_box ? 1 : 0;
  const int S = c->S;
  int box[16][4];
  std::memcpy(box, s.acc_box, sizeof box);
  if (s.ipc_on) ipc_dilate(s.acc_box, S, box);
  for (int r = 0; r < 16; ++r) {
    for (int i = 0; i < 4; ++i) boxes[4 * r + i] = s.use_box ? box[r][i] : 0;
    int n = 0;
    if (r < s.R) {
      for (int p0 = 0; p0 < S * S; p0 += 64) {
        const int wy0 = p0 / S, wy1 = std::min(p0 + 63, S * S - 1) / S, wx0 = p0 - wy0 * S;
        const int* b = box[r];
        const bool rows = wy0 < b[3] && wy1 >= b[2];
        const bool cols = (wy0 != wy1) || (wx0 < b[1] && wx0 + 64 > b[0]);
        n += (!s.use_box || (rows && cols)) ? 1 : 0;
      }
    }
    segments[r] = n;
  }
  return WAYNE_OK;
}

int wayne_exposure_debug_depth(wayne_ctx* c, int slot, double* depth) {
  if (!c || !depth) return WAYNE_E_INVALID;
  if (slot < 0 || slot >= kSlots) return fail(c, WAYNE_E_INVALID, "debug_depth: slot");
  Slot& s = c->slots[slot];
  if (!s.uploaded || !s.has_depth) return fail(c, WAYNE_E_STATE, "debug_depth: no depth matrix in this slot");
  (void)hipSetDevice(c->device);
  use_slot_stream(c, slot);
  HIP_TRY(c, hipMemcpyAsync(depth, s.depth.p, (size_t)s.K * s.W * sizeof(double), hipMemcpyDeviceToHost, c->stream));
  HIP_TRY(c, hipStreamSynchronize(c->stream));
  return WAYNE_OK;
}


int wayne_exposure_set_sources(wayne_ctx* c, int slot, const wayne_source_desc* src, int n) {
  if (!c) return WAYNE_E_INVALID;
  if (slot < 0 || slot >= kSlots) return fail(c, WAYNE_E_INVALID, "set_sources: slot");
  Slot& s = c->slots[slot];
  if (!s.uploaded) return fail(c, WAYNE_E_STATE, "set_sources: slot not uploaded");
  if (n < 0 || n > kMaxSources) return fail(c, WAYNE_E_INVALID, "set_sources: n must be 0 .. WAYNE_MAX_SOURCES");
  if (n > 0 && !src) return fail(c, WAYNE_E_INVALID, "set_sources: null list");
  if (n > 0 && s.d.rng_mode == WAYNE_RNG_REPLAY)
    return fail(c, WAYNE_E_INVALID, "set_sources: replay mode reproduces the reference, which has no second star");
  const int K = s.K, R = s.R;
  for (int i = 0; i < n; ++i) {
    const wayne_source_desc& q = src[i];
    if (q.tag == 0) return fail(c, WAYNE_E_INVALID, "set_sources: tag 0 is the target's");
    for (int j = 0; j < i; ++j)
      if (src[j].tag == q.tag) return fail(c, WAYNE_E_INVALID, "set_sources: duplicate tag");
    if (q.n_wl < 2 || q.n_wl > 32768) return fail(c, WAYNE_E_INVALID, "set_sources: n_wl must be 2 .. 32768");
    if ((long long)K * q.n_wl > 0x7FFFFFFFLL) return fail(c, WAYNE_E_INVALID, "set_sources: K*W too large");
    if (!q.wl_um || !q.flux) return fail(c, WAYNE_E_INVALID, "set_sources: null array");
    if (!std::isfinite(q.dx) || !std::isfinite(q.dy)) return fail(c, WAYNE_E_INVALID, "set_sources: offset not finite");
  }
  (void)hipSetDevice(c->device);
  use_slot_stream(c, slot);
  s.n_extra = 0;
  s.front_done = false;
  const double* x0 = s.stage.host_of<double>(s.xref);
  const double* y0 = s.stage.host_of<double>(s.yref);
  const double* dur = s.stage.host_of<double>(s.dur);
  const int32_t* sread = s.stage.host_of<int32_t>(s.sread);
  const bool no_box = c->knobs.no_acc_box > 0;
  s.use_box = plan::accumulator_boxes(c->est, s.W, s.stage.host_of<double>(s.wl), s.stage.host_of<double>(s.flux), K, R, c->S,
                                      s.d.sub_scale, x0, y0, sread, s.acc_box) && !no_box;
  if (n == 0) return WAYNE_OK;
  bool use_box = s.use_box;
  int box[16][4];
  std::memcpy(box, s.acc_box, sizeof box);
  for (int i = 0; i < n; ++i) {
    const wayne_source_desc& q = src[i];
    SourceState& e = s.extra[i];
    const int W = q.n_wl;
    StageArena& st = e.src_stage;
    int rc = st.begin(c, 2 * align64((size_t)W * 8) + 2 * align64((size_t)K * 8) + align64((size_t)K * kTrStride * 8) + 256,
                      "set_sources: pinned staging allocation failed");
    if (rc) return rc;
// ... 974 lines not shown
```

wayne_amd/synthetic.py:

```python
import numpy as np

from . import tools

H_C_OVER_K = 1.438776877e4


def wavelength_grid():
    return np.sort(1.0 / (0.5 + 1e-4 * np.arange(15000)))


def blackbody_shape(wl_um, T=6100.0):
    wl = np.asarray(wl_um, dtype=float)
    return 1.0 / (wl ** 5 * (np.exp(H_C_OVER_K / (wl * T)) - 1.0))


def depth_spectrum(wl_um):
    wl = np.asarray(wl_um, dtype=float)
    return 0.0146 + 2e-4 * np.sin(2 * np.pi * (wl - 1.1) / 0.3)


def transit_shape(t_days, mid=0.0, full_width=0.125, ingress=0.02):
    t = np.abs(np.asarray(t_days, dtype=float) - mid)
    half = full_width / 2.
    g = np.where(t <= half - ingress, 1.0, 0.0)
    edge = (t > half - ingress) & (t < half)
    g = np.where(edge, 0.5 * (1 + np.cos(np.pi * (t - (half - ingress)) / ingress)), g)
    return g


def sample_times(read_times_s, K_per_read=None, sample_rate_ms=None):
    read_ms = np.asarray(read_times_s, dtype=float) * 1000.
    if sample_rate_ms is not None:
        starts, idx, i, prev = [], [], -1, 0.
        for rt in read_ms:
            s = np.arange(prev, rt, sample_rate_ms)
            starts.append(s)
            i += len(s)
            idx.append(i)
            prev = rt
        starts = np.concatenate(starts)
        ends = np.roll(starts, -1)
        ends[-1] = read_ms[-1]
    else:
        starts, ends, idx, prev, i = [], [], [], 0., -1
        for rt, n in zip(read_ms, K_per_read):
            e = np.linspace(prev, rt, n + 1)
            starts.append(e[:-1])
            ends.append(e[1:])
            i += n
            idx.append(i)
            prev = rt
        starts, ends = np.concatenate(starts), np.concatenate(ends)
    durs = ends - starts
    return starts + durs / 2., durs, idx


def distribute_samples(read_times_s, K):
    dt = np.diff(np.concatenate([[0.], np.asarray(read_times_s, dtype=float)]))
    R = len(dt)
    if K < R:
        raise ValueError("need at least one sub-sample per read")
    n = np.ones(R, dtype=int)
    rest = K - R
    share = dt / dt.sum() * rest
    n += np.floor(share).astype(int)
    for j in np.argsort(-(share - np.floor(share)))[:K - n.sum()]:
        n[j] += 1
    return n


CONFIGS = {
    "cfg1": dict(grism="G141", SUBARRAY=256, SAMPSEQ="SPARS10", NSAMP=5, E=2.5e7, scan_speed=7.4325,
                 x_ref=404.0, y_ref=457.3 - 70.0, sample_rate=10.0, ssv=(1.5, 1.1, 0.0), cosmic_rate=11.0),
    "cfg2": dict(grism="G141", SUBARRAY=1024, SAMPSEQ="SPARS10", NSAMP=16, K=15, E=2.5e7, scan_speed=0.0,
                 x_ref=404.5 + 379, y_ref=500.0),
    "cfg3": dict(grism="G141", SUBARRAY=256, SAMPSEQ="SPARS10", NSAMP=15, K=64, E=4e8, scan_speed=1.6,
                 x_ref=404.5, y_ref=457.4 - 75.0),
    "cfg4": dict(grism="G141", SUBARRAY=1024, SAMPSEQ="SPARS10", NSAMP=16, K=128, E=1e9, scan_speed=5.0,
                 x_ref=404.5 + 379, y_ref=80.0),
    "cfg5": dict(grism="G141", SUBARRAY=1024, SAMPSEQ="SPARS10", NSAMP=16, K=128, E=1e9, scan_speed=5.0,
                 x_ref=404.5 + 379, y_ref=80.0, ssv=(1.5, 1.1, 0.0), cosmic_rate=11.0),
    "cfg5_g102": dict(grism="G102", SUBARRAY=1024, SAMPSEQ="SPARS10", NSAMP=16, K=128, E=1e9, scan_speed=5.0,
                      x_ref=404.5 + 379, y_ref=80.0, ssv=(1.5, 1.1, 0.0), cosmic_rate=11.0),
    "tiny": dict(grism="G141", SUBARRAY=64, SAMPSEQ="RAPID", NSAMP=4, K=6, E=3e4, scan_speed=40.0,
                 x_ref=440.0, y_ref=490.0, n_wl=600),
    "tiny_g102": dict(grism="G102", SUBARRAY=64, SAMPSEQ="RAPID", NSAMP=3, K=4, E=2e4, scan_speed=25.0,
                      x_ref=455.0, y_ref=492.0, n_wl=500),
    "tiny128": dict(grism="G141", SUBARRAY=128, SAMPSEQ="RAPID", NSAMP=5, K=8, E=1e5, scan_speed=60.0,
                    x_ref=400.0, y_ref=460.0, n_wl=900),
    "tiny512": dict(grism="G141", SUBARRAY=512, SAMPSEQ="RAPID", NSAMP=3, K=5, E=3e5, scan_speed=8.0,
                    x_ref=330.0, y_ref=420.0, n_wl=1500),
    "ramp16_128": dict(grism="G141", SUBARRAY=128, SAMPSEQ="RAPID", NSAMP=16, K=30, E=3e5, scan_speed=45.0,
                       x_ref=400.0, y_ref=460.0, n_wl=900),
    "stare256": dict(grism="G141", SUBARRAY=256, SAMPSEQ="SPARS10", NSAMP=4, K=3, E=1e6, scan_speed=0.0,
                     x_ref=404.5, y_ref=500.0),
    "small256": dict(grism="G141", SUBARRAY=256, SAMPSEQ="SPARS10", NSAMP=4, K=9, E=3e6, scan_speed=3.0,
                     x_ref=404.5, y_ref=420.0),
    "stare16_128": dict(grism="G141", SUBARRAY=128, SAMPSEQ="SPARS10", NSAMP=16, K=15, E=2e7, scan_speed=0.0,
                        x_ref=400.0, y_ref=470.0, n_wl=900),
    "full3": dict(grism="G141", SUBARRAY=1024, SAMPSEQ="RAPID", NSAMP=3, K=6, E=3e5, scan_speed=20.0,
                  x_ref=404.5 + 379, y_ref=300.0, n_wl=900),
}


class Visit(object):

    def __init__(self, name, detector, grism, calibration, n_exposures=1, seed=1963, E=None, K=None):
        cfg = dict(CONFIGS[name])
        self.name, self.cfg = name, cfg
        self.detector, self.grism, self.calibration = detector, grism, calibration
        self.seed = seed
        self.n_exposures = n_exposures
        self.NSAMP, self.SAMPSEQ, self.SUBARRAY = cfg["NSAMP"], cfg["SAMPSEQ"], cfg["SUBARRAY"]
        self.E = E or cfg["E"]
        self.scan_speed = cfg["scan_speed"]
        self.read_times = detector.get_read_times(self.NSAMP, self.SUBARRAY, self.SAMPSEQ)
        if "sample_rate" in cfg:
            self.sample_mid_points, self.sample_durations, self.read_index = sample_times(
                self.read_times, sample_rate_ms=cfg["sample_rate"])
            self.K = len(self.sample_mid_points)
        else:
            self.K = K or cfg["K"]
        wl = wavelength_grid()
        if "n_wl" in cfg:
            i0, i1 = tools.crop_spectrum_ind(grism.wl_limits[0], grism.wl_limits[1], wl)
            sel = np.linspace(i0, i1 - 1, cfg["n_wl"]).astype(int)
            wl = wl[np.unique(sel)]
        self.wl = wl
        if "sample_rate" not in cfg:
            n_per_read = distribute_samples(self.read_times, self.K)
            self.sample_mid_points, self.sample_durations, self.read_index = sample_times(self.read_times, n_per_read)
        i0, i1 = tools.crop_spectrum_ind(grism.wl_limits[0], grism.wl_limits[1], wl)
        cw = wl[i0:i1]
        sens_wl, sens_val = calibration.sensitivity(grism.name)
        per_flux_unit = (blackbody_shape(cw) * np.interp(cw, sens_wl, sens_val) * tools.bin_centers_to_widths(cw) * 1e4
                         ).sum() * (self.read_times[-1])
        self.stellar_flux = blackbody_shape(wl) * (self.E / per_flux_unit)
        self.depth0 = depth_spectrum(wl)
        self.exp_start_days = np.linspace(-0.1, 0.1, n_exposures) if n_exposures > 1 else np.array([0.0])
        rng = np.random.RandomState(seed)
        self.x_refs = cfg["x_ref"] + rng.uniform(-0.5, 0.5, n_exposures)
        self.y_refs = cfg["y_ref"] + rng.uniform(-0.1, 0.1, n_exposures)
        self.sky = rng.uniform(4.7, 6.7, n_exposures)
        self.x_jitter, self.y_jitter = 0.025, 1e-15
        self.cosmic_rate = cfg.get("cosmic_rate", 11.0)
        self.ssv = cfg.get("ssv")

    def planet_signal(self, i):
        t = self.exp_start_days[i] + self.sample_mid_points / 86400e3
        return transit_shape(t)[:, None] * self.depth0[None, :]

    ORBIT = dict(period=3.524746, sma_over_rs=8.81, eccentricity=0.0, inclination=86.71, periastron=0.0)
    LD = (0.800627, -0.757066, 0.897268, -0.384804)

    def device_depths(self, i):
        from . import lightcurve
        t = self.exp_start_days[i] + self.sample_mid_points / 86400e3
        table = getattr(self, "ld_table", None)
        ld = self.LD if table is None else table.on_grid(self.wl)
        star_spots = getattr(self, "spots", None)
        if star_spots is None:
            z_tr, hidden = lightcurve.depth_inputs(mid_time=0.0, time_array=t, rp_white=np.sqrt(self.depth0.mean()),
                                                   **self.ORBIT)
            return lightcurve.DeviceDepths(z_tr, hidden, self.depth0, ld)
        z_tr, hidden, X, Y = lightcurve.depth_inputs_track(mid_time=0.0, time_array=t,
                                                           rp_white=np.sqrt(self.depth0.mean()), **self.ORBIT)
        return lightcurve.DeviceDepths(z_tr, hidden, self.depth0, ld, spots=star_spots.geometry(X, Y, self.wl))

    def scale_factor(self, i):
        return 1.0 - 0.002 * np.exp(-i / 6.0)

    def frame_kwargs(self, i, **override):
# ... 16 lines not shown
```

Baseline: 3609 exposures/s.

## Precompute per-chunk tile plans in prep and an inverse-gain map for ramp

The prep kernel now reduces, per sub-sample and wavelength chunk, the lane and narrow bounding boxes, the reach and any-flags into a 32-byte TilePlan record. The lane and narrow thrower kernels load that record instead of re-reading per-bin counts and positions and running wave reductions, LDS atomics and barriers to rebuild the same boxes. In addition, the ramp kernel reads a precomputed inverse-gain map in the production path and computes row/column directly when the workgroup spans one row. This adds prep work and a per-chunk write, and relies on the prep chunk size matching the thrower chunk sizes.

```diff
diff --git a/include/wayne_hip.h b/include/wayne_hip.h
--- a/include/wayne_hip.h
+++ b/include/wayne_hip.h
@@ -170,6 +170,9 @@
 uint32_t wayne_source_seed(uint32_t seed, uint32_t tag);
 int wayne_exposure_debug_fetch_source(wayne_ctx *ctx, int slot, int source, int32_t *counts, double *x_pos,
                                       double *y_pos);
+int wayne_exposure_debug_fetch_tile_plan(wayne_ctx *ctx, int slot, int source, int32_t *records, int32_t *nlane,
+                                         int32_t *nwide, int32_t *nsplit, double *sigl, double *sigh);
+int wayne_ctx_debug_fetch_inv_gain(wayne_ctx *ctx, float *inv_gain);
 
 
 typedef struct wayne_trap_desc {
diff --git a/wayne_amd/_lib.py b/wayne_amd/_lib.py
--- a/wayne_amd/_lib.py
+++ b/wayne_amd/_lib.py
@@ -179,6 +179,8 @@
     "wayne_ctx_trap_state_download": (C.c_int, [_vp, _vp]),
     "wayne_exposure_set_trap_history": (C.c_int, [_vp, C.c_int, C.POINTER(TrapHistoryDesc)]),
     "wayne_exposure_debug_fetch_source": (C.c_int, [_vp, C.c_int, C.c_int, _vp, _vp, _vp]),
+    "wayne_exposure_debug_fetch_tile_plan": (C.c_int, [_vp, C.c_int, C.c_int, _vp, _vp, _vp, _vp, _vp, _vp]),
+    "wayne_ctx_debug_fetch_inv_gain": (C.c_int, [_vp, _vp]),
     "wayne_exposure_set_extraction": (C.c_int, [_vp, C.c_int, C.POINTER(ExtractDesc)]),
     "wayne_exposure_fetch_spectra_async": (C.c_int, [_vp, C.c_int]),
     "wayne_exposure_wait_spectra": (C.c_int, [_vp, C.c_int, C.POINTER(_dp), C.POINTER(_dp)]),
@@ -300,7 +302,7 @@
 
 KNOBS = ("tile_ints", "batch", "thin", "no_acc_box", "lane_reach", "throw_wgs", "keep_narrow", "no_fuse", "fork_narrow",
          "streams", "upload_timing", "ramp_reads", "narrow_compact", "lane_tight_tile",
-         "fuse_thrower", "prep_wl_per_run")
+         "fuse_thrower", "prep_wl_per_run", "tile_plan")
 _live_contexts = weakref.WeakSet()
 _knob_defaults = {}
 
@@ -939,6 +941,22 @@
         y = np.empty((K, W), dtype=np.float64)
         self.check(self._L.wayne_exposure_debug_fetch_source(self._h, int(slot), int(source), ptr(counts), ptr(x), ptr(y)))
         return counts, x, y
+
+    def debug_fetch_tile_plan(self, slot, source=0):
+        K, W, R, _ = self._slot_meta[slot]
+        if source > 0:
+            W = self._slot_src[slot][source - 1]
+        rec = np.empty((K, (W + 511) // 512, 8), dtype=np.uint32)
+        nlane, nwide, nsplit = (np.empty((K, W), dtype=np.int32) for _ in range(3))
+        sigl, sigh = np.empty(W, dtype=np.float64), np.empty(W, dtype=np.float64)
+        self.check(self._L.wayne_exposure_debug_fetch_tile_plan(self._h, int(slot), int(source), ptr(rec), ptr(nlane),
+                                                                ptr(nwide), ptr(nsplit), ptr(sigl), ptr(sigh)))
+        return rec, nlane, nwide, nsplit, sigl, sigh
+
+    def debug_fetch_inv_gain(self):
+        out = np.empty((self.S, self.S), dtype=np.float32)
+        self.check(self._L.wayne_ctx_debug_fetch_inv_gain(self._h, ptr(out)))
+        return out
 
     def run(self, slot):
         self.check(self._L.wayne_exposure_run(self._h, int(slot)))
diff --git a/wayne_amd/csrc/common.h b/wayne_amd/csrc/common.h
--- a/wayne_amd/csrc/common.h
+++ b/wayne_amd/csrc/common.h
@@ -97,6 +97,30 @@
                                                               __builtin_amdgcn_readlane(hi, 32) + __builtin_amdgcn_readlane(hi, 48));
   return L + (H << 24);
 }
+
+__device__ __forceinline__ void lane_box_add(int n, int nw, bool sane, int ic, int jc, float sh, float sl, float reach_sigmas,
+                                             int spare, int (&box)[4], float& reach, bool& any) {
+  if (n > 0) {
+    any = true;
+    const bool sig_ok = (nw > 0 ? (sh >= 0.f && sh < 1e6f) : true) && (n > nw ? (sl >= 0.f && sl < 1e6f) : true);
+    const float smax = fmaxf(nw > 0 ? sh : 0.f, n > nw ? sl : 0.f);
+    float r = sig_ok ? reach_sigmas * smax + 1.f : __int_as_float(0x7F800000);
+    if (sane) {
+      box[0] = min(box[0], ic - spare); box[1] = max(box[1], ic + spare);
+      box[2] = min(box[2], jc - spare); box[3] = max(box[3], jc + spare);
+    } else {
+      r = __int_as_float(0x7F800000);
+    }
+    reach = fmaxf(reach, r);
+  }
+}
+__device__ __forceinline__ void narrow_box_add(bool act, int ic0, int jc0, int (&box)[4]) {
+  box[0] = min(box[0], act ? ic0 - kNarrowR : 0x7FFFFFFF); box[1] = max(box[1], act ? ic0 + kNarrowR + 1 : -0x7FFFFFFF);
+  box[2] = min(box[2], act ? jc0 - kNarrowR : 0x7FFFFFFF); box[3] = max(box[3], act ? jc0 + kNarrowR + 1 : -0x7FFFFFFF);
+}
+__device__ __forceinline__ void wave_box(int (&box)[4]) {
+  box[0] = wave_mini(box[0]); box[1] = wave_maxi(box[1]); box[2] = wave_mini(box[2]); box[3] = wave_maxi(box[3]);
+}
 #endif
 
 }
diff --git a/wayne_amd/csrc/k_narrow.h b/wayne_amd/csrc/k_narrow.h
--- a/wayne_amd/csrc/k_narrow.h
+++ b/wayne_amd/csrc/k_narrow.h
@@ -47,8 +47,12 @@
   const int k = blockIdx.x;
   const int tid = threadIdx.x;
   const uint32_t order_word = reinterpret_cast<const uint32_t*>(a.chunk_order)[by >> 2];
-  const int w = (int)((order_word >> (8 * (by & 3))) & 0xFFu) * kNarrowThreads + tid;
+  const int chunk = (int)((order_word >> (8 * (by & 3))) & 0xFFu);
+  const int w = chunk * kNarrowThreads + tid;
   const SubInfo si = a.sub[k];
+  const bool planned = a.tile_plan != nullptr;
+  TilePlan tp{};
+  if (planned) tp = a.tile_plan[(size_t)k * ((a.W + kNarrowThreads - 1) / kNarrowThreads) + chunk];
   int n0 = 0;
   double xd = 0., yd = 0., sgd = 1.;
   if (w < a.W) {
@@ -58,7 +62,8 @@
     yd = a.ypos[kw];
     sgd = a.sigl[w];
   }
-  if (!__syncthreads_or(n0 > 0)) return;
+  if (planned) { if (!(tp.any & kTilePlanNarrowAny)) return; }
+  else if (!__syncthreads_or(n0 > 0)) return;
   const bool split = n0 > 0;
   BinLocal bl{};
   if (split) bl = bin_local(xd, yd);
@@ -66,18 +71,23 @@
   const float sg = split ? (float)sgd : 1.f;
   const int ic0 = bl.ox, jc0 = bl.oy;
   s_pool[tid] = 0;
-  if (tid == 0) { s_box[0] = 0x7FFFFFFF; s_box[1] = -0x7FFFFFFF; s_box[2] = 0x7FFFFFFF; s_box[3] = -0x7FFFFFFF; }
-  __syncthreads();
-  {
-    const int x_lo = wave_mini(act ? ic0 - kNarrowR : 0x7FFFFFFF), x_hi = wave_maxi(act ? ic0 + kNarrowR + 1 : -0x7FFFFFFF);
-    const int y_lo = wave_mini(act ? jc0 - kNarrowR : 0x7FFFFFFF), y_hi = wave_maxi(act ? jc0 + kNarrowR + 1 : -0x7FFFFFFF);
-    if ((tid & 63) == 0) {
-      atomicMin(&s_box[0], x_lo); atomicMax(&s_box[1], x_hi);
-      atomicMin(&s_box[2], y_lo); atomicMax(&s_box[3], y_hi);
-    }
-  }
-  __syncthreads();
-  int tx0 = max(s_box[0], 1), tx1 = min(s_box[1], a.N), ty0 = max(s_box[2], 1), ty1 = min(s_box[3], a.N);
+  int wbox[4] = {tp.narrow_box[0], tp.narrow_box[1], tp.narrow_box[2], tp.narrow_box[3]};
+  if (!planned) {
+    if (tid == 0) { s_box[0] = 0x7FFFFFFF; s_box[1] = -0x7FFFFFFF; s_box[2] = 0x7FFFFFFF; s_box[3] = -0x7FFFFFFF; }
+    __syncthreads();
+    {
+      int box[4] = {0x7FFFFFFF, -0x7FFFFFFF, 0x7FFFFFFF, -0x7FFFFFFF};
+      narrow_box_add(act, ic0, jc0, box);
+      wave_box(box);
+      if ((tid & 63) == 0) {
+        atomicMin(&s_box[0], box[0]); atomicMax(&s_box[1], box[1]);
+        atomicMin(&s_box[2], box[2]); atomicMax(&s_box[3], box[3]);
+      }
+    }
+    __syncthreads();
+    wbox[0] = s_box[0]; wbox[1] = s_box[1]; wbox[2] = s_box[2]; wbox[3] = s_box[3];
+  }
+  int tx0 = max(wbox[0], 1), tx1 = min(wbox[1], a.N), ty0 = max(wbox[2], 1), ty1 = min(wbox[3], a.N);
   int tw = max(tx1 - tx0, 0), th = max(ty1 - ty0, 0);
   if ((long long)tw * th > kNarrowTile) { th = min(th, kNarrowTile / max(tw, 1)); if (th < 1) { th = 0; tw = 0; } }
   const int tarea = tw * th;
@@ -327,8 +337,12 @@
   const int k0 = BATCH ? (int)blockIdx.x * a.kb : (int)blockIdx.x, k1 = BATCH ? min(k0 + a.kb, a.K) : k0 + 1;
   const int tid = threadIdx.x;
   const uint32_t order_word = reinterpret_cast<const uint32_t*>(a.lane_order)[by >> 2];
-  const int w = (int)((order_word >> (8 * (by & 3))) & 0xFFu) * kLaneThreads + tid;
+  const int chunk = (int)((order_word >> (8 * (by & 3))) & 0xFFu);
+  const int w = chunk * kLaneThreads + tid;
   const bool inw = w < a.W;
+  const bool planned = !THIN && !BATCH && !FUSED && a.tile_plan != nullptr;
+  TilePlan tp{};
+  if (planned) tp = a.tile_plan[(size_t)k0 * ((a.W + kLaneThreads - 1) / kLaneThreads) + chunk];
   int n_one = 0, nw_one = 0;
   BinLocal bl_one{};
   float ch = 0.f, cl = 0.f, sh = 0.f, sl = 0.f;
@@ -362,10 +376,10 @@
       s_sub[tid] = make_sub_info(p, k, p.x_ref[k], p.y_ref[k], p.tr + kTrStride * (size_t)k, 0u, 1e300, -1e300, 1e300, -1e300);
     }
   }
-  int x_lo = 0x7FFFFFFF, x_hi = -0x7FFFFFFF, y_lo = 0x7FFFFFFF, y_hi = -0x7FFFFFFF;
+  int box[4] = {0x7FFFFFFF, -0x7FFFFFFF, 0x7FFFFFFF, -0x7FFFFFFF};
   float reach = 0.f;
   bool any = false;
-  for (int k = k0; k < k1; ++k) {
+  for (int k = k0; k < k1 && !planned; ++k) {
     const size_t kw = (size_t)k * a.W + (inw ? w : 0);
     int n = 0, nw = 0;
     int ic = 0, jc = 0;
@@ -389,40 +403,35 @@
         nw = min(max(a.nwide[kw], 0), n);
       }
     }
-    if (n > 0) {
-      any = true;
-      const bool sig_ok = (nw > 0 ? (sh >= 0.f && sh < 1e6f) : true) && (n > nw ? (sl >= 0.f && sl < 1e6f) : true);
-      const float smax = fmaxf(nw > 0 ? sh : 0.f, n > nw ? sl : 0.f);
-      float r = sig_ok ? a.lane_reach_sigmas * smax + 1.f : __int_as_float(0x7F800000);
-      if (sane) {
-        constexpr int spare = FUSED ? 1 : 0;
-        x_lo = min(x_lo, ic - spare); x_hi = max(x_hi, ic + spare); y_lo = min(y_lo, jc - spare); y_hi = max(y_hi, jc + spare);
-      } else {
-        r = __int_as_float(0x7F800000);
-      }
-      reach = fmaxf(reach, r);
-    }
-  }
-  if (!__syncthreads_or(any)) return;
-  if (tid == 0) { s_box[0] = 0x7FFFFFFF; s_box[1] = -0x7FFFFFFF; s_box[2] = 0x7FFFFFFF; s_box[3] = -0x7FFFFFFF; s_reach = 0; s_cnt[0] = 0; s_cnt[1] = 0; }
-  __syncthreads();
-  {
-    x_lo = wave_mini(x_lo); x_hi = wave_maxi(x_hi); y_lo = wave_mini(y_lo); y_hi = wave_maxi(y_hi);
-    const int r_hi = wave_maxi(__float_as_int(reach));
-    if ((tid & 63) == 0) {
-      atomicMin(&s_box[0], x_lo); atomicMax(&s_box[1], x_hi);
-      atomicMin(&s_box[2], y_lo); atomicMax(&s_box[3], y_hi);
-      atomicMax(&s_reach, r_hi);
-    }
-  }
-  __syncthreads();
-  const float reach_wg = __int_as_float(s_reach);
+    lane_box_add(n, nw, sane, ic, jc, sh, sl, a.lane_reach_sigmas, FUSED ? 1 : 0, box, reach, any);
+  }
+  int wbox[4] = {tp.lane_box[0], tp.lane_box[1], tp.lane_box[2], tp.lane_box[3]};
+  float reach_wg = __uint_as_float(tp.lane_reach);
+  if (planned) {
+    if (!(tp.any & kTilePlanLaneAny)) return;
+  } else {
+    if (!__syncthreads_or(any)) return;
+    if (tid == 0) { s_box[0] = 0x7FFFFFFF; s_box[1] = -0x7FFFFFFF; s_box[2] = 0x7FFFFFFF; s_box[3] = -0x7FFFFFFF; s_reach = 0; s_cnt[0] = 0; s_cnt[1] = 0; }
+    __syncthreads();
+    {
+      wave_box(box);
+      const int r_hi = wave_maxi(__float_as_int(reach));
+      if ((tid & 63) == 0) {
+        atomicMin(&s_box[0], box[0]); atomicMax(&s_box[1], box[1]);
+        atomicMin(&s_box[2], box[2]); atomicMax(&s_box[3], box[3]);
+        atomicMax(&s_reach, r_hi);
+      }
+    }
+    __syncthreads();
+    wbox[0] = s_box[0]; wbox[1] = s_box[1]; wbox[2] = s_box[2]; wbox[3] = s_box[3];
+    reach_wg = __int_as_float(s_reach);
+  }
   bool sure = reach_wg <= (float)kLaneReachMax;
   const int margin = sure ? (int)ceilf(reach_wg) : kLaneMargin;
-  const int bx0 = s_box[0] - margin, bx1 = s_box[1] + margin + 1, by0 = s_box[2] - margin, by1 = s_box[3] + margin + 1;
+  const int bx0 = wbox[0] - margin, bx1 = wbox[1] + margin + 1, by0 = wbox[2] - margin, by1 = wbox[3] + margin + 1;
   int tx0 = max(bx0, 1), tx1 = min(bx1, a.N), ty0 = max(by0, 1), ty1 = min(by1, a.N);
   int tw = max(tx1 - tx0, 0), th = max(ty1 - ty0, 0);
-  sure = sure && s_box[0] <= s_box[1] && tx0 == bx0 && tx1 == bx1 && ty0 == by0 && ty1 == by1 && (long long)tw * th <= kLaneTile;
+  sure = sure && wbox[0] <= wbox[1] && tx0 == bx0 && tx1 == bx1 && ty0 == by0 && ty1 == by1 && (long long)tw * th <= kLaneTile;
   while ((long long)tw * th > kLaneTile && th > 1) { ty0 += 1; th = max(th - 2, 1); }
   while ((long long)tw * th > kLaneTile && tw > 1) { tx0 += 1; tw = max(tw - 2, 1); }
   if ((long long)tw * th > kLaneTile) { tw = 0; th = 0; }
diff --git a/wayne_amd/csrc/k_prep.h b/wayne_amd/csrc/k_prep.h
--- a/wayne_amd/csrc/k_prep.h
+++ b/wayne_amd/csrc/k_prep.h
@@ -107,6 +107,8 @@
   double* chunk_box;
   int fix_inline;
   int no_narrow;
+  TilePlan* tile_plan;
+  float lane_reach_sigmas;
 };
 
 __device__ __forceinline__ void raise_status(const PrepArgs& a, int bit) { atomicMax(a.status + (bit >> 1), a.run); }
@@ -358,9 +360,14 @@
 
   const int w = ch * kPrepThreads + tid;
   uint32_t c = 0;
+  int tp_lane = 0, tp_nwide = 0, tp_narrow = 0, tp_ox = 0, tp_oy = 0;
+  bool tp_sane = false;
+  float tp_sh = 0.f, tp_sl = 0.f;
   if (w < W) {
     const size_t kw = (size_t)k * W + w;
-    const BinPlan b = plan_bin(a, k, w, a.wl[w], a.flux[w], a.wa.sens[w], a.wa.dlam[w], a.wa.ratio[w], a.wa.sigl[w], s_tr,
+    const double sigl_w = a.wa.sigl[w];
+    if (a.tile_plan) { tp_sh = (float)a.wa.sigh[w]; tp_sl = (float)sigl_w; }
+    const BinPlan b = plan_bin(a, k, w, a.wl[w], a.flux[w], a.wa.sens[w], a.wa.dlam[w], a.wa.ratio[w], sigl_w, s_tr,
                                x_ref, y_ref, dur, a.depth ? a.depth[kw] : 0.);
     a.xpos[kw] = b.xs;
     a.ypos[kw] = b.ys;
@@ -379,12 +386,37 @@
       c = b.rest;
       if (a.fix_inline && c > 0u) raise_status(a, 2);
       if (a.no_narrow && b.narrow > 0u) raise_status(a, 2);
+      if (a.tile_plan) {
+        tp_lane = (int32_t)b.lane; tp_nwide = b.nwide; tp_narrow = (int32_t)b.narrow;
+        if (tp_lane > 0 || tp_narrow > 0) {
+          const BinLocal bl = bin_local(b.xs, b.ys);
+          tp_sane = bl.sane; tp_ox = bl.ox; tp_oy = bl.oy;
+        }
+      }
     }
   }
   if (overflow) raise_status(a, 1);
   const unsigned long long n_split_total = wave_sum_u32(n_split);
   __shared__ unsigned long long s_split[NW];
   if (lane == 0) s_split[wave] = n_split_total;
+  __shared__ int s_plan[NW][11];
+  if (a.tile_plan) {
+    int lbox[4] = {0x7FFFFFFF, -0x7FFFFFFF, 0x7FFFFFFF, -0x7FFFFFFF}, nbox[4] = {0x7FFFFFFF, -0x7FFFFFFF, 0x7FFFFFFF, -0x7FFFFFFF};
+    float reach = 0.f;
+    bool lane_any = false;
+    lane_box_add(tp_lane, min(max(tp_nwide, 0), tp_lane), tp_sane, tp_ox, tp_oy, tp_sh, tp_sl, a.lane_reach_sigmas, 0, lbox, reach, lane_any);
+    narrow_box_add(tp_narrow > 0 && tp_sane, tp_ox, tp_oy, nbox);
+    wave_box(lbox);
+    wave_box(nbox);
+    const int r_hi = wave_maxi(__float_as_int(reach));
+    const bool l_any = __any(lane_any), n_any = __any(tp_narrow > 0);
+    if (lane == 0) {
+      int* const o = s_plan[wave];
+      o[0] = lbox[0]; o[1] = lbox[1]; o[2] = lbox[2]; o[3] = lbox[3];
+      o[4] = nbox[0]; o[5] = nbox[1]; o[6] = nbox[2]; o[7] = nbox[3];
+      o[8] = r_hi; o[9] = l_any ? 1 : 0; o[10] = n_any ? 1 : 0;
+    }
+  }
 
   if (!a.fix_inline) {
     uint32_t incl = c;
@@ -430,6 +462,22 @@
     unsigned long long tot = 0;
     for (int i = 0; i < NW; ++i) tot += s_split[i];
     if (tot) count_electrons(a.total_electrons, blockIdx.y * gridDim.x + blockIdx.x, tot);
+    if (a.tile_plan) {
+      int m[11];
+      for (int j = 0; j < 11; ++j) m[j] = s_plan[0][j];
+      for (int i = 1; i < NW; ++i) {
+        for (int j = 0; j < 8; j += 2) { m[j] = min(m[j], s_plan[i][j]); m[j + 1] = max(m[j + 1], s_plan[i][j + 1]); }
+        for (int j = 8; j < 11; ++j) m[j] = max(m[j], s_plan[i][j]);
+      }
+      TilePlan tp;
+      for (int j = 0; j < 4; ++j) {
+        tp.lane_box[j] = m[j];
+        tp.narrow_box[j] = (int16_t)min(max(m[4 + j], -32768), 32767);
+      }
+      tp.lane_reach = (uint32_t)m[8];
+      tp.any = (m[9] ? kTilePlanLaneAny : 0u) | (m[10] ? kTilePlanNarrowAny : 0u);
+      a.tile_plan[(size_t)k * gridDim.y + ch] = tp;
+    }
   }
 
   if (a.fix_inline && ch == 0 && tid == 0) a.sub[k] = make_sub_info(a, k, x_ref, y_ref, s_tr, 0u, 1e300, -1e300, 1e300, -1e300);
diff --git a/wayne_amd/csrc/k_ramp.h b/wayne_amd/csrc/k_ramp.h
--- a/wayne_amd/csrc/k_ramp.h
+++ b/wayne_amd/csrc/k_ramp.h
@@ -11,6 +11,7 @@
   const double* read_dt;
   long long* acc;
   const float* pfl;
+  const float* inv_gain;
   const float* sky;
   const float* lin[4];
   const float* dark_sci;
@@ -303,7 +304,10 @@
   const int p_raw = blockIdx.x * blockDim.x + tid;
   const bool valid = p_raw < S * S;
   const int p = valid ? p_raw : 0;
-  const int Y = p / S, X = p - Y * S;
+  const bool row_wg = S == kRampThreads;
+  int Y, X;
+  if (row_wg) { Y = (int)blockIdx.x; X = tid; }
+  else { Y = p / S; X = p - Y * S; }
   const bool interior = valid && (X >= kBorder && X < S - kBorder && Y >= kBorder && Y < S - kBorder);
   const size_t SS = (size_t)S * S;
   OutT* out = (OutT*)a.out;
@@ -358,7 +362,7 @@
   float c1 = 0, c2 = 7e-7f + 1e-12f * (float)(p & 63), c3 = 0, c4 = 0;
 #else
   const float t_sky = (interior && do_sky) ? a.sky[p] : 0.f;
-  const float t_pfl = (interior && gainvar) ? a.pfl[p] : 1.0f;
+  const float t_pfl = (interior && gainvar) ? (PROD ? a.inv_gain[p] : a.pfl[p]) : 1.0f;
   float c1 = 0, c2 = 0, c3 = 0, c4 = 0;
   if (do_lin && valid) { c1 = a.lin[0][p]; c2 = a.lin[1][p]; c3 = a.lin[2][p]; c4 = a.lin[3][p]; }
 #endif
@@ -419,7 +423,9 @@
     }
   }
 
-  const int wy0 = p0 / S, wy1 = min(p0 + 63, S * S - 1) / S, wx0 = p0 - wy0 * S;
+  int wy0, wy1, wx0;
+  if (row_wg) { wy0 = wy1 = (int)blockIdx.x; wx0 = p0 - wy0 * S; }
+  else { wy0 = p0 / S; wy1 = min(p0 + 63, S * S - 1) / S; wx0 = p0 - wy0 * S; }
   unsigned long long live_bits = ~0ull;
   if (a.use_box) {
     uint32_t cbits = 0u;
@@ -445,9 +451,8 @@
     st_out(0, (ArithT)v);
   }
 
-  const float g32 = 2.35f / t_pfl;
   double inv_g = 1.0 / kGain;
-  if (interior && gainvar && !PROD) inv_g = 1.0 / (double)g32;
+  if (interior && gainvar && !PROD) inv_g = 1.0 / (double)(2.35f / t_pfl);
 
   float te_s = 0.f, te_f = 0.f, te_0 = 0.f;
   double td_s = 0., td_f = 0.;
@@ -504,7 +509,7 @@
   if (PROD) {
     {
       const bool f_dark = ALLON || do_dark, f_lin = ALLON || do_lin, f_clip = ALLON || clip, f_rdn = ALLON || rdn;
-      const float inv_gf = !interior ? 0.f : (gainvar ? 1.0f / g32 : (float)(1.0 / kGain));
+      const float inv_gf = !interior ? 0.f : (gainvar ? t_pfl : (float)(1.0 / kGain));
       const float c1p = (1.0f + c1) - 1.0f;
       const float zf = (float)z;
       const bool has_sky_px = skyv > 0.f;
@@ -696,6 +701,14 @@
   ramp_body<OutT, FAST, SKY, NOISE, ALLON, true, true>(a, t, h);
 }
 
+__global__ __launch_bounds__(256) void k_inv_gain(const float* __restrict__ pfl, float* __restrict__ inv_gain, int n) {
+  const int i = blockIdx.x * blockDim.x + threadIdx.x;
+  if (i < n) {
+    const float g32 = 2.35f / pfl[i];
+    inv_gain[i] = 1.0f / g32;
+  }
+}
+
 __global__ __launch_bounds__(256) void k_trap_state_fill(float2* state, int n, float initial_s, float initial_f) {
   const int i = blockIdx.x * blockDim.x + threadIdx.x;
   if (i < n) state[i] = make_float2(initial_s, initial_f);
diff --git a/wayne_amd/csrc/k_throw.h b/wayne_amd/csrc/k_throw.h
--- a/wayne_amd/csrc/k_throw.h
+++ b/wayne_amd/csrc/k_throw.h
@@ -35,6 +35,7 @@
   const float* flat[4];
   long long* acc;
   int32_t* frame;
+  const TilePlan* tile_plan;
 };
 
 struct Affine { uint32_t a, c; };
diff --git a/wayne_amd/csrc/plan_consts.h b/wayne_amd/csrc/plan_consts.h
--- a/wayne_amd/csrc/plan_consts.h
+++ b/wayne_amd/csrc/plan_consts.h
@@ -27,6 +27,15 @@
 constexpr int kMaxChunks = 128;
 constexpr int kLaneListCap = 4096;
 constexpr int kLaneBatchMax = 32;
+
+struct alignas(32) TilePlan {
+  int32_t lane_box[4];
+  uint32_t lane_reach;
+  uint32_t any;
+  int16_t narrow_box[4];
+};
+static_assert(sizeof(TilePlan) == 32, "TilePlan: one 32-byte scalar load");
+constexpr uint32_t kTilePlanLaneAny = 1u, kTilePlanNarrowAny = 2u;
 
 constexpr int kSkyAlias = 256;
 constexpr float kSkyPiece = 16.f;
diff --git a/wayne_amd/csrc/wayne_hip.hip b/wayne_amd/csrc/wayne_hip.hip
--- a/wayne_amd/csrc/wayne_hip.hip
+++ b/wayne_amd/csrc/wayne_hip.hip
@@ -133,6 +133,8 @@
   DevBuf wl, flux, xref, yref;
   DevBuf ratio, sigl, sigh, sens, dlam;
   DevBuf counts, nwide, nsplit, nlane, prefix, xpos, ypos, sub, chunk_total, chunk_box;
+  DevBuf tile_plan;
+  bool plan_last = false;
   DevBuf tr;
   int kb = 1;
   bool thin = false;
@@ -283,6 +285,7 @@
   long long prep_wl_per_run = -1;
   long long fuse_thrower = -1;
   long long lane_tight_tile = -1;
+  long long tile_plan = -1;
   long long ramp_reads = -1;
 };
 struct KnobName { const char* name; const char* env; long long Knobs::*field; };
@@ -297,6 +300,7 @@
     {"lane_tight_tile", "WAYNE_LANE_TIGHT_TILE", &Knobs::lane_tight_tile},
     {"fuse_thrower", "WAYNE_FUSE_THROWER", &Knobs::fuse_thrower},
     {"prep_wl_per_run", "WAYNE_PREP_WL_PER_RUN", &Knobs::prep_wl_per_run},
+    {"tile_plan", "WAYNE_TILE_PLAN", &Knobs::tile_plan},
 };
 constexpr size_t kMiscBytes = 64;
 
@@ -340,6 +344,7 @@
   bool have_cal = false;
   int subarray = 0, N = 0, S = 0, cal_R = 0;
   DevBuf flat[4], pfl, sky, lin[4], dark_sci, dark_err, zero_read;
+  DevBuf inv_gain;
   bool has_flat = false, has_pfl = false, has_sky = false, has_lin = false, has_dark = false,
        has_zero = false;
   float sky_max = 0.f, sky_min = 0.f;
@@ -385,6 +390,7 @@
   HIP_TRY(c, ss.sub.reserve((size_t)K * sizeof(SubInfo)));
   HIP_TRY(c, ss.chunk_total.reserve(K * n_chunks * sizeof(uint32_t)));
   HIP_TRY(c, ss.chunk_box.reserve(K * n_chunks * 4 * sizeof(double)));
+  HIP_TRY(c, ss.tile_plan.reserve(K * n_chunks * sizeof(TilePlan)));
   return WAYNE_OK;
 }
 
@@ -1363,6 +1369,10 @@
   if (c->has_pfl) {
     std::vector<float> v = embed(k->pfl, N, S, 1.0f);
     if ((rc = upload(c, c->pfl, v.data(), SS))) return rc;
+    HIP_TRY(c, c->inv_gain.reserve(SS * sizeof(float)));
+    hipLaunchKernelGGL(k_inv_gain, dim3((unsigned)((SS + 255) / 256)), dim3(256), 0, c->stream, c->pfl.as<float>(),
+                       c->inv_gain.as<float>(), (int)SS);
+    HIP_TRY(c, hipGetLastError());
     HIP_TRY(c, hipStreamSynchronize(c->stream));
   }
   c->has_sky = k->sky != nullptr;
@@ -1595,6 +1605,8 @@
     a.fix_inline = lane_unlimited ? 1 : 0;
     skip_narrow = lane_unlimited && ss.max_narrow <= 6. && !(c->knobs.keep_narrow > 0);
     a.no_narrow = skip_narrow ? 1 : 0;
+    a.tile_plan = (d.rng_mode == WAYNE_RNG_SPLIT && c->knobs.tile_plan != 0) ? ss.tile_plan.as<TilePlan>() : nullptr;
+    a.lane_reach_sigmas = lane_reach_sigmas(c);
     CosmicArgs& ca = cosmic_args;
     ca.R = R; ca.N = N; ca.S = S; ca.seed = ss.seed; ca.exposure = d.exposure_index;
     ca.rate = (src == 0 && d.cosmic_rate >= 0.) ? d.cosmic_rate : -1.;
@@ -1602,6 +1614,7 @@
     ca.seg = s.seg.as<uint32_t>();
     fused = lane_unlimited && skip_narrow && ss.thin && !(c->knobs.no_fuse > 0);
     ss.fused_last = fused;
+    ss.plan_last = !fused && a.tile_plan != nullptr;
     ss.last_prep = a;
     ss.last_chunks = n_chunks;
     if (!fused) {
@@ -1656,6 +1669,7 @@
     for (int i = 0; i < 4; ++i) a.flat[i] = c->has_flat ? c->flat[i].as<float>() : nullptr;
     a.acc = s.acc.as<long long>();
     a.frame = nullptr;
+    a.tile_plan = ss.plan_last ? ss.tile_plan.as<TilePlan>() : nullptr;
     if ((d.flags & WAYNE_F_ADD_FLAT) && !c->has_flat) return fail(c, WAYNE_E_STATE, "run: add_flat without a flat cube");
     const int si_ = slot % c->n_streams;
     const bool fork = d.rng_mode == WAYNE_RNG_SPLIT && c->fork_narrow && !skip_narrow;
@@ -1848,6 +1862,7 @@
   a.read_dt = s.read_dt.as<double>();
   a.acc = s.acc.as<long long>();
   a.pfl = c->has_pfl ? c->pfl.as<float>() : nullptr;
+  a.inv_gain = c->has_pfl ? c->inv_gain.as<float>() : nullptr;
   a.sky = c->has_sky ? c->sky.as<float>() : nullptr;
   for (int i = 0; i < 4; ++i) a.lin[i] = c->has_lin ? c->lin[i].as<float>() : nullptr;
   a.dark_sci = c->has_dark ? c->dark_sci.as<float>() : nullptr;
@@ -2104,6 +2119,38 @@
   return fetch_source(c, slot, source, counts, x_pos, y_pos, nullptr);
 }
 
+int wayne_exposure_debug_fetch_tile_plan(wayne_ctx* c, int slot, int source, int32_t* records, int32_t* nlane, int32_t* nwide,
+                                         int32_t* nsplit, double* sigl, double* sigh) {
+  if (!c || !records) return WAYNE_E_INVALID;
+  if (slot < 0 || slot >= kSlots) return fail(c, WAYNE_E_INVALID, "debug_fetch_tile_plan: slot");
+  Slot& s = c->slots[slot];
+  if (!s.uploaded || !s.front_done) return fail(c, WAYNE_E_STATE, "debug_fetch_tile_plan: run the slot's front half first");
+  if (source < 0 || source > s.n_extra) return fail(c, WAYNE_E_INVALID, "debug_fetch_tile_plan: no such source in this slot");
+  SourceState& ss = s.source(source);
+  if (!ss.plan_last) return fail(c, WAYNE_E_STATE, "debug_fetch_tile_plan: the last run wrote no tile plans (knob tile_plan = 0, a fused front half, or not split mode)");
+  (void)hipSetDevice(c->device);
+  use_slot_stream(c, slot);
+  const size_t n = (size_t)s.K * ((ss.W + kPrepThreads - 1) / kPrepThreads);
+  HIP_TRY(c, hipMemcpyAsync(records, ss.tile_plan.p, n * sizeof(TilePlan), hipMemcpyDeviceToHost, c->stream));
+  const size_t KW = (size_t)s.K * ss.W;
+  if (nlane) HIP_TRY(c, hipMemcpyAsync(nlane, ss.nlane.p, KW * sizeof(int32_t), hipMemcpyDeviceToHost, c->stream));
+  if (nwide) HIP_TRY(c, hipMemcpyAsync(nwide, ss.nwide.p, KW * sizeof(int32_t), hipMemcpyDeviceToHost, c->stream));
+  if (nsplit) HIP_TRY(c, hipMemcpyAsync(nsplit, ss.nsplit.p, KW * sizeof(int32_t), hipMemcpyDeviceToHost, c->stream));
+  if (sigl) HIP_TRY(c, hipMemcpyAsync(sigl, ss.sigl.p, (size_t)ss.W * sizeof(double), hipMemcpyDeviceToHost, c->stream));
+  if (sigh) HIP_TRY(c, hipMemcpyAsync(sigh, ss.sigh.p, (size_t)ss.W * sizeof(double), hipMemcpyDeviceToHost, c->stream));
+  HIP_TRY(c, hipStreamSynchronize(c->stream));
+  return WAYNE_OK;
+}
+
+int wayne_ctx_debug_fetch_inv_gain(wayne_ctx* c, float* inv_gain) {
+  if (!c || !inv_gain) return WAYNE_E_INVALID;
+  if (!c->have_cal || !c->has_pfl) return fail(c, WAYNE_E_STATE, "debug_fetch_inv_gain: no calibration with a pixel flat");
+  (void)hipSetDevice(c->device);
+  { int rc0 = sync_all(c); if (rc0) return rc0; }
+  HIP_TRY(c, hipMemcpy(inv_gain, c->inv_gain.p, (size_t)c->S * c->S * sizeof(float), hipMemcpyDeviceToHost));
+  return WAYNE_OK;
+}
+
 int wayne_exposure_debug_boxes(wayne_ctx* c, int slot, int32_t* boxes, int32_t* segments, int* use_box) {
   if (!c || !boxes || !segments || !use_box) return WAYNE_E_INVALID;
   if (slot < 0 || slot >= kSlots) return fail(c, WAYNE_E_INVALID, "debug_boxes: slot");
diff --git a/wayne_amd/synthetic.py b/wayne_amd/synthetic.py
--- a/wayne_amd/synthetic.py
+++ b/wayne_amd/synthetic.py
@@ -88,6 +88,8 @@
                       x_ref=455.0, y_ref=492.0, n_wl=500),
     "tiny128": dict(grism="G141", SUBARRAY=128, SAMPSEQ="RAPID", NSAMP=5, K=8, E=1e5, scan_speed=60.0,
                     x_ref=400.0, y_ref=460.0, n_wl=900),
+    "plan128": dict(grism="G141", SUBARRAY=128, SAMPSEQ="RAPID", NSAMP=4, K=3, E=3e6, scan_speed=60.0,
+                    x_ref=400.0, y_ref=460.0, n_wl=700),
     "tiny512": dict(grism="G141", SUBARRAY=512, SAMPSEQ="RAPID", NSAMP=3, K=5, E=3e5, scan_speed=8.0,
                     x_ref=330.0, y_ref=420.0, n_wl=1500),
     "ramp16_128": dict(grism="G141", SUBARRAY=128, SAMPSEQ="RAPID", NSAMP=16, K=30, E=3e5, scan_speed=45.0,
```

Measured after the change: 3605 exposures/s. Within noise of the previous version (-0.1%).
